# sepsamavi/safe-interactive-crowdnav

Measured on AMD Instinct MI355X. Metric: sampled trajectories/sec (N x K, 50 denoise steps), higher is better.
Workload: dtype fp16 activations x split-fp16 weights (weight-lo term as one bf8 MFMA per k64), fp32 accumulate; 1 GPU; cfg3: 256 episodes/GPU x N=5 x K=20 x H=12, 50 DDIM steps, JMID; episodes_per_gpu=256, total_episodes=256, humans=5, samples=20, horizon=12, denoise_steps=50, net=jmid, precision=f16mx, class_default_precision=f16mx, lanes=2

## Files before the change

include/jmid_hip.h:

```cpp
#ifndef JMID_HIP_H
#define JMID_HIP_H

#include <stddef.h>
#include <stdint.h>

#ifdef __cplusplus
extern "C" {
#endif
typedef struct jmid_ctx* jmid_handle_t;

#pragma GCC visibility push(default)

enum { JMID_NET_IMID = 0, JMID_NET_JMID = 1 };
enum { JMID_MEM_HOST = 0, JMID_MEM_DEVICE = 1 };
enum { JMID_PREC_F32 = 0, JMID_PREC_F16X3 = 1, JMID_PREC_F16 = 2, JMID_PREC_F16X2 = 3, JMID_PREC_F16MX = 4 };

enum {
    JMID_OK = 0,
    JMID_EINVAL = -1,
    JMID_ENOWEIGHT = -2,
    JMID_EHIP = -3,
    JMID_ENOMEM = -4,
    JMID_ERANGE = -5,
    JMID_ETIMEOUT = -6,
    JMID_EHISTORY = -7
};

const char* jmid_version(void);
int jmid_device_count(void);

int jmid_create(jmid_handle_t* out, int device_id, int net_kind, int ctx_dim, int tf_layer, int nhead,
                int hist_len);
int jmid_destroy(jmid_handle_t h);
const char* jmid_last_error(jmid_handle_t h);

int jmid_load_weight(jmid_handle_t h, const char* name, const float* host_data, size_t n_elems);
int jmid_finalize_weights(jmid_handle_t h);

int jmid_set_ddim_table(jmid_handle_t h, int n_steps, const float* beta, const float* c_e, const float* c_x,
                        const float* n_x, const float* n_e);

int jmid_set_ddpm_table(jmid_handle_t h, int n_steps, const float* beta, const float* c0, const float* c1,
                        const float* sigma, const int* use_noise);

int jmid_encode(jmid_handle_t h, int n_agents, const float* x_st, const float* nbr_sum, const float* edge_mask,
                float* ctx_out, int mem);

int jmid_denoise(jmid_handle_t h, int E, int A, int K, int T, const float* x_T, const float* ctx,
                 const float* p0, float dt, int precision, float* vel_out, float* pos_out, int mem);

int jmid_denoise_ddpm(jmid_handle_t h, int E, int A, int K, int T, const float* x_T, const float* z, const float* ctx,
                      const float* p0, float dt, int precision, float* vel_out, float* pos_out, int mem);

int jmid_net_eval(jmid_handle_t h, int E, int A, int K, int T, int step_idx, const float* x, const float* ctx,
                  int precision, float* e_out, int mem);

int jmid_episode_metrics(jmid_handle_t h, int E, int A, int K, int T, const float* pos, const float* gt,
                         float* out, int mem);

int jmid_eval_statistics(jmid_handle_t h, int E, int A, int K, int T, const float* pos, const float* gt, float* agent_out,
                         float* scene_out, int mem);

int jmid_eval_statistics_masked(jmid_handle_t h, int E, int A, int K, int T, const float* pos, const float* gt,
                                const uint8_t* interp_future, const uint8_t* skip, int n_cut, const int* cutoffs, float* agent_out,
                                float* cut_out, float* scene_out, int mem);

int jmid_collision_statistics(jmid_handle_t h, int E, int A, int K, int T, const float* pos, double threshold,
                              float* pair_out, uint8_t* agent_out, float* sample_out, float* scene_out, int mem);

int jmid_topk(jmid_handle_t h, int E, int A, int K, int T, int k, const float* pos, const float* bw, float* sel, float* logw,
              int mem);

int jmid_predict(jmid_handle_t h, int E, int A, int K, int T, int k, const float* x_st, const float* nbr_sum, const float* edge_mask,
                 const float* x_T, const float* p0, float dt, int precision, const float* bw, float* sel, float* logw, float* pos_out);

int jmid_build_scene(jmid_handle_t h, int E, int N, int F, const double* human_xy, const double* robot_xy, double time_step, int horizon,
                     int force_all_in_cluster, uint8_t* in_cluster_out, uint8_t* robot_in_cluster_out, int* n_in_out, double* cv_out, int mem);

int jmid_scene_get(jmid_handle_t h, float* x, float* x_st, float* nbr_sum, float* edge_mask, float* p0, int mem);

int jmid_predict_scene(jmid_handle_t h, int E, int A, int K, int T, int k, const float* x_T, float dt, int precision, const float* bw,
                       float* sel, float* logw, float* pos_out);

int jmid_build_scene_stamped(jmid_handle_t h, int E, int N, int R, const double* stamps, const double* human_xy, const double* robot_xy,
                             const int* n_frames, double time_step, int horizon, int force_all_in_cluster, uint8_t* in_cluster_out,
                             uint8_t* robot_in_cluster_out, int* n_in_out, int* n_grid_out, double* cv_out, int mem);

int jmid_scene_get_frames(jmid_handle_t h, double* human_xy_out, double* robot_xy_out, double* pose_now_out, int mem);

int jmid_forecast_scene(jmid_handle_t h, int E, int A, int K, int T, int k, const float* x_T, float dt, int precision, const float* bw,
                        double* forecasts_out, double* logw_out);

int jmid_noise_fill(jmid_handle_t h, uint64_t seed, int E, int rows, int T, const uint32_t* episode_ids, int draw, float* out, int mem);

int jmid_denoise_seeded(jmid_handle_t h, int E, int A, int K, int T, uint64_t seed, const uint32_t* episode_ids, const float* ctx,
                        const float* p0, float dt, int precision, float* vel_out, float* pos_out, int mem);

int jmid_predict_scene_seeded(jmid_handle_t h, int E, int A, int K, int T, int k, uint64_t seed, const uint32_t* episode_ids, float dt,
                              int precision, const float* bw, float* sel, float* logw, float* pos_out);
int jmid_forecast_scene_seeded(jmid_handle_t h, int E, int A, int K, int T, int k, uint64_t seed, const uint32_t* episode_ids, float dt,
                               int precision, const float* bw, double* forecasts_out, double* logw_out);

int jmid_set_caller_stream(jmid_handle_t h, void* stream);

int64_t jmid_graph_replays(jmid_handle_t h);

int64_t jmid_erange_count(jmid_handle_t h);
int64_t jmid_timeout_count(jmid_handle_t h);

int jmid_set_chunk_episodes(jmid_handle_t h, int episodes);
int jmid_set_tuning(jmid_handle_t h, const char* key, int value);
int jmid_profile_enable(jmid_handle_t h, uint32_t class_mask);
int jmid_profile_reset(jmid_handle_t h);
int jmid_profile_get(jmid_handle_t h, int cls, int64_t* n_launches, double* total_ms);
int jmid_kernel_class_count(void);
const char* jmid_kernel_class_name(int cls);
int jmid_synchronize(jmid_handle_t h);

#ifdef JMID_DIAGNOSTICS
int jmid_dbg_gemm(jmid_handle_t h, int M, int N, int K, const float* A, const float* Wt, const float* bias, int relu,
                  int precision, float* C);
int jmid_dbg_attention(jmid_handle_t h, int nseq, int S, const float* QKV, int precision, float* OUT);
int jmid_dbg_gemm_ln_mx(jmid_handle_t h, int M, int K, const float* A, const float* Wt, const float* bias, const float* gamma,
                        const float* beta, float* X, int fused);
int jmid_dbg_add_layernorm(jmid_handle_t h, int M, int d, float* X, const float* Y, const float* gamma,
                           const float* beta);
int jmid_dbg_plan_chunks(int net_kind, int nhead, int lanes, int chunk_episodes, int E, int tokens_per_episode, int* sizes, int cap);
int jmid_dbg_plan_chunks_mode(int net_kind, int nhead, int lanes, int chunk_episodes, int E, int tokens_per_episode, int precision, int* sizes, int cap);
#define JMID_DBG_GEMM_PLAN_KNOBS 13
int jmid_dbg_gemm_plan(int mode, int epi, int out, int M, int N, int K, int small_now, int one_chunk, const int* knobs, int* plan);
int jmid_dbg_qkv0(jmid_handle_t h, int E, int A, int K, int T, const float* x, const float* hyp, int hyp_width, int step, int precision,
                  float* qkv, float* thyp_row);
int jmid_dbg_noise_words(jmid_handle_t h, uint64_t seed, int E, int rows, int T, const uint32_t* episode_ids, int draw, uint32_t* out, int mem);
#endif

#pragma GCC visibility pop
#ifdef __cplusplus
}
#endif
#endif
```

safe-interactive-crowdnav_amd/_lib.py:

```python
from __future__ import annotations

import ctypes as C
import os

from .build import library_path

c_float_p = C.POINTER(C.c_float)
Handle = C.c_void_p

NET_IMID, NET_JMID = 0, 1
MEM_HOST, MEM_DEVICE = 0, 1
PREC_F32, PREC_F16X3, PREC_F16, PREC_F16X2, PREC_F16MX = 0, 1, 2, 3, 4
PRECISIONS = {"f32": PREC_F32, "f16x3": PREC_F16X3, "f16": PREC_F16, "f16x2": PREC_F16X2, "f16mx": PREC_F16MX}

ERR_NAMES = {-1: "JMID_EINVAL", -2: "JMID_ENOWEIGHT", -3: "JMID_EHIP", -4: "JMID_ENOMEM", -5: "JMID_ERANGE", -6: "JMID_ETIMEOUT",
             -7: "JMID_EHISTORY"}

SIGNATURES = {
    "jmid_version": (C.c_char_p, []),
    "jmid_device_count": (C.c_int, []),
    "jmid_create": (C.c_int, [C.POINTER(Handle), C.c_int, C.c_int, C.c_int, C.c_int, C.c_int, C.c_int]),
    "jmid_destroy": (C.c_int, [Handle]),
    "jmid_last_error": (C.c_char_p, [Handle]),
    "jmid_load_weight": (C.c_int, [Handle, C.c_char_p, C.c_void_p, C.c_size_t]),
    "jmid_finalize_weights": (C.c_int, [Handle]),
    "jmid_set_ddim_table": (C.c_int, [Handle, C.c_int, C.c_void_p, C.c_void_p, C.c_void_p, C.c_void_p, C.c_void_p]),
    "jmid_set_ddpm_table": (C.c_int, [Handle, C.c_int, C.c_void_p, C.c_void_p, C.c_void_p, C.c_void_p, C.c_void_p]),
    "jmid_denoise_ddpm": (C.c_int, [Handle, C.c_int, C.c_int, C.c_int, C.c_int, C.c_void_p, C.c_void_p, C.c_void_p,
                                    C.c_void_p, C.c_float, C.c_int, C.c_void_p, C.c_void_p, C.c_int]),
    "jmid_encode": (C.c_int, [Handle, C.c_int, C.c_void_p, C.c_void_p, C.c_void_p, C.c_void_p, C.c_int]),
    "jmid_denoise": (C.c_int, [Handle, C.c_int, C.c_int, C.c_int, C.c_int, C.c_void_p, C.c_void_p, C.c_void_p,
                               C.c_float, C.c_int, C.c_void_p, C.c_void_p, C.c_int]),
    "jmid_net_eval": (C.c_int, [Handle, C.c_int, C.c_int, C.c_int, C.c_int, C.c_int, C.c_void_p, C.c_void_p,
                                C.c_int, C.c_void_p, C.c_int]),
    "jmid_episode_metrics": (C.c_int, [Handle, C.c_int, C.c_int, C.c_int, C.c_int, C.c_void_p, C.c_void_p,
                                       C.c_void_p, C.c_int]),
    "jmid_eval_statistics": (C.c_int, [Handle, C.c_int, C.c_int, C.c_int, C.c_int, C.c_void_p, C.c_void_p, C.c_void_p,
                                       C.c_void_p, C.c_int]),
    "jmid_eval_statistics_masked": (C.c_int, [Handle, C.c_int, C.c_int, C.c_int, C.c_int, C.c_void_p, C.c_void_p, C.c_void_p,
                                              C.c_void_p, C.c_int, C.POINTER(C.c_int), C.c_void_p, C.c_void_p, C.c_void_p, C.c_int]),
    "jmid_collision_statistics": (C.c_int, [Handle, C.c_int, C.c_int, C.c_int, C.c_int, C.c_void_p, C.c_double, C.c_void_p,
                                            C.c_void_p, C.c_void_p, C.c_void_p, C.c_int]),
    "jmid_topk": (C.c_int, [Handle, C.c_int, C.c_int, C.c_int, C.c_int, C.c_int, C.c_void_p, C.c_void_p, C.c_void_p,
                            C.c_void_p, C.c_int]),
    "jmid_predict": (C.c_int, [Handle, C.c_int, C.c_int, C.c_int, C.c_int, C.c_int, C.c_void_p, C.c_void_p, C.c_void_p, C.c_void_p,
                               C.c_void_p, C.c_float, C.c_int, C.c_void_p, C.c_void_p, C.c_void_p, C.c_void_p]),
    "jmid_build_scene": (C.c_int, [Handle, C.c_int, C.c_int, C.c_int, C.c_void_p, C.c_void_p, C.c_double, C.c_int, C.c_int, C.c_void_p,
                                   C.c_void_p, C.c_void_p, C.c_void_p, C.c_int]),
    "jmid_scene_get": (C.c_int, [Handle, C.c_void_p, C.c_void_p, C.c_void_p, C.c_void_p, C.c_void_p, C.c_int]),
    "jmid_predict_scene": (C.c_int, [Handle, C.c_int, C.c_int, C.c_int, C.c_int, C.c_int, C.c_void_p, C.c_float, C.c_int, C.c_void_p,
                                     C.c_void_p, C.c_void_p, C.c_void_p]),
    "jmid_build_scene_stamped": (C.c_int, [Handle, C.c_int, C.c_int, C.c_int, C.c_void_p, C.c_void_p, C.c_void_p, C.c_void_p, C.c_double,
                                           C.c_int, C.c_int, C.c_void_p, C.c_void_p, C.c_void_p, C.c_void_p, C.c_void_p, C.c_int]),
    "jmid_scene_get_frames": (C.c_int, [Handle, C.c_void_p, C.c_void_p, C.c_void_p, C.c_int]),
    "jmid_forecast_scene": (C.c_int, [Handle, C.c_int, C.c_int, C.c_int, C.c_int, C.c_int, C.c_void_p, C.c_float, C.c_int, C.c_void_p,
                                      C.c_void_p, C.c_void_p]),
    "jmid_noise_fill": (C.c_int, [Handle, C.c_uint64, C.c_int, C.c_int, C.c_int, C.c_void_p, C.c_int, C.c_void_p, C.c_int]),
    "jmid_denoise_seeded": (C.c_int, [Handle, C.c_int, C.c_int, C.c_int, C.c_int, C.c_uint64, C.c_void_p, C.c_void_p, C.c_void_p,
                                      C.c_float, C.c_int, C.c_void_p, C.c_void_p, C.c_int]),
    "jmid_predict_scene_seeded": (C.c_int, [Handle, C.c_int, C.c_int, C.c_int, C.c_int, C.c_int, C.c_uint64, C.c_void_p, C.c_float, C.c_int,
                                            C.c_void_p, C.c_void_p, C.c_void_p, C.c_void_p]),
    "jmid_forecast_scene_seeded": (C.c_int, [Handle, C.c_int, C.c_int, C.c_int, C.c_int, C.c_int, C.c_uint64, C.c_void_p, C.c_float, C.c_int,
                                             C.c_void_p, C.c_void_p, C.c_void_p]),
    "jmid_set_chunk_episodes": (C.c_int, [Handle, C.c_int]),
    "jmid_set_tuning": (C.c_int, [Handle, C.c_char_p, C.c_int]),
    "jmid_set_caller_stream": (C.c_int, [Handle, C.c_void_p]),
    "jmid_graph_replays": (C.c_int64, [Handle]),
    "jmid_erange_count": (C.c_int64, [Handle]),
    "jmid_timeout_count": (C.c_int64, [Handle]),
    "jmid_profile_enable": (C.c_int, [Handle, C.c_uint32]),
    "jmid_profile_reset": (C.c_int, [Handle]),
    "jmid_profile_get": (C.c_int, [Handle, C.c_int, C.POINTER(C.c_int64), C.POINTER(C.c_double)]),
    "jmid_kernel_class_count": (C.c_int, []),
    "jmid_kernel_class_name": (C.c_char_p, [C.c_int]),
    "jmid_synchronize": (C.c_int, [Handle]),
}

DIAG_SIGNATURES = {
    "jmid_dbg_gemm": (C.c_int, [Handle, C.c_int, C.c_int, C.c_int, C.c_void_p, C.c_void_p, C.c_void_p, C.c_int,
                                C.c_int, C.c_void_p]),
    "jmid_dbg_attention": (C.c_int, [Handle, C.c_int, C.c_int, C.c_void_p, C.c_int, C.c_void_p]),
    "jmid_dbg_gemm_ln_mx": (C.c_int, [Handle, C.c_int, C.c_int, C.c_void_p, C.c_void_p, C.c_void_p, C.c_void_p, C.c_void_p,
                                      C.c_void_p, C.c_int]),
    "jmid_dbg_add_layernorm": (C.c_int, [Handle, C.c_int, C.c_int, C.c_void_p, C.c_void_p, C.c_void_p, C.c_void_p]),
    "jmid_dbg_plan_chunks": (C.c_int, [C.c_int, C.c_int, C.c_int, C.c_int, C.c_int, C.c_int, C.POINTER(C.c_int), C.c_int]),
    "jmid_dbg_plan_chunks_mode": (C.c_int, [C.c_int, C.c_int, C.c_int, C.c_int, C.c_int, C.c_int, C.c_int, C.POINTER(C.c_int), C.c_int]),
    "jmid_dbg_gemm_plan": (C.c_int, [C.c_int] * 8 + [C.POINTER(C.c_int), C.POINTER(C.c_int)]),
    "jmid_dbg_qkv0": (C.c_int, [Handle, C.c_int, C.c_int, C.c_int, C.c_int, C.c_void_p, C.c_void_p, C.c_int, C.c_int, C.c_int, C.c_void_p, C.c_void_p]),
    "jmid_dbg_noise_words": (C.c_int, [Handle, C.c_uint64, C.c_int, C.c_int, C.c_int, C.c_void_p, C.c_int, C.c_void_p, C.c_int]),
}


class JmidError(RuntimeError):
    def __init__(self, code: int, message: str):
        super().__init__(f"{ERR_NAMES.get(code, code)}: {message}")
        self.code = code


_LIBS = {}


def load_library(path: str = None) -> C.CDLL:
    key = os.path.abspath(path or library_path())
    if key in _LIBS:
        return _LIBS[key]
    import torch

    path = key
    if not os.path.exists(path):
        raise ImportError(
            f"{path} is missing: build it with `python -c 'import __graft_entry__ as g; g.build()'` "
            "(hipcc --offload-arch=gfx950).  The predictor has no CPU fallback.")
    lib = C.CDLL(path)
    for name, (res, args) in SIGNATURES.items():
        fn = getattr(lib, name)
        fn.restype = res
        fn.argtypes = args
    lib.has_diagnostics = b"diagnostics" in lib.jmid_version()
    if lib.has_diagnostics:
        for name, (res, args) in DIAG_SIGNATURES.items():
            fn = getattr(lib, name)
            fn.restype = res
            fn.argtypes = args
    _LIBS[key] = lib
    return lib
```

safe-interactive-crowdnav_amd/csrc/common.hpp:

```cpp
#pragma once
#include <hip/hip_runtime.h>
#include <hip/hip_fp16.h>
#include <stdint.h>

#include <atomic>
#include <mutex>

namespace jmid {

typedef float f32x4 __attribute__((ext_vector_type(4)));
typedef float f32x16 __attribute__((ext_vector_type(16)));
typedef _Float16 f16x8 __attribute__((ext_vector_type(8)));
typedef _Float16 f16x4 __attribute__((ext_vector_type(4)));
typedef _Float16 f16x2 __attribute__((ext_vector_type(2)));

constexpr int kWave = 64;
constexpr int kPeMaxLen = 24;

struct HyperLayout {
    int g1, b1, g3, b3, g4, b4, go, bo, total;
};
__host__ __device__ inline HyperLayout make_hyper_layout(int d_model, int d_mid, int d_low) {
    HyperLayout L;
    L.g1 = 0;
    L.b1 = L.g1 + d_model;
    L.g3 = L.b1 + d_model;
    L.b3 = L.g3 + d_mid;
    L.g4 = L.b3 + d_mid;
    L.b4 = L.g4 + d_low;
    L.go = L.b4 + d_low;
    L.bo = L.go + 2;
    L.total = L.bo + 2;
    return L;
}

__device__ __forceinline__ int fast_div(int x, int d, unsigned m) {
    return m ? (int)__umulhi((unsigned)x, m) : (d == 1 ? x : x / d);
}
inline unsigned fast_div_magic(int d, unsigned long long x_max) {
    return d > 1 && x_max * (unsigned long long)d < (1ull << 32) ? (unsigned)((1ull << 32) / (unsigned)d + 1) : 0u;
}

struct RowMap {
    int T, A, KA;
    unsigned mT = 0, mKA = 0, mA = 0;
    __device__ __forceinline__ int ea(int m) const {
        const int r = fast_div(m, T, mT);
        const int e = fast_div(r, KA, mKA);
        const int a = r - fast_div(r, A, mA) * A;
        return e * A + a;
    }
    __device__ __forceinline__ int t_of(int m) const { return m - fast_div(m, T, mT) * T; }
};
inline RowMap make_rowmap(int T, int A, int KA, unsigned long long M) {
    RowMap r{T, A, KA};
    r.mT = fast_div_magic(T, M);
    r.mKA = fast_div_magic(KA, M);
    r.mA = fast_div_magic(A, M);
    return r;
}

__host__ __device__ __forceinline__ size_t blk_index(int row, int k, int K) {
    const int rb = row >> 7, r = row & 127, kb = k >> 5, kk = k & 31;
    return ((size_t)rb * (K >> 5) + kb) * 4096 + (size_t)(r * 32 + ((((kk >> 3) ^ ((r >> 2) & 3)) << 3) | (kk & 7)));
}
__host__ __device__ __forceinline__ size_t blk_plane_elems(size_t rows, int K) {
    return ((rows + 127) / 128) * 128 * (size_t)K;
}

__host__ __device__ __forceinline__ int vt_key_pos(int key) {
    const int g = (key >> 2) & 3;
    return (key & ~15) | ((((g & 1) << 1) | (g >> 1)) << 2) | (key & 3);
}
__host__ __device__ __forceinline__ int vt_spad(int S) { return (S + 15) / 16 * 16; }

template <typename T>
__device__ __forceinline__ void args_now(const T& a) {
    static_assert(sizeof(T) % 4 == 0, "argument block of whole dwords");
    struct Words { unsigned w[sizeof(T) / 4]; };
    const Words w = __builtin_bit_cast(Words, a);
#pragma unroll
    for (unsigned i = 0; i < sizeof(T) / 4; ++i) asm volatile("" ::"s"(w.w[i]));
}
template <typename... T>
__device__ __forceinline__ void args_now_each(const T&... t) { (args_now(t), ...); }

__device__ __forceinline__ unsigned long long pin_uniform(unsigned long long v) {
    asm volatile("" : "+s"(v));
    return v;
}
__device__ __forceinline__ unsigned long long pin_uniform_rfl(unsigned long long v) {
    const unsigned lo = __builtin_amdgcn_readfirstlane((unsigned)v), hi = __builtin_amdgcn_readfirstlane((unsigned)(v >> 32));
    unsigned long long u = ((unsigned long long)hi << 32) | lo;
    asm volatile("" : "+s"(u));
    return u;
}

struct Tuning {
    int fuse_embed = 1;
    int ln_fuse = 0;
    int ln_rows = 0;
    int bystander_lds = 0;
    int gemm_h_variant = 0;
    int gemm_ng = 0;
    int no_vt_direct = 0;
    int attn_h_variant = 0;
    int attn_pack = 1;
    int vt_stage = 0;
    int graph = 0;
    int attn_nsplit = 0;
    int csl_swap = 0;
    int attn_sm = 0;
    int attn_prio = 0;
    int attn_one_wg = 0;
    int h1_stage = 0;
    int out_traj = 0;
    int attn_mx = 0;
    int mx_ln = 0;
    int attn_pf = 0;
    int gemm_small = 0;
    int small_cmb = 0;
    int small_lnx = 0;
    int cus = 256;
    int lnx_polls = 0;
    int lnx_withhold = 0;
    int small_lnx2 = 0;
    int gemm_pn = 0;
    int small_lanes = 0;
    int small_qk = 0;
    int small_pn = 0;
    int qkv0 = 0;
    int attn_abl = 0;
    int gemm_abl = 0;
};
#ifdef JMID_ABLATIONS
inline int attn_abl_bits(const Tuning& t) { return t.attn_abl; }
inline int gemm_abl_bits(const Tuning& t) { return t.gemm_abl; }
#else
inline int attn_abl_bits(const Tuning&) { return 0; }
inline int gemm_abl_bits(const Tuning&) { return 0; }
#endif

struct DevSeen {
    std::atomic<bool> v[64];
    DevSeen() { for (auto& b : v) b.store(false, std::memory_order_relaxed); }
};
struct DeviceOnce {
    std::unique_lock<std::mutex> lk;
    std::atomic<bool>* slot = nullptr;
    explicit operator bool() const { return slot != nullptr; }
    DeviceOnce() = default;
    DeviceOnce(DeviceOnce&& o) noexcept : lk(std::move(o.lk)), slot(o.slot) { o.slot = nullptr; }
    ~DeviceOnce() { if (slot) slot->store(true, std::memory_order_release); }
};
inline std::mutex& device_once_mutex() {
    static std::mutex m;
    return m;
}
inline DeviceOnce first_use_on_device(DevSeen& seen) {
    int dev = 0;
    (void)hipGetDevice(&dev);
    dev &= 63;
    DeviceOnce o;
    if (seen.v[dev].load(std::memory_order_acquire)) return o;
    o.lk = std::unique_lock<std::mutex>(device_once_mutex());
    if (seen.v[dev].load(std::memory_order_acquire)) {
        o.lk.unlock();
        return o;
    }
    o.slot = &seen.v[dev];
    return o;
}

template <auto Kernel, size_t MaxLds = 0, typename... Args>
inline hipError_t launch_with_lds(dim3 grid, dim3 block, size_t lds_bytes, hipStream_t st, Args... args) {
    static DevSeen seen;
    if (auto once_ = first_use_on_device(seen))
        (void)hipFuncSetAttribute(reinterpret_cast<const void*>(Kernel), hipFuncAttributeMaxDynamicSharedMemorySize,
                                  (int)(MaxLds ? MaxLds : lds_bytes));
    hipLaunchKernelGGL(Kernel, grid, block, lds_bytes, st, args...);
    return hipGetLastError();
}

template <typename F>
static inline int bystander_lds(int n, F* fn) {
    if (n > 0) (void)hipFuncSetAttribute((const void*)fn, hipFuncAttributeMaxDynamicSharedMemorySize, n);
    return n;
}

__device__ __forceinline__ float sigmoidf_(float x) { return 1.0f / (1.0f + expf(-x)); }

__device__ __forceinline__ float wave_sum(float v) {
#pragma unroll
    for (int o = 32; o > 0; o >>= 1) v += __shfl_xor(v, o, 64);
    return v;
}

__device__ __forceinline__ void half_swap(float x, float& lo_half, float& hi_half) {
#ifdef JMID_ATT_SHFL
    lo_half = x;
    hi_half = __shfl_xor(x, 32, 64);
#else
    float a = x, b = x;
    asm volatile("s_nop 1\n\tv_permlane32_swap_b32 %0, %1" : "+v"(a), "+v"(b));
    lo_half = a;
    hi_half = b;
#endif
}

__device__ __forceinline__ int frag_row(int reg, int hi) { return (reg & 3) + 8 * (reg >> 2) + 4 * hi; }

}
```

safe-interactive-crowdnav_amd/csrc/jmid_abi.hip:

```cpp
#include "jmid_ctx.hpp"
#include "collision_stats.hpp"

namespace jmid_host {

std::string& thread_error() {
    static thread_local std::string e;
    return e;
}

int fail(jmid_ctx* h, int code, const std::string& msg) {
    if (h) h->err = msg;
    thread_error() = msg;
    return code;
}

int ensure_kde_ws(jmid_ctx* h, size_t need, const char* who) {
    if (need <= h->kde_ws_bytes) return 0;
    if (h->kde_ws) {
        HIPCHK(h, hipStreamSynchronize(h->stream));
        HIPCHK(h, hipFree(h->kde_ws));
        h->kde_ws = nullptr;
        h->kde_ws_bytes = 0;
    }
    if (hipMalloc((void**)&h->kde_ws, need) != hipSuccess) return fail(h, JMID_ENOMEM, std::string(who) + " workspace allocation failed");
// ... 630 lines not shown
    if (int rc = ensure_kde_ws(h, need, "jmid_collision_statistics")) return rc;
    CollisionStatsArgs g{};
    g.E = E; g.A = A; g.K = K; g.T = T;
    g.threshold = threshold;
    g.pos = pos ? pos : h->last_pos;
    g.ws = reinterpret_cast<double*>(h->kde_ws + o_ws);
    g.pair_out = pair_out; g.agent_out = agent_out; g.sample_out = sample_out; g.scene_out = scene_out;
    if (host) {
        if (pos) {
            float* dp = reinterpret_cast<float*>(h->kde_ws + o_pos);
            HIPCHK(h, hipMemcpyAsync(dp, pos, n_pos * 4, hipMemcpyHostToDevice, h->stream));
            g.pos = dp;
        }
        if (pair_out) g.pair_out = reinterpret_cast<float*>(h->kde_ws + o_pr);
        if (agent_out) g.agent_out = reinterpret_cast<unsigned char*>(h->kde_ws + o_ag);
        if (sample_out) g.sample_out = reinterpret_cast<float*>(h->kde_ws + o_sm);
        if (scene_out) g.scene_out = reinterpret_cast<float*>(h->kde_ws + o_sc);
    }
    {
        ProfScope ps(h, KC_EVAL_STATS);
        HIPCHK(h, launch_collision_stats(g, h->stream));
    }
    if (host) {
        if (n_pr) HIPCHK(h, hipMemcpyAsync(pair_out, g.pair_out, n_pr * 4, hipMemcpyDeviceToHost, h->stream));
        if (n_ag) HIPCHK(h, hipMemcpyAsync(agent_out, g.agent_out, n_ag, hipMemcpyDeviceToHost, h->stream));
        if (n_sm) HIPCHK(h, hipMemcpyAsync(sample_out, g.sample_out, n_sm * 4, hipMemcpyDeviceToHost, h->stream));
        if (n_sc) HIPCHK(h, hipMemcpyAsync(scene_out, g.scene_out, n_sc * 4, hipMemcpyDeviceToHost, h->stream));
        HIPCHK(h, hipStreamSynchronize(h->stream));
    }
    return order_out(h, mem);
}

int jmid_topk(jmid_handle_t h, int E, int A, int K, int T, int k, const float* pos, const float* bw, float* sel, float* logw,
              int mem) {
    if (!h || !sel || !logw || E <= 0 || A <= 0 || K <= 1 || T <= 0) return fail(h, JMID_EINVAL, "bad argument");
    if (k < 1 || k > K) return fail(h, JMID_EINVAL, "k must be in 1..K");
    if (A > 32 || K > 1024 || T > 24) return fail(h, JMID_EINVAL, "jmid_topk supports A <= 32, K <= 1024, T <= 24");
    HIPCHK(h, hipSetDevice(h->device));
    if (!pos && !resident_positions(h, E, A, K, T)) return JMID_EINVAL;
    if (int rc = order_in(h, mem)) return rc;
    const int d = 2 * A;
    const size_t n_pos = (size_t)E * K * A * T * 2, n_sel = (size_t)E * A * k * T * 2, n_lw = (size_t)E * A * k;
    auto up = [](size_t b) { return (b + 255) / 256 * 256; };
    const size_t y_bytes = kde_y_in_lds(A, K) ? 0 : up((size_t)E * T * K * d * 8);
    const size_t o_ll = 0, o_Y = up((size_t)E * T * K * 8), o_bw = o_Y + y_bytes, o_pos = o_bw + up(T * 4),
                 o_sel = o_pos + (pos && mem == JMID_MEM_HOST ? up(n_pos * 4) : 0), o_lw = o_sel + (mem == JMID_MEM_HOST ? up(n_sel * 4) : 0),
                 need = o_lw + (mem == JMID_MEM_HOST ? up(n_lw * 4) : 0);
    if (int rc = ensure_kde_ws(h, need, "jmid_topk")) return rc;
    KdeArgs g{};
    g.E = E; g.A = A; g.K = K; g.T = T; g.k = k;
    g.ll = reinterpret_cast<double*>(h->kde_ws + o_ll);
    g.Y = reinterpret_cast<double*>(h->kde_ws + o_Y);
    g.pos = pos ? pos : h->last_pos;
    g.sel = sel; g.logw = logw;
    if (bw) {
        float* dbw = reinterpret_cast<float*>(h->kde_ws + o_bw);
        HIPCHK(h, hipMemcpyAsync(dbw, bw, T * sizeof(float), mem == JMID_MEM_HOST ? hipMemcpyHostToDevice : hipMemcpyDeviceToDevice, h->stream));
        g.bw = dbw;
    }
    if (mem == JMID_MEM_HOST) {
        if (pos) {
            float* dp = reinterpret_cast<float*>(h->kde_ws + o_pos);
            HIPCHK(h, hipMemcpyAsync(dp, pos, n_pos * 4, hipMemcpyHostToDevice, h->stream));
            g.pos = dp;
        }
        g.sel = reinterpret_cast<float*>(h->kde_ws + o_sel);
        g.logw = reinterpret_cast<float*>(h->kde_ws + o_lw);
    }
    {
        ProfScope ps(h, KC_TOPK);
        HIPCHK(h, launch_kde(g, h->stream));
    }
    if (mem == JMID_MEM_HOST) {
        HIPCHK(h, hipMemcpyAsync(sel, g.sel, n_sel * 4, hipMemcpyDeviceToHost, h->stream));
        HIPCHK(h, hipMemcpyAsync(logw, g.logw, n_lw * 4, hipMemcpyDeviceToHost, h->stream));
        HIPCHK(h, hipStreamSynchronize(h->stream));
    }
    return order_out(h, mem);
}

int jmid_predict(jmid_handle_t h, int E, int A, int K, int T, int k, const float* x_st, const float* nbr_sum, const float* edge_mask,
                 const float* x_T, const float* p0, float dt, int precision, const float* bw, float* sel, float* logw, float* pos_out) {
    if (!h) return JMID_EINVAL;
    if (int rc = check_ready(h)) return rc;
    if (E <= 0 || A <= 0 || K <= 0 || T <= 0 || k < 1 || k > K) return fail(h, JMID_EINVAL, "jmid_predict: bad dimensions");
    if (!x_st || !nbr_sum || !edge_mask || !x_T || !p0) return fail(h, JMID_EINVAL, "jmid_predict: null input");
    const bool rank = k < K;
    if (rank && (!sel || !logw)) return fail(h, JMID_EINVAL, "jmid_predict: k < K needs sel and logw");
    if (!rank && !pos_out) return fail(h, JMID_EINVAL, "jmid_predict: k == K needs pos_out");
    if (rank && (A > 32 || K > 1024 || T > 24)) return fail(h, JMID_EINVAL, "jmid_predict: the device top-k supports A <= 32, K <= 1024, T <= 24");
    if (h->ddpm) return fail(h, JMID_EINVAL, "jmid_predict samples with DDIM (MID.eval_sicnav: sampling=\"ddim\", MID/mid.py:333)");
    HIPCHK(h, hipSetDevice(h->device));
    return predict_chain(h, E, A, K, T, k, x_st, nbr_sum, edge_mask, x_T, p0, dt, precision, bw, sel, logw, pos_out, false, "jmid_predict");
}

int jmid_build_scene(jmid_handle_t h, int E, int N, int F, const double* human_xy, const double* robot_xy, double time_step, int horizon,
                     int force_all_in_cluster, uint8_t* in_cluster_out, uint8_t* robot_in_cluster_out, int* n_in_out, double* cv_out, int mem) {
    if (!h) return JMID_EINVAL;
    if (E <= 0 || !human_xy || !robot_xy || !in_cluster_out || !robot_in_cluster_out || !n_in_out) return fail(h, JMID_EINVAL, "jmid_build_scene: bad argument");
    if (int rc = check_scene_dims(h, "jmid_build_scene", N, F, cv_out, horizon, time_step)) return rc;
    HIPCHK(h, hipSetDevice(h->device));
    if (int rc = order_in(h, mem)) return rc;
    if (int rc = build_scene_resident(h, E, N, F, human_xy, robot_xy, mem == JMID_MEM_HOST ? 0 : 1, time_step, horizon, force_all_in_cluster,
                                      in_cluster_out, robot_in_cluster_out, n_in_out, cv_out, mem))
        return rc;
    return order_out(h, mem);
}

int jmid_build_scene_stamped(jmid_handle_t h, int E, int N, int R, const double* stamps, const double* human_xy, const double* robot_xy,
                             const int* n_frames, double time_step, int horizon, int force_all_in_cluster, uint8_t* in_cluster_out,
                             uint8_t* robot_in_cluster_out, int* n_in_out, int* n_grid_out, double* cv_out, int mem) {
    if (!h) return JMID_EINVAL;
    if (E <= 0 || !stamps || !human_xy || !robot_xy || !in_cluster_out || !robot_in_cluster_out || !n_in_out || !n_grid_out)
        return fail(h, JMID_EINVAL, "jmid_build_scene_stamped: bad argument");
    if (R < 1 || R > FRM_MAX_R) return fail(h, JMID_EINVAL, "jmid_build_scene_stamped supports 1 <= R <= 64 raw frames");
    const int F = h->hist_len;
    if (int rc = check_scene_dims(h, "jmid_build_scene_stamped", N, F, cv_out, horizon, time_step)) return rc;
    const double wd = std::nearbyint(time_step * 100.0);
    if (!(wd >= 1.0) || wd > 9.0e15) return fail(h, JMID_EINVAL, "jmid_build_scene_stamped: round(time_step * 100) must be at least 1");
    const bool host = mem == JMID_MEM_HOST;
    if (host && n_frames)
        for (int e = 0; e < E; ++e)
            if (n_frames[e] < 1 || n_frames[e] > R)
                return fail(h, JMID_EINVAL, "jmid_build_scene_stamped: n_frames[" + std::to_string(e) + "] = " + std::to_string(n_frames[e]) + " is outside 1..R");
    HIPCHK(h, hipSetDevice(h->device));
    if (int rc = order_in(h, mem)) return rc;
    auto up = [](size_t b) { return (b + 255) / 256 * 256; };
    const size_t b_st = (size_t)E * R * 8, b_hum = (size_t)E * R * N * 2 * 8, b_rob = (size_t)E * R * 2 * 8, b_nf = n_frames ? (size_t)E * 4 : 0;
    const GridBlock gb = grid_block(E, N, F);
    const size_t o_ng = gb.end, o_st = o_ng + up((size_t)E * 4), o_rh = o_st + (host ? up(b_st) : 0), o_rr = o_rh + (host ? up(b_hum) : 0),
                 o_nf = o_rr + (host ? up(b_rob) : 0), need = o_nf + (host ? up(b_nf) : 0), raw = need - o_st;
    if (need > h->frames_bytes) {
        HIPCHK(h, hipStreamSynchronize(h->stream));
        if (h->frames_dev) HIPCHK(h, hipFree(h->frames_dev));
        h->frames_dev = nullptr;
        h->frames_bytes = 0;
        if (hipMalloc((void**)&h->frames_dev, need) != hipSuccess) return fail(h, JMID_ENOMEM, "jmid_build_scene_stamped: workspace allocation failed");
        h->frames_bytes = need;
    }
    if (int rc = ensure_pin(h, raw + (size_t)E * 4, "jmid_build_scene_stamped")) return rc;
    char* fd = h->frames_dev;
    FramesArgs f{};
    f.E = E; f.N = N; f.R = R; f.F = F;
    f.w = (long long)wd;
    f.stamps = stamps; f.human_xy = human_xy; f.robot_xy = robot_xy; f.n_frames = n_frames;
    f.o_human = reinterpret_cast<double*>(fd + gb.o_hum); f.o_robot = reinterpret_cast<double*>(fd + gb.o_rob);
    f.o_pose = reinterpret_cast<double*>(fd + gb.o_pose); f.o_n_grid = reinterpret_cast<int*>(fd + o_ng);
    if (host) {
        std::memcpy(h->pin, stamps, b_st);
        std::memcpy(h->pin + (o_rh - o_st), human_xy, b_hum);
        std::memcpy(h->pin + (o_rr - o_st), robot_xy, b_rob);
        if (n_frames) std::memcpy(h->pin + (o_nf - o_st), n_frames, b_nf);
        HIPCHK(h, hipMemcpyAsync(fd + o_st, h->pin, raw, hipMemcpyHostToDevice, h->stream));
        f.stamps = reinterpret_cast<const double*>(fd + o_st); f.human_xy = reinterpret_cast<const double*>(fd + o_rh);
        f.robot_xy = reinterpret_cast<const double*>(fd + o_rr);
        f.n_frames = n_frames ? reinterpret_cast<const int*>(fd + o_nf) : nullptr;
    }
    HIPCHK(h, launch_frames(f, h->stream));
    int* ng = reinterpret_cast<int*>(h->pin + raw);
    HIPCHK(h, hipMemcpyAsync(ng, f.o_n_grid, (size_t)E * 4, hipMemcpyDeviceToHost, h->stream));
    if (!host) HIPCHK(h, hipMemcpyAsync(n_grid_out, f.o_n_grid, (size_t)E * 4, hipMemcpyDeviceToDevice, h->stream));
    HIPCHK(h, hipStreamSynchronize(h->stream));
    if (host) std::memcpy(n_grid_out, ng, (size_t)E * 4);
    for (int e = 0; e < E; ++e)
        if (ng[e] < 0) {
            (void)order_out(h, mem);
            return fail(h, JMID_EINVAL, "jmid_build_scene_stamped: n_frames[" + std::to_string(e) + "] is outside 1..R");
        }
    for (int e = 0; e < E; ++e)
        if (ng[e] < F) {
            const int got = ng[e];
            (void)order_out(h, mem);
            return fail(h, JMID_EHISTORY, "jmid_build_scene_stamped: episode " + std::to_string(e) + " has " + std::to_string(got) +
                                              " history frames on the time_step grid, " + std::to_string(F) + " needed");
        }
    if (int rc = build_scene_resident(h, E, N, F, reinterpret_cast<const double*>(fd), nullptr, 2, time_step, horizon, force_all_in_cluster,
                                      in_cluster_out, robot_in_cluster_out, n_in_out, cv_out, mem))
        return rc;
    return order_out(h, mem);
}

int jmid_scene_get_frames(jmid_handle_t h, double* human_xy_out, double* robot_xy_out, double* pose_now_out, int mem) {
    if (!h) return JMID_EINVAL;
    const jmid_ctx::SceneWs& sc = h->scene;
    if (!sc.E) return fail(h, JMID_EINVAL, "jmid_scene_get_frames needs a preceding jmid_build_scene on this handle");
    HIPCHK(h, hipSetDevice(h->device));
    if (int rc = order_in(h, mem)) return rc;
    const size_t F = h->hist_len, row = (size_t)sc.N * 2 * 8;
    const hipMemcpyKind kind = mem == JMID_MEM_HOST ? hipMemcpyDeviceToHost : hipMemcpyDeviceToDevice;
    if (human_xy_out) HIPCHK(h, hipMemcpyAsync(human_xy_out, sc.dev + sc.o_hum, (size_t)sc.E * F * row, kind, h->stream));
    if (robot_xy_out) HIPCHK(h, hipMemcpyAsync(robot_xy_out, sc.dev + sc.o_rob, (size_t)sc.E * F * 2 * 8, kind, h->stream));
    if (pose_now_out) {
        if (sc.stamped) HIPCHK(h, hipMemcpyAsync(pose_now_out, sc.dev + sc.o_pose, (size_t)sc.E * row, kind, h->stream));
        else
            HIPCHK(h, hipMemcpy2DAsync(pose_now_out, row, sc.dev + sc.o_hum + (F - 1) * row, F * row, row, sc.E, kind, h->stream));
    }
    if (mem == JMID_MEM_HOST) HIPCHK(h, hipStreamSynchronize(h->stream));
    return order_out(h, mem);
}

int jmid_scene_get(jmid_handle_t h, float* x, float* x_st, float* nbr_sum, float* edge_mask, float* p0, int mem) {
    if (!h) return JMID_EINVAL;
    const jmid_ctx::SceneWs& sc = h->scene;
    if (!sc.E) return fail(h, JMID_EINVAL, "jmid_scene_get needs a preceding jmid_build_scene on this handle");
    HIPCHK(h, hipSetDevice(h->device));
    if (int rc = order_in(h, mem)) return rc;
    const size_t rows = (size_t)sc.E * sc.N, F = h->hist_len;
    const hipMemcpyKind kind = mem == JMID_MEM_HOST ? hipMemcpyDeviceToHost : hipMemcpyDeviceToDevice;
    if (x) HIPCHK(h, hipMemcpyAsync(x, sc.dev + sc.o_x, rows * F * 6 * 4, kind, h->stream));
    if (x_st) HIPCHK(h, hipMemcpyAsync(x_st, sc.dev + sc.o_xst, rows * F * 6 * 4, kind, h->stream));
    if (nbr_sum) HIPCHK(h, hipMemcpyAsync(nbr_sum, sc.dev + sc.o_nbr, rows * 2 * F * 6 * 4, kind, h->stream));
    if (edge_mask) HIPCHK(h, hipMemcpyAsync(edge_mask, sc.dev + sc.o_em, rows * 2 * 4, kind, h->stream));
    if (p0) HIPCHK(h, hipMemcpyAsync(p0, sc.dev + sc.o_p0, rows * 2 * 4, kind, h->stream));
    if (mem == JMID_MEM_HOST) HIPCHK(h, hipStreamSynchronize(h->stream));
    return order_out(h, mem);
}

int jmid_predict_scene(jmid_handle_t h, int E, int A, int K, int T, int k, const float* x_T, float dt, int precision, const float* bw, float* sel,
                       float* logw, float* pos_out) {
    return predict_scene_entry(h, "jmid_predict_scene", E, A, K, T, k, x_T, nullptr, dt, precision, bw, sel, logw, pos_out, nullptr, nullptr, false);
}

int jmid_forecast_scene(jmid_handle_t h, int E, int A, int K, int T, int k, const float* x_T, float dt, int precision, const float* bw,
                        double* forecasts_out, double* logw_out) {
    return predict_scene_entry(h, "jmid_forecast_scene", E, A, K, T, k, x_T, nullptr, dt, precision, bw, nullptr, nullptr, nullptr, forecasts_out,
                               logw_out, true);
}

int jmid_predict_scene_seeded(jmid_handle_t h, int E, int A, int K, int T, int k, uint64_t seed, const uint32_t* episode_ids, float dt, int precision,
                              const float* bw, float* sel, float* logw, float* pos_out) {
    const SeedArgs sa{seed, episode_ids};
    return predict_scene_entry(h, "jmid_predict_scene_seeded", E, A, K, T, k, nullptr, &sa, dt, precision, bw, sel, logw, pos_out, nullptr, nullptr, false);
}

int jmid_forecast_scene_seeded(jmid_handle_t h, int E, int A, int K, int T, int k, uint64_t seed, const uint32_t* episode_ids, float dt, int precision,
                               const float* bw, double* forecasts_out, double* logw_out) {
    const SeedArgs sa{seed, episode_ids};
    return predict_scene_entry(h, "jmid_forecast_scene_seeded", E, A, K, T, k, nullptr, &sa, dt, precision, bw, nullptr, nullptr, nullptr, forecasts_out,
                               logw_out, true);
}

int jmid_denoise_seeded(jmid_handle_t h, int E, int A, int K, int T, uint64_t seed, const uint32_t* episode_ids, const float* ctx, const float* p0,
                        float dt, int precision, float* vel_out, float* pos_out, int mem) {
    if (!h) return JMID_EINVAL;
    if (!episode_ids) return fail(h, JMID_EINVAL, "jmid_denoise_seeded: null episode_ids");
    const SeedArgs sa{seed, episode_ids};
    return run_network(h, E, A, K, T, nullptr, ctx, p0, dt, precision, -1, vel_out, pos_out, nullptr, mem, nullptr, &sa);
}

int jmid_noise_fill(jmid_handle_t h, uint64_t seed, int E, int rows, int T, const uint32_t* episode_ids, int draw, float* out, int mem) {
    return noise_entry(h, "jmid_noise_fill", seed, E, rows, T, episode_ids, draw, out, nullptr, mem);
}

int jmid_set_chunk_episodes(jmid_handle_t h, int episodes) {
    if (!h || episodes < 0) return JMID_EINVAL;
    h->chunk_eps = episodes;
    drop_graphs(h);
    return JMID_OK;
}

int jmid_set_tuning(jmid_handle_t h, const char* key, int value) {
    if (!h || !key) return JMID_EINVAL;
    const std::string k(key);
    struct Knob {
        const char* name;
        int Tuning::*field;
        int lo, hi;
    };
#ifdef JMID_DIAGNOSTICS
    static const Knob knobs[] = {
        {"gemm_h_variant", &Tuning::gemm_h_variant, 0, 8},
        {"attn_pack", &Tuning::attn_pack, 0, 1},
        {"fuse_embed", &Tuning::fuse_embed, 0, 1},
        {"bystander_lds", &Tuning::bystander_lds, 0, 160 * 1024},
        {"ln_rows", &Tuning::ln_rows, 0, 128},
        {"ln_fuse", &Tuning::ln_fuse, 0, 2},
        {"no_vt_direct", &Tuning::no_vt_direct, 0, 1},
        {"gemm_ng", &Tuning::gemm_ng, 0, 64},
        {"attn_h_variant", &Tuning::attn_h_variant, 0, 2},
        {"vt_stage", &Tuning::vt_stage, 0, 3},
        {"graph", &Tuning::graph, 0, 2},
        {"attn_nsplit", &Tuning::attn_nsplit, 0, 16},
        {"attn_mx", &Tuning::attn_mx, 0, 3},
        {"out_traj", &Tuning::out_traj, 0, 2},
        {"attn_pf", &Tuning::attn_pf, 0, 2},
        {"attn_one_wg", &Tuning::attn_one_wg, 0, 1},
        {"attn_sm", &Tuning::attn_sm, 0, 2},
        {"attn_prio", &Tuning::attn_prio, 0, 2},
        {"mx_ln", &Tuning::mx_ln, 0, 2},
        {"csl_swap", &Tuning::csl_swap, 0, 3},
        {"h1_stage", &Tuning::h1_stage, 0, 2},
        {"gemm_small", &Tuning::gemm_small, 0, 2},
        {"gemm_pn", &Tuning::gemm_pn, 0, 8},
        {"small_lanes", &Tuning::small_lanes, 0, 2},
        {"small_cmb", &Tuning::small_cmb, 0, 2},
        {"small_lnx", &Tuning::small_lnx, 0, 2},
        {"cus", &Tuning::cus, 0, 4096},
        {"lnx_polls", &Tuning::lnx_polls, 0, 1 << 20},
        {"lnx_withhold", &Tuning::lnx_withhold, 0, 1},
        {"small_lnx2", &Tuning::small_lnx2, 0, 2},
        {"small_qk", &Tuning::small_qk, 0, 2},
        {"small_pn", &Tuning::small_pn, 0, 8},
        {"qkv0", &Tuning::qkv0, 0, 2},
#ifdef JMID_ABLATIONS
        {"attn_abl", &Tuning::attn_abl, 0, 1 << 30},
        {"gemm_abl", &Tuning::gemm_abl, 0, 1 << 30},
#endif
    };
#endif
    if (k == "lanes") {
        if (value < 1 || value > jmid_ctx::kMaxLanes) return fail(h, JMID_EINVAL, "lanes must be 1..4");
        h->lanes = value;
        return JMID_OK;
    }
#ifdef JMID_DIAGNOSTICS
    for (const Knob& kn : knobs)
        if (k == kn.name) {
            if (value < kn.lo || value > kn.hi || (k == "ln_rows" && value != 0 && value != 64 && value != 128))
                return fail(h, JMID_EINVAL, k + " out of range");
            h->tune.*(kn.field) = value;
            if (k == "cus" && value == 0) {
                int cus = 0;
                h->tune.cus = hipDeviceGetAttribute(&cus, hipDeviceAttributeMultiprocessorCount, h->device) == hipSuccess && cus > 0 ? cus : 256;
            }
            drop_graphs(h);
            return JMID_OK;
        }
#endif
    return fail(h, JMID_EINVAL, "unknown tuning key " + k);
}

int64_t jmid_graph_replays(jmid_handle_t h) { return h ? h->graph_replays : -1; }

int64_t jmid_erange_count(jmid_handle_t h) { return h ? h->erange_calls : -1; }
int64_t jmid_timeout_count(jmid_handle_t h) { return h ? h->lnx_timeouts : -1; }

int jmid_set_caller_stream(jmid_handle_t h, void* stream) {
    if (!h) return JMID_EINVAL;
    h->caller_stream = reinterpret_cast<hipStream_t>(stream);
    return JMID_OK;
}

int jmid_synchronize(jmid_handle_t h) {
    if (!h) return JMID_EINVAL;
    HIPCHK(h, hipSetDevice(h->device));
    HIPCHK(h, hipStreamSynchronize(h->stream));
    return JMID_OK;
}

}
```

safe-interactive-crowdnav_amd/csrc/jmid_ctx.hpp:

```cpp
#pragma once
#include "../../include/jmid_hip.h"

#include <hip/hip_runtime.h>

#include <algorithm>
#include <cmath>
#include <cstdio>
#include <cstring>
#include <map>
#include <string>
#include <vector>

#include "attn_f16x3.hpp"
#include "attn_f32.hpp"
#include "common.hpp"
#include "elementwise.hpp"
#include "encoder.hpp"
#include "eval_stats.hpp"
#include "gemm_f16x3.hpp"
#include "gemm_ln_f16x3.hpp"
#include "gemm_ln2_mx.hpp"
#include "gemm_small.hpp"
#include "gemm_f32.hpp"
#include "kde.hpp"
#include "launch_plan.hpp"
#include "noise.hpp"
#include "qkv0.hpp"
#include "scene.hpp"
#include "frames.hpp"

using namespace jmid;

enum KClass {
    KC_GEMM_QKV = 0,
    KC_GEMM_OUT,
    KC_GEMM_FF1,
    KC_GEMM_FF2,
    KC_GEMM_TAIL,
    KC_ATTN,
    KC_ADD_LN,
    KC_EMBED,
    KC_OUT_DDIM,
    KC_HYPER,
    KC_ENCODER,
    KC_INTEGRATE,
    KC_METRICS,
    KC_VTRANS,
    KC_TOPK,
    KC_EVAL_STATS,
    KC_COUNT
};
extern const char* const kClassNames[KC_COUNT];

struct DevBuf {
    float* p = nullptr;
    size_t n = 0;
};

struct EvPair {
    hipEvent_t a, b;
};

struct HalfPair {
    half_t* hi = nullptr;
    half_t* lo = nullptr;
};

struct LinearW {
    const float *W = nullptr, *bias = nullptr;
    HalfPair split;
    HalfPair k16;
    const unsigned char* w8 = nullptr;
};
struct NormW {
    const float *gamma = nullptr, *beta = nullptr;
};
struct LayerW {
    LinearW in_proj, out_proj, linear1, linear2;
    NormW norm1, norm2;
};
struct WeightTable {
    std::vector<LayerW> layers;
    LinearW concat1, concat3, concat4, linear;
    const float* edge_v = nullptr;
};

struct jmid_ctx {
    int device = 0;
    hipStream_t stream = nullptr;
    static constexpr int kMaxLanes = 4;
    hipStream_t lane_stream[kMaxLanes - 1] = {nullptr, nullptr, nullptr};
    hipEvent_t ev_fork = nullptr, ev_join[kMaxLanes - 1] = {nullptr, nullptr, nullptr};
    int lanes = 2;
    Tuning tune;
    hipStream_t caller_stream = nullptr;
    hipEvent_t ev_in = nullptr, ev_out = nullptr;
    struct LoopGraph {
        hipGraphExec_t exec = nullptr;
        char* arena = nullptr;
        bool warm = false;
    };
    std::map<std::string, LoopGraph> graphs;
    int64_t graph_replays = 0;
    const float* last_pos = nullptr;
    int last_pos_dims[4] = {0, 0, 0, 0};
    char* kde_ws = nullptr;
    size_t kde_ws_bytes = 0;
    char* pin = nullptr;
    size_t pin_bytes = 0;
    char* io_dev = nullptr;
    size_t io_dev_bytes = 0;
    struct SceneWs {
        char* dev = nullptr;
        size_t bytes = 0;
        int E = 0, N = 0;
        size_t o_x = 0, o_xst = 0, o_nbr = 0, o_em = 0, o_p0 = 0, o_inc = 0;
        std::vector<int> n_in;
        size_t o_hum = 0, o_rob = 0, o_pose = 0, o_cv = 0;
        bool stamped = false;
        int horizon = 0;
    } scene;
    char* frames_dev = nullptr;
    size_t frames_bytes = 0;
    unsigned* noise_ids = nullptr;
    int noise_ids_cap = 0;
    unsigned* noise_ids_pin = nullptr;
    hipEvent_t ev_ids = nullptr;
    bool chained = false;
    int64_t erange_calls = 0;
    unsigned lnx_epoch = 0;
    bool lnx_off = false;
    int64_t lnx_timeouts = 0;
    int x2 = 0;
    int net_kind = 1, ctx_dim = 256, tf_layer = 3, nhead = 4, hist_len = 6;
    int d = 512, ff = 1024, dmid = 256, dlow = 128, H = 128;
    HyperLayout hl;
    std::map<std::string, std::vector<size_t>> expected;
    std::map<std::string, DevBuf> w;
    std::map<std::string, HalfPair> wsplit;
    struct W8Image { unsigned char* p = nullptr; };
    std::map<std::string, W8Image> w8;
    int mx = 0;
    std::map<std::string, HalfPair> w16;
    WeightTable wt;
    int* range_flag = nullptr;
    bool weights_in_half_range = true;
    bool finalized = false;
    float* pe = nullptr;
    float* ppe = nullptr;
    float* Whyp = nullptr;
    float* bhyp = nullptr;
    float* thyp = nullptr;
    std::vector<float> time_w;
    float* lstmT[3][3] = {{nullptr}};
    float* attW1T = nullptr;
    float* attW2T = nullptr;
    std::vector<float> beta, c_e, c_x, n_x, n_e;
    bool ddpm = false;
    std::vector<float> p_c0, p_c1, p_sigma;
    std::vector<int> p_noise;
    char* arena = nullptr;
    size_t arena_bytes = 0;
    int chunk_eps = 0;
    uint32_t prof_mask = 0;
    std::vector<EvPair> prof_ev[KC_COUNT];
    std::vector<EvPair> ev_pool;
    double prof_ms[KC_COUNT] = {0};
    int64_t prof_n[KC_COUNT] = {0};
    std::string err;
};

constexpr size_t kLnxWords = 2 * jmid::SM_LNX_GRANULES;

namespace jmid_host {

std::string& thread_error();
int fail(jmid_ctx* h, int code, const std::string& msg);

#define HIPCHK(h, expr)                                                                               \
    do {                                                                                              \
        hipError_t e__ = (expr);                                                                      \
        if (e__ != hipSuccess)                                                                        \
            return fail(h, JMID_EHIP, std::string(#expr) + ": " + hipGetErrorString(e__));            \
    } while (0)

struct ProfScope {
    jmid_ctx* h;
    int cls;
    bool on;
    EvPair ev;
    ProfScope(jmid_ctx* h_, int cls_) : h(h_), cls(cls_), on((h_->prof_mask >> cls_) & 1u) {
        if (on) {
            if (!h->ev_pool.empty()) {
                ev = h->ev_pool.back();
                h->ev_pool.pop_back();
            } else {
                hipEventCreate(&ev.a);
                hipEventCreate(&ev.b);
            }
            hipEventRecord(ev.a, h->stream);
        }
    }
    ~ProfScope() {
        if (on) {
            hipEventRecord(ev.b, h->stream);
            h->prof_ev[cls].push_back(ev);
        }
    }
};

struct Carver {
    char* base;
    size_t off = 0;
    explicit Carver(char* b) : base(b) {}
    float* take(size_t nfloats) {
        float* p = reinterpret_cast<float*>(base ? base + off : nullptr);
        off += ((nfloats * sizeof(float) + 255) / 256) * 256;
        return p;
    }
};

inline size_t numel(const std::vector<size_t>& s) {
    size_t n = 1;
    for (size_t v : s) n *= v;
    return n;
}

void register_shapes(jmid_ctx* h);
int dev_alloc_copy(jmid_ctx* h, float** out, const std::vector<float>& host);
int fetch_host(jmid_ctx* h, const std::string& name, std::vector<float>& out);
int upload_time_table(jmid_ctx* h);
int make_w8(jmid_ctx* h, const float* dW, int N, int K, jmid_ctx::W8Image* out);
void free_planes(jmid_ctx* h);
void drop_graphs(jmid_ctx* h);
void sync_lanes(jmid_ctx* h);
int ensure_arena(jmid_ctx* h, size_t bytes);
std::vector<int> plan_chunks(const jmid_ctx* h, int E, int tokens_per_episode);
int check_ready(jmid_ctx* h);
int order_in(jmid_ctx* h, int mem);
int order_out(jmid_ctx* h, int mem);
struct SeedArgs {
    uint64_t seed;
    const uint32_t* ids;
};
int upload_noise_ids(jmid_ctx* h, const uint32_t* ids, int E);
int fill_noise(jmid_ctx* h, uint64_t seed, const unsigned* ids_dev, int E, size_t n, int draw, float* out, unsigned* words, hipStream_t stream);
int run_network(jmid_ctx* h, int E, int A, int K, int T, const float* x_in, const float* ctx, const float* p0, float dt,
                int precision, int single_step, float* vel_out, float* pos_out, float* e_out, int mem,
                const float* z_in = nullptr, const SeedArgs* seeded = nullptr);
int flagged_call(jmid_ctx* h, int flag);
int launch_episode_metrics(jmid_ctx* h, const float* pos, const float* gt, float* out, int E, int K, int A, int T);
#ifdef JMID_DIAGNOSTICS
int dbg_qkv0(jmid_ctx* h, int E, int A, int K, int T, const float* x, const float* hyp, int hyp_width, int step, int precision, float* qkv, float* thyp_row);
#endif
int noise_entry(jmid_ctx* h, const char* who, uint64_t seed, int E, int rows, int T, const uint32_t* episode_ids, int draw, float* out,
                unsigned* words, int mem);
int prof_collect(jmid_ctx* h);

}
using namespace jmid_host;
```

safe-interactive-crowdnav_amd/csrc/jmid_diag.hip:

```cpp
#include "jmid_ctx.hpp"
#include "jmid_launch.hpp"

#ifdef JMID_DIAGNOSTICS
extern "C" {

int jmid_dbg_plan_chunks(int net_kind, int nhead, int lanes, int chunk_episodes, int E, int tokens_per_episode, int* sizes, int cap) {
    if (E <= 0 || tokens_per_episode <= 0 || nhead <= 0 || !sizes || cap <= 0) return JMID_EINVAL;
    jmid_ctx ctx;
    ctx.net_kind = net_kind; ctx.nhead = nhead; ctx.lanes = lanes; ctx.chunk_eps = chunk_episodes;
    const std::vector<int> plan = plan_chunks(&ctx, E, tokens_per_episode);
    for (size_t i = 0; i < plan.size() && (int)i < cap; ++i) sizes[i] = plan[i];
    return (int)plan.size();
}

int jmid_dbg_plan_chunks_mode(int net_kind, int nhead, int lanes, int chunk_episodes, int E, int tokens_per_episode, int precision, int* sizes, int cap) {
    if (E <= 0 || tokens_per_episode <= 0 || nhead <= 0 || !sizes || cap <= 0) return JMID_EINVAL;
    if (precision != JMID_PREC_F32 && precision != JMID_PREC_F16X3 && precision != JMID_PREC_F16X2 && precision != JMID_PREC_F16MX) return JMID_EINVAL;
    jmid_ctx ctx;
    ctx.net_kind = net_kind; ctx.nhead = nhead; ctx.lanes = lanes; ctx.chunk_eps = chunk_episodes;
    ctx.mx = precision == JMID_PREC_F16MX;
    ctx.x2 = precision == JMID_PREC_F16X2 || ctx.mx;
    const std::vector<int> plan = plan_chunks(&ctx, E, tokens_per_episode);
    for (size_t i = 0; i < plan.size() && (int)i < cap; ++i) sizes[i] = plan[i];
    return (int)plan.size();
}

int jmid_dbg_gemm_plan(int mode, int epi, int out, int M, int N, int K, int small_now, int one_chunk, const int* knobs, int* plan) {
    if (mode < GM_X3 || mode > GM_MX || epi < EPI_BIAS || epi > EPI_CSL || (out != OUT_F32 && out != OUT_SPLIT && out != OUT_QKV && out != OUT_LNX) ||
        M <= 0 || N <= 0 || K <= 0 || !knobs || !plan || knobs[0] < 0 || knobs[0] > 8)
        return JMID_EINVAL;
    Tuning t;
    int Tuning::*const fields[JMID_DBG_GEMM_PLAN_KNOBS] = {&Tuning::gemm_h_variant, &Tuning::gemm_small, &Tuning::ln_rows, &Tuning::small_lnx, &Tuning::small_lnx2,
                                                           &Tuning::cus, &Tuning::vt_stage, &Tuning::csl_swap, &Tuning::h1_stage, &Tuning::gemm_pn,
                                                           &Tuning::small_qk, &Tuning::small_pn, &Tuning::gemm_ng};
    for (int i = 0; i < JMID_DBG_GEMM_PLAN_KNOBS; ++i) t.*fields[i] = knobs[i];
    CallFacts cf;
    cf.small_now = small_now;
    cf.one_chunk = one_chunk;
    const GemmPlan p = plan_gemm((GemmMode)mode, epi, out, M, N, K, cf, t);
    plan[0] = p.mode; plan[1] = p.shape; plan[2] = p.flags; plan[3] = p.group_tiles;
    plan[4] = gemm_shape_bm(p.shape); plan[5] = gemm_shape_bn(p.shape);
    plan[6] = plan_ln_rows(false, M, t); plan[7] = plan_ln_rows(true, M, t);
    return JMID_OK;
}

int jmid_dbg_gemm(jmid_handle_t h, int M, int N, int K, const float* A, const float* Wt, const float* bias, int relu,
                  int precision, float* C) {
    if (!h || !A || !Wt || !C) return JMID_EINVAL;
    if (precision != JMID_PREC_F32 && precision != JMID_PREC_F16X3 && precision != JMID_PREC_F16X2 && precision != JMID_PREC_F16MX)
        return fail(h, JMID_EINVAL, "bad precision");
    h->mx = precision == JMID_PREC_F16MX;
    h->x2 = precision == JMID_PREC_F16X2 || h->mx;
    HIPCHK(h, hipSetDevice(h->device));
    if (!h->range_flag) {
        HIPCHK(h, hipMalloc((void**)&h->range_flag, sizeof(int)));
        HIPCHK(h, hipMemsetAsync(h->range_flag, 0, sizeof(int), h->stream));
    }
    float *dA, *dW, *dB = nullptr, *dC;
    HIPCHK(h, hipMalloc((void**)&dA, (size_t)M * K * 4));
    HIPCHK(h, hipMalloc((void**)&dW, (size_t)N * K * 4));
    HIPCHK(h, hipMalloc((void**)&dC, (size_t)M * N * 4));
    HIPCHK(h, hipMemcpy(dA, A, (size_t)M * K * 4, hipMemcpyHostToDevice));
    HIPCHK(h, hipMemcpy(dW, Wt, (size_t)N * K * 4, hipMemcpyHostToDevice));
    if (bias) {
        HIPCHK(h, hipMalloc((void**)&dB, (size_t)N * 4));
        HIPCHK(h, hipMemcpy(dB, bias, (size_t)N * 4, hipMemcpyHostToDevice));
    }
    int rc = 0;
    half_t *ah = nullptr, *al = nullptr, *wh = nullptr, *wl = nullptr;
    jmid_ctx::W8Image w8img;
    if (precision == JMID_PREC_F32) {
        GemmArgs g{};
        g.A = dA; g.lda = K; g.W = dW; g.ldw = K; g.bias = dB; g.C = dC; g.ldc = N; g.M = M; g.N = N; g.K = K;
        rc = relu ? run_gemm<EPI_BIAS_RELU>(h, KC_GEMM_QKV, g) : run_gemm<EPI_BIAS>(h, KC_GEMM_QKV, g);
    } else {
        const size_t pa = blk_plane_elems(M, K) * 2, pw = blk_plane_elems(N, K) * 2;
        HIPCHK(h, hipMalloc((void**)&ah, pa));
        HIPCHK(h, hipMalloc((void**)&al, pa));
        HIPCHK(h, hipMalloc((void**)&wh, pw));
        HIPCHK(h, hipMalloc((void**)&wl, pw));
        for (auto pr : {std::make_pair(ah, pa), std::make_pair(al, pa), std::make_pair(wh, pw), std::make_pair(wl, pw)})
            HIPCHK(h, hipMemsetAsync(pr.first, 0, pr.second, h->stream));
        hipLaunchKernelGGL(split_planes_blocked_kernel, dim3(512), dim3(256), 0, h->stream, dA, ah, al, M, K,
                           h->range_flag, 1.0f);
        hipLaunchKernelGGL(split_planes_blocked_kernel, dim3(512), dim3(256), 0, h->stream, dW, wh, wl, N, K,
                           h->range_flag, kWScale);
        GemmHArgs g{};
        g.Ahi = ah; g.Alo = al; g.Whi = wh; g.Wlo = wl; g.bias = dB; g.C = dC; g.ldc = N;
        g.M = M; g.N = N; g.K = K;
        if (h->mx && N % 32 == 0 && K % 64 == 0) {
            if (int rc8 = make_w8(h, dW, N, K, &w8img)) return rc8;
            g.W8 = w8img.p;
        }
        const GemmPlan plan = plan_gemm(gemm_mode(h), relu ? EPI_BIAS_RELU : EPI_BIAS, OUT_F32, M, N, K, CallFacts{}, h->tune);
        rc = relu ? run_gemm_h<EPI_BIAS_RELU, OUT_F32>(h, KC_GEMM_QKV, g, plan) : run_gemm_h<EPI_BIAS, OUT_F32>(h, KC_GEMM_QKV, g, plan);
    }
    if (!rc) {
        hipError_t e = hipStreamSynchronize(h->stream);
        if (e != hipSuccess) rc = fail(h, JMID_EHIP, hipGetErrorString(e));
    }
    if (!rc) HIPCHK(h, hipMemcpy(C, dC, (size_t)M * N * 4, hipMemcpyDeviceToHost));
    hipFree(dA); hipFree(dW); hipFree(dC);
    if (dB) hipFree(dB);
    for (half_t* p : {ah, al, wh, wl})
        if (p) hipFree(p);
    if (w8img.p) hipFree(w8img.p);
    return rc;
}

int jmid_dbg_attention(jmid_handle_t h, int nseq, int S, const float* QKV, int precision, float* OUT) {
    if (!h || !QKV || !OUT) return JMID_EINVAL;
    if (precision != JMID_PREC_F32 && precision != JMID_PREC_F16X3 && precision != JMID_PREC_F16X2 && precision != JMID_PREC_F16MX)
        return fail(h, JMID_EINVAL, "bad precision");
    h->mx = precision == JMID_PREC_F16MX;
    h->x2 = precision == JMID_PREC_F16X2 || h->mx;
    HIPCHK(h, hipSetDevice(h->device));
    if (!h->range_flag) {
        HIPCHK(h, hipMalloc((void**)&h->range_flag, sizeof(int)));
        HIPCHK(h, hipMemsetAsync(h->range_flag, 0, sizeof(int), h->stream));
    }
    const size_t Mt = (size_t)nseq * S;
    const int d = h->d, hd = h->d / h->nhead;
    float *dQ, *dO;
    HIPCHK(h, hipMalloc((void**)&dQ, Mt * 3 * d * 4));
    HIPCHK(h, hipMalloc((void**)&dO, Mt * d * 4));
    HIPCHK(h, hipMemcpy(dQ, QKV, Mt * 3 * d * 4, hipMemcpyHostToDevice));
    int rc = 0;
    std::vector<half_t*> tmp;
    if (precision == JMID_PREC_F32) {
        AttnArgs aa{dQ, dO, S, d, h->nhead, 1.0f / sqrtf((float)hd), nullptr, nullptr};
        ProfScope ps(h, KC_ATTN);
        hipError_t e = launch_attn_f32(aa, nseq, hd, plan_attn(hd, h->tune).pack, h->stream);
        if (e != hipSuccess) rc = fail(h, JMID_EHIP, hipGetErrorString(e));
    } else {
        const int Spad = vt_spad(S);
        const size_t vt = (size_t)nseq * d * Spad;
        half_t* b[8];
        const size_t sz[8] = {Mt * d, Mt * d, Mt * d, Mt * d, vt, vt, blk_plane_elems(Mt, d), blk_plane_elems(Mt, d)};
        for (int i = 0; i < 8; ++i) {
            HIPCHK(h, hipMalloc((void**)&b[i], sz[i] * sizeof(half_t)));
            HIPCHK(h, hipMemsetAsync(b[i], 0, sz[i] * sizeof(half_t), h->stream));
            tmp.push_back(b[i]);
        }
        hipLaunchKernelGGL(qkv_to_planes_kernel, dim3(512), dim3(256), 0, h->stream, dQ, b[0], b[1], b[2], b[3], b[4],
                           b[5], Mt, d, hd, S, Spad, 1.4426950408889634f / sqrtf((float)hd));
        int ns = 1;
        float *opart = nullptr, *mlpart = nullptr;
        if (hd == 128) ns = attn_pick_nsplit(((S + 127) / 128) * h->nhead * nseq, S);
        if (ns > 1) {
            HIPCHK(h, hipMalloc((void**)&opart, (size_t)ns * Mt * d * 4));
            HIPCHK(h, hipMalloc((void**)&mlpart, (size_t)ns * Mt * h->nhead * 2 * 4));
            tmp.push_back(reinterpret_cast<half_t*>(opart));
            tmp.push_back(reinterpret_cast<half_t*>(mlpart));
        }
        AttnHArgs aa{b[0], b[1], b[2], b[3], b[4], b[5], b[6], b[7], S, Spad, d, h->nhead, 1.0f / sqrtf((float)hd),
                     h->range_flag, ns, opart, mlpart, h->x2};
        {
            ProfScope ps(h, KC_ATTN);
            hipError_t e = launch_attn_f16x3(aa, nseq, hd, plan_attn(hd, h->tune), h->stream);
            if (e != hipSuccess) rc = fail(h, JMID_EHIP, hipGetErrorString(e));
        }
        hipLaunchKernelGGL(merge_planes_kernel, dim3(512), dim3(256), 0, h->stream, b[6], b[7], dO, (int)Mt, d);
    }
    if (!rc) {
        hipError_t e = hipStreamSynchronize(h->stream);
        if (e != hipSuccess) rc = fail(h, JMID_EHIP, hipGetErrorString(e));
    }
    if (!rc) HIPCHK(h, hipMemcpy(OUT, dO, Mt * d * 4, hipMemcpyDeviceToHost));
    hipFree(dQ); hipFree(dO);
    for (half_t* p : tmp) hipFree(p);
    return rc;
}

int jmid_dbg_gemm_ln_mx(jmid_handle_t h, int M, int K, const float* A, const float* Wt, const float* bias, const float* gamma,
                        const float* beta, float* X, int fused) {
    if (!h || !A || !Wt || !bias || !gamma || !beta || !X || M <= 0 || K % 64 != 0) return JMID_EINVAL;
    constexpr int N = GLN_BN;
    HIPCHK(h, hipSetDevice(h->device));
    h->mx = 1;
    h->x2 = 1;
    if (!h->range_flag) {
        HIPCHK(h, hipMalloc((void**)&h->range_flag, sizeof(int)));
        HIPCHK(h, hipMemsetAsync(h->range_flag, 0, sizeof(int), h->stream));
    }
    std::vector<void*> tmp;
    auto dalloc = [&](size_t bytes, const void* host) -> void* {
        void* p = nullptr;
        if (hipMalloc(&p, bytes) != hipSuccess) return nullptr;
        tmp.push_back(p);
        if (host) (void)hipMemcpy(p, host, bytes, hipMemcpyHostToDevice);
        else (void)hipMemsetAsync(p, 0, bytes, h->stream);
        return p;
    };
    float* dA = (float*)dalloc((size_t)M * K * 4, A);
    float* dW = (float*)dalloc((size_t)N * K * 4, Wt);
    float* dB = (float*)dalloc(N * 4, bias);
    float* dG = (float*)dalloc(N * 4, gamma);
    float* dT = (float*)dalloc(N * 4, beta);
    float* dX = (float*)dalloc((size_t)M * N * 4, X);
    float* dY = (float*)dalloc((size_t)(M + 63) / 64 * 64 * N * 4, nullptr);
    const size_t pa = blk_plane_elems(M, K) * 2, pw = blk_plane_elems(N, K) * 2, px = blk_plane_elems(M, N) * 2;
    half_t* ah = (half_t*)dalloc(pa, nullptr);
    half_t* al = (half_t*)dalloc(pa, nullptr);
    half_t* wh = (half_t*)dalloc(pw, nullptr);
    half_t* wl = (half_t*)dalloc(pw, nullptr);
    half_t* w16h = (half_t*)dalloc((size_t)N * K * 2, nullptr);
    half_t* w16l = (half_t*)dalloc((size_t)N * K * 2, nullptr);
    half_t* xh = (half_t*)dalloc(px, nullptr);
    unsigned char* xl8 = (unsigned char*)dalloc(px, nullptr);
    for (void* p : tmp)
        if (!p) return fail(h, JMID_ENOMEM, "jmid_dbg_gemm_ln_mx: allocation failed");
    hipLaunchKernelGGL(split_planes_blocked_kernel, dim3(512), dim3(256), 0, h->stream, dA, ah, al, M, K, h->range_flag, 1.0f);
    hipLaunchKernelGGL(split_planes_blocked_kernel, dim3(512), dim3(256), 0, h->stream, dW, wh, wl, N, K, h->range_flag, kWScale);
    hipLaunchKernelGGL(split_planes_k16_kernel, dim3(256), dim3(256), 0, h->stream, dW, w16h, w16l, N, K);
    hipLaunchKernelGGL(split_planes_lo8_kernel, dim3(512), dim3(256), 0, h->stream, dX, xh, xl8, M);
    jmid_ctx::W8Image img;
    if (int rc = make_w8(h, dW, N, K, &img)) return rc;
    tmp.push_back(img.p);
    int rc = 0;
    if (fused == 1) {
        GemmLn2Args g2{ah, w16h, img.p, dB, dG, dT, xh, xl8, M, K, 1e-5f, h->range_flag, 0};
        hipError_t e = launch_gemm_ln2_mx(g2, plan_ln_rows(true, M, h->tune), h->stream);
        if (e != hipSuccess) rc = fail(h, JMID_EHIP, hipGetErrorString(e));
    } else {
        GemmHArgs g{};
        g.Ahi = ah; g.Alo = al; g.Whi = wh; g.Wlo = wl; g.W8 = img.p; g.bias = dB; g.C = dY; g.ldc = N; g.M = M; g.N = N; g.K = K;
        if (fused == 3) {
            unsigned long long* xs = (unsigned long long*)dalloc(kLnxWords * sizeof(unsigned), nullptr);
            const GemmPlan lnx = plan_gemm(GM_MX, EPI_BIAS, OUT_LNX, M, N, K, CallFacts{}, h->tune);
            if (!xs || lnx.shape == GS_NONE) return fail(h, JMID_EINVAL, "jmid_dbg_gemm_ln_mx: shape does not take the small kernel with the statistics exchange");
            g.ln_gamma = dG; g.ln_beta = dT; g.ln_xh = xh; g.ln_xl = nullptr; g.ln_xl8 = xl8; g.ln_xchg = xs; g.ln_eps = 1e-5f; g.ln_no_lo = 0;
            (void)hipMemsetAsync(h->range_flag, 0, sizeof(int), h->stream);
            rc = run_gemm_lnx_small(h, KC_GEMM_OUT, g, lnx);
            if (!rc) {
                int flag = 0;
                (void)hipMemcpyAsync(&flag, h->range_flag, sizeof(int), hipMemcpyDeviceToHost, h->stream);
                (void)hipStreamSynchronize(h->stream);
                if (flag & 2) rc = fail(h, JMID_EHIP, "jmid_dbg_gemm_ln_mx: a workgroup gave up waiting for its row tile's statistics");
            }
        } else
        {
        rc = run_gemm_h<EPI_BIAS, OUT_F32>(h, KC_GEMM_OUT, g, plan_gemm(GM_MX, EPI_BIAS, OUT_F32, M, N, K, CallFacts{}, h->tune));
        if (!rc) rc = run_add_ln(h, nullptr, dY, dG, dT, M, N, xh, reinterpret_cast<half_t*>(xl8), true, 0);
        }
    }
    if (!rc) {
        hipLaunchKernelGGL(merge_planes_lo8_kernel, dim3(512), dim3(256), 0, h->stream, xh, xl8, dX, M);
        hipError_t e = hipStreamSynchronize(h->stream);
        if (e != hipSuccess) rc = fail(h, JMID_EHIP, hipGetErrorString(e));
    }
    if (!rc) HIPCHK(h, hipMemcpy(X, dX, (size_t)M * N * 4, hipMemcpyDeviceToHost));
    for (void* p : tmp) hipFree(p);
    return rc;
}

int jmid_dbg_add_layernorm(jmid_handle_t h, int M, int d, float* X, const float* Y, const float* gamma,
                           const float* beta) {
    if (!h || !X || !Y || !gamma || !beta) return JMID_EINVAL;
    HIPCHK(h, hipSetDevice(h->device));
    float *dX, *dY, *dG, *dB;
    HIPCHK(h, hipMalloc((void**)&dX, (size_t)M * d * 4));
    HIPCHK(h, hipMalloc((void**)&dY, (size_t)M * d * 4));
    HIPCHK(h, hipMalloc((void**)&dG, (size_t)d * 4));
    HIPCHK(h, hipMalloc((void**)&dB, (size_t)d * 4));
    HIPCHK(h, hipMemcpy(dX, X, (size_t)M * d * 4, hipMemcpyHostToDevice));
    HIPCHK(h, hipMemcpy(dY, Y, (size_t)M * d * 4, hipMemcpyHostToDevice));
    HIPCHK(h, hipMemcpy(dG, gamma, (size_t)d * 4, hipMemcpyHostToDevice));
    HIPCHK(h, hipMemcpy(dB, beta, (size_t)d * 4, hipMemcpyHostToDevice));
    int rc = run_add_ln(h, dX, dY, dG, dB, M, d);
    if (!rc) {
        hipError_t e = hipStreamSynchronize(h->stream);
        if (e != hipSuccess) rc = fail(h, JMID_EHIP, hipGetErrorString(e));
    }
    if (!rc) HIPCHK(h, hipMemcpy(X, dX, (size_t)M * d * 4, hipMemcpyDeviceToHost));
    hipFree(dX); hipFree(dY); hipFree(dG); hipFree(dB);
    return rc;
}

int jmid_dbg_qkv0(jmid_handle_t h, int E, int A, int K, int T, const float* x, const float* hyp, int hyp_width, int step, int precision,
                  float* qkv, float* thyp_row) {
    if (!h) return JMID_EINVAL;
    return dbg_qkv0(h, E, A, K, T, x, hyp, hyp_width, step, precision, qkv, thyp_row);
}

int jmid_dbg_noise_words(jmid_handle_t h, uint64_t seed, int E, int rows, int T, const uint32_t* episode_ids, int draw, uint32_t* out, int mem) {
    return noise_entry(h, "jmid_dbg_noise_words", seed, E, rows, T, episode_ids, draw, nullptr, out, mem);
}

}
#endif
```

safe-interactive-crowdnav_amd/csrc/jmid_planner.hip:

```cpp
#include "jmid_ctx.hpp"
#include "jmid_launch.hpp"

namespace jmid_host {

void drop_graphs(jmid_ctx* h) {
    for (auto& kv : h->graphs)
        if (kv.second.exec) hipGraphExecDestroy(kv.second.exec);
    h->graphs.clear();
}

void sync_lanes(jmid_ctx* h) {
    for (int l = 0; l + 1 < jmid_ctx::kMaxLanes; ++l)
        if (h->lane_stream[l]) (void)hipStreamSynchronize(h->lane_stream[l]);
    if (h->stream) (void)hipStreamSynchronize(h->stream);
}

int ensure_arena(jmid_ctx* h, size_t bytes) {
    if (bytes <= h->arena_bytes) return 0;
    drop_graphs(h);
    h->last_pos = nullptr;
    if (h->arena) {
        sync_lanes(h);
        HIPCHK(h, hipFree(h->arena));
        h->arena = nullptr;
        h->arena_bytes = 0;
    }
    hipError_t e = hipMalloc((void**)&h->arena, bytes);
    if (e != hipSuccess) return fail(h, JMID_ENOMEM, "workspace allocation of " + std::to_string(bytes) + " bytes failed");
    h->arena_bytes = bytes;
    return 0;
}

struct StepBuffers {
    float *X, *QKV, *ATT, *Y, *H1, *Y3, *Y4;
    half_t *Xh, *Xl, *Qh, *Ql, *Kh, *Kl, *Vh, *Vl, *Vth, *Vtl, *Ah, *Al, *H1h, *H1l, *Y3h, *Y3l;
    size_t vt_elems;
    float *Opart, *MLpart;
    float *coef, *uvc;
    unsigned long long* ln_xchg;
};

half_t* take_half(Carver& c, size_t n) { return reinterpret_cast<half_t*>(c.take((n + 1) / 2)); }

struct SeqGeom {
    int nseq, S, Spad;
};
SeqGeom seq_geom(const jmid_ctx* h, int Ec, int A, int K, int T) {
    SeqGeom g;
    g.nseq = h->net_kind == JMID_NET_JMID ? Ec : Ec * K * A;
    g.S = h->net_kind == JMID_NET_JMID ? K * A * T : T;
    g.Spad = vt_spad(g.S);
    return g;
}

size_t step_ws_floats(const jmid_ctx* h, size_t Mc, int precision, const SeqGeom& sg, int nsplit, StepBuffers* sb,
                      char* base, size_t qkv0_rows) {
    Carver c(base);
    StepBuffers s{};
    s.X = c.take(Mc * h->d);
    s.Y = c.take((Mc + 63) / 64 * 64 * h->d);
    s.ln_xchg = reinterpret_cast<unsigned long long*>(c.take(kLnxWords));
    s.Y4 = c.take(Mc * h->dlow);
    if (precision == JMID_PREC_F32) {
        s.QKV = c.take(Mc * 3 * h->d);
        s.ATT = c.take(Mc * h->d);
        s.H1 = c.take(Mc * h->ff);
        s.Y3 = c.take(Mc * h->dmid);
    } else {
        s.Xh = take_half(c, blk_plane_elems(Mc, h->d));
        s.Xl = take_half(c, blk_plane_elems(Mc, h->d));
        if (h->net_kind == JMID_NET_JMID) {
            s.Qh = take_half(c, Mc * h->d);
            s.Ql = take_half(c, Mc * h->d);
            s.Kh = take_half(c, Mc * h->d);
            s.Kl = take_half(c, Mc * h->d);
            s.Vh = take_half(c, Mc * h->d);
            s.Vl = take_half(c, Mc * h->d);
            s.vt_elems = (size_t)sg.nseq * h->d * sg.Spad;
            s.Vth = take_half(c, s.vt_elems);
            s.Vtl = take_half(c, s.vt_elems);
            if (nsplit > 1) {
                s.Opart = c.take((size_t)nsplit * Mc * h->d);
                s.MLpart = c.take((size_t)nsplit * Mc * h->nhead * 2);
            }
            if (qkv0_rows) {
                s.coef = c.take(qkv0_rows * h->d);
                s.uvc = c.take(qkv0_rows * 3 * h->d);
            }
        } else {
            s.QKV = c.take(Mc * 3 * h->d);
        }
        s.Ah = take_half(c, blk_plane_elems(Mc, h->d));
        s.Al = take_half(c, blk_plane_elems(Mc, h->d));
        s.H1h = take_half(c, blk_plane_elems(Mc, h->ff));
        s.H1l = take_half(c, blk_plane_elems(Mc, h->ff));
        s.Y3h = take_half(c, blk_plane_elems(Mc, h->dmid));
        s.Y3l = take_half(c, blk_plane_elems(Mc, h->dmid));
    }
    if (sb) *sb = s;
    return c.off;
}

bool byte_lo_plane(const jmid_ctx* h) { return h->mx && h->d == GLN_BN && h->tune.mx_ln != 2; }

enum ResidualPath {
    RB_GEMM_LN2,
    RB_GEMM_LN,
    RB_LNX_SMALL,
    RB_GEMM_ADD_LN,
};
struct ResidualPlan {
    ResidualPath path;
    int ln_rows;
    GemmPlan gemm;
    bool merge;
};

ResidualPlan residual_path(const jmid_ctx* h, int M, int K, const CallFacts& cf) {
    const Tuning& t = h->tune;
    if (h->d == GLN_BN && t.ln_fuse != 2 && (t.ln_fuse == 1 || M >= 7168))
        return {byte_lo_plane(h) ? RB_GEMM_LN2 : RB_GEMM_LN, plan_ln_rows(byte_lo_plane(h), M, t), {}, false};
    if (byte_lo_plane(h) && !h->lnx_off) {
        const GemmPlan lnx = plan_gemm(GM_MX, EPI_BIAS, OUT_LNX, M, h->d, K, cf, t);
        if (lnx.shape != GS_NONE) return {RB_LNX_SMALL, 0, lnx, false};
    }
    return {RB_GEMM_ADD_LN, 0, plan_gemm(gemm_mode(h), EPI_BIAS, OUT_F32, M, h->d, K, cf, t), false};
}

bool one_launch_shape(const jmid_ctx* h, long tokens) { return h->mx && h->d == GLN_BN && tokens <= 2560; }

struct StepPlan {
    int Ec, M, T;
    int R;
    bool qkv0;
    int qkv0_steps;
    bool split, mxv2, joint;
    RowMap rm;
    SeqGeom sg;
    int hd;
    float att_scale;
    bool vt_direct;
    bool k8, q8l;
    CallFacts cf;
    GemmPlan in_proj, linear1, concat3, concat4;
    ResidualPlan out_proj, linear2;
    AttnPlan attn;
    int out_tpw;
};

StepPlan plan_step(const jmid_ctx* h, int Ec, int A, int K, int T, int precision, const CallFacts& cf) {
    StepPlan p{};
    const int d = h->d;
    p.Ec = Ec;
    p.M = Ec * K * A * T;
    p.T = T;
    p.R = Ec * A;
    p.split = precision != JMID_PREC_F32;
    p.mxv2 = p.split && byte_lo_plane(h);
    p.joint = h->net_kind == JMID_NET_JMID;
    p.rm = make_rowmap(T, A, K * A, (unsigned long long)p.M);
    p.sg = seq_geom(h, Ec, A, K, T);
    p.hd = d / h->nhead;
    p.att_scale = 1.0f / sqrtf((float)p.hd);
    p.cf = cf;
    const Tuning& t = h->tune;
    p.attn = plan_attn(p.hd, t);
    p.qkv0 = p.split && p.joint && t.qkv0 != 1 && d % 32 == 0;
    p.qkv0_steps = cf.qkv0_steps;
    if (p.split) {
        const auto gemm = [&](int epi, int out, int N, int K) { return plan_gemm(gemm_mode(h), epi, out, p.M, N, K, cf, t); };
        p.in_proj = gemm(EPI_BIAS, p.joint ? OUT_QKV : OUT_F32, 3 * d, d);
        p.linear1 = gemm(EPI_BIAS_RELU, OUT_SPLIT, h->ff, d);
        p.concat3 = gemm(EPI_CSL, OUT_SPLIT, h->dmid, d);
        p.concat4 = gemm(EPI_CSL, OUT_F32, h->dlow, h->dmid);
        p.out_proj = residual_path(h, p.M, d, cf);
        p.linear2 = residual_path(h, p.M, h->ff, cf);
    }
    if (p.split && p.joint) {
        p.vt_direct = (p.sg.S % 4 == 0) && !t.no_vt_direct;
        p.k8 = p.in_proj.mode == GM_MX && p.hd == 128 && t.attn_h_variant == 0 && t.attn_mx != 2;
        p.q8l = p.k8 && t.attn_mx != 3;
        p.out_proj.merge = p.out_proj.path == RB_LNX_SMALL && small_cmb_fits(p.attn, p.cf.attn_nsplit, h->x2, t);
    }
    if (d <= 512 && p.M % T == 0 && t.out_traj != 2 && (t.out_traj == 1 || p.M >= 4096 * 4)) {
        p.out_tpw = T;
        while (p.out_tpw > 1 && (p.M / p.out_tpw < 4096 || T % p.out_tpw != 0)) --p.out_tpw;
        if (t.out_traj == 1) p.out_tpw = T;
    }
    return p;
}

int residual_block(jmid_ctx* h, const StepPlan& p, const ResidualPlan& rp, const StepBuffers& sb, const half_t* Ahi, const half_t* Alo,
                   int K, const LinearW& lin, const NormW& nrm, int cls, bool no_lo_out) {
    const int M = p.M, d = h->d;
    unsigned char* Xl8 = p.mxv2 ? reinterpret_cast<unsigned char*>(sb.Xl) : nullptr;
    if (rp.path == RB_GEMM_LN2) {
        GemmLn2Args g2{Ahi, lin.k16.hi, lin.w8, lin.bias, nrm.gamma, nrm.beta, sb.Xh, Xl8, M, K, 1e-5f, h->range_flag, no_lo_out};
        ProfScope ps(h, cls);
        HIPCHK(h, launch_gemm_ln2_mx(g2, rp.ln_rows, h->stream));
        return 0;
    }
    if (rp.path == RB_GEMM_LN) {
        GemmLnArgs gl{Ahi, Alo, lin.k16.hi, lin.k16.lo, lin.bias, nrm.gamma, nrm.beta, sb.Xh, sb.Xl, M, K, 1e-5f, h->range_flag, h->x2};
        gl.W8 = h->mx ? lin.w8 : nullptr;
        gl.no_lo_out = h->x2 && no_lo_out;
        ProfScope ps(h, cls);
        HIPCHK(h, launch_gemm_ln(gl, rp.ln_rows, h->stream));
        return 0;
    }
    GemmHArgs g = gemm_h_args(h, p.rm, M, Ahi, Alo, lin, d, K);
    g.C = sb.Y; g.ldc = d;
    if (rp.path == RB_LNX_SMALL) {
        if (rp.merge) {
            g.cmb_O = sb.Opart; g.cmb_ML = sb.MLpart; g.cmb_ns = p.cf.attn_nsplit; g.cmb_nhead = h->nhead;
            g.cmb_Mtot = (unsigned)((size_t)p.sg.nseq * p.sg.S);
        }
        g.ln_gamma = nrm.gamma; g.ln_beta = nrm.beta; g.ln_xh = sb.Xh; g.ln_xl = nullptr;
        g.ln_xl8 = Xl8; g.ln_xchg = sb.ln_xchg; g.ln_eps = 1e-5f; g.ln_no_lo = no_lo_out;
        return run_gemm_lnx_small(h, cls, g, rp.gemm);
    }
    if (int rc = (run_gemm_h<EPI_BIAS, OUT_F32>(h, cls, g, rp.gemm))) return rc;
    return run_add_ln(h, sb.X, sb.Y, nrm.gamma, nrm.beta, M, d, sb.Xh, sb.Xl, p.mxv2, no_lo_out);
}

constexpr size_t kQkv0TableMaxBytes = size_t(512) << 20;
int qkv0_table_steps(int steps, int Ec, int A, int d) {
    const size_t bytes = (size_t)steps * Ec * A * 3 * 4 * d * sizeof(float);
    return bytes <= kQkv0TableMaxBytes ? steps : 1;
}

int qkv0_build_table(jmid_ctx* h, const StepPlan& p, const StepBuffers& sb, const float* hyp_chunk, int step0, int nsteps) {
    const int d = h->d;
    ProfScope ps(h, KC_HYPER);
    Qkv0CoefArgs ca{h->wt.concat1.W, h->wt.concat1.bias, hyp_chunk, h->thyp + (size_t)step0 * h->hl.total, sb.coef,
                    nsteps, p.R, d, h->hl.total, h->hl.g1, h->hl.b1, h->range_flag};
    const long total = (long)nsteps * p.R * (d / 4);
    hipLaunchKernelGGL(qkv0_coef_kernel, dim3((int)std::min<long>((total + 255) / 256, 256L * 16)), dim3(256), 0, h->stream, ca);
    HIPCHK(h, hipGetLastError());
    GemmArgs g{};
    g.A = sb.coef; g.lda = d; g.W = h->wt.layers[0].in_proj.W; g.ldw = d; g.C = sb.uvc; g.ldc = 3 * d;
    g.M = nsteps * p.R * 3; g.N = 3 * d; g.K = d;
    if (h->tune.qkv0 == 2) HIPCHK(h, (launch_gemm_f32<EPI_BIAS, false>(g, h->stream)));
    else HIPCHK(h, (launch_gemm_f32<EPI_BIAS, true>(g, h->stream)));
    return 0;
}

EmbedArgs embed_args(const jmid_ctx* h, const StepPlan& p, const StepBuffers& sb, const float* x_chunk, const float* hyp_chunk, const float* th) {
    unsigned char* Xl8 = p.mxv2 ? reinterpret_cast<unsigned char*>(sb.Xl) : nullptr;
    return EmbedArgs{x_chunk, h->wt.concat1.W, h->wt.concat1.bias, h->pe, hyp_chunk, th,
                     p.split ? nullptr : sb.X, p.M, h->d, h->hl.total, h->hl.g1, h->hl.b1, p.rm, p.split ? sb.Xh : nullptr,
                     p.split && !p.mxv2 ? sb.Xl : nullptr, Xl8};
}

int run_embed(jmid_ctx* h, const StepPlan& p, const StepBuffers& sb, const float* x_chunk, const float* hyp_chunk, const float* thyp) {
    ProfScope ps(h, KC_EMBED);
    EmbedArgs ea = embed_args(h, p, sb, x_chunk, hyp_chunk, thyp);
    const long total = (long)p.M * (h->d / 4);
    int blocks = (int)std::min<long>((total + 255) / 256, 256L * 16);
    hipLaunchKernelGGL(embed_kernel, dim3(blocks), dim3(256), bystander_lds(h->tune.bystander_lds, embed_kernel), h->stream, ea);
    HIPCHK(h, hipGetLastError());
    return 0;
}

struct LoImages {
    unsigned char *k8h, *k8l, *q8l;
};
LoImages lo_images(const StepPlan& p, const StepBuffers& sb, int d) {
    LoImages im{};
    im.k8h = p.k8 ? reinterpret_cast<unsigned char*>(sb.Kl) : nullptr;
    im.k8l = p.k8 ? im.k8h + (size_t)p.M * d : nullptr;
    im.q8l = p.q8l ? reinterpret_cast<unsigned char*>(sb.Ql) : nullptr;
    return im;
}

int qkv_planes(jmid_ctx* h, const StepPlan& p, const StepBuffers& sb, int l, int step_idx, const float* x_chunk, const float* hyp_chunk) {
    const int M = p.M, d = h->d, hd = p.hd, S = p.sg.S;
    const LoImages im = lo_images(p, sb, d);
    const float qscale = p.att_scale * 1.4426950408889634f;
    if (l == 0 && p.qkv0) {
        if (p.qkv0_steps <= 1)
            if (int rc = qkv0_build_table(h, p, sb, hyp_chunk, step_idx, 1)) return rc;
        Qkv0Args qa{};
        qa.x = x_chunk;
        qa.uvc = sb.uvc + (p.qkv0_steps <= 1 ? 0 : (size_t)step_idx * p.R * 9 * d);
        qa.ppe = h->ppe;
        qa.Qh = sb.Qh; qa.Ql = sb.Ql; qa.Kh = sb.Kh; qa.Kl = sb.Kl; qa.Vth = sb.Vth; qa.Vtl = sb.Vtl;
        qa.Q8l = im.q8l; qa.K8h = im.k8h; qa.K8l = im.k8l;
        qa.M = M; qa.d = d; qa.hd = hd; qa.S = S; qa.Spad = p.sg.Spad; qa.nseq = p.sg.nseq;
        qa.qscale = qscale; qa.rmap = p.rm; qa.range_flag = h->range_flag; qa.x2 = h->x2;
        qkv0_plan(qa, p.T);
        ProfScope ps(h, KC_GEMM_QKV);
        HIPCHK(h, launch_qkv0_expand(qa, h->stream));
        return 0;
    }
    GemmHArgs g = gemm_h_args(h, p.rm, M, sb.Xh, sb.Xl, h->wt.layers[l].in_proj, 3 * d, d);
    g.Chi = sb.Qh; g.Clo = sb.Ql; g.Khi = sb.Kh; g.Klo = sb.Kl;
    g.Vthi = p.vt_direct ? sb.Vth : sb.Vh; g.Vtlo = p.vt_direct ? sb.Vtl : sb.Vl; g.vt_direct = p.vt_direct;
    g.d = d; g.hd = hd; g.S = S; g.Spad = p.sg.Spad; g.qscale = qscale;
    g.K8h = im.k8h; g.K8l = im.k8l; g.Q8l = im.q8l;
    if (int rc = (run_gemm_h<EPI_BIAS, OUT_QKV>(h, KC_GEMM_QKV, g, p.in_proj))) return rc;
    if (!p.vt_direct) {
        ProfScope ps(h, KC_VTRANS);
        hipLaunchKernelGGL(v_transpose_kernel, dim3((S + 63) / 64, d / 64, p.sg.nseq), dim3(256), 0, h->stream,
                           sb.Vh, sb.Vl, sb.Vth, sb.Vtl, S, p.sg.Spad, d, hd);
        HIPCHK(h, hipGetLastError());
    }
    return 0;
}

int net_step(jmid_ctx* h, const StepPlan& p, const StepBuffers& sb, int step_idx, float* x_chunk, const float* hyp_chunk,
             float* e_out, const float* z_chunk = nullptr, bool embed_done = false, int next_step = -1) {
    const bool split = p.split;
    const int M = p.M, d = h->d, ff = h->ff;
    const WeightTable& wt = h->wt;
    const float* thyp = h->thyp + (size_t)step_idx * h->hl.total;
    const RowMap& rm = p.rm;
    if (!embed_done)
        if (int rc = run_embed(h, p, sb, x_chunk, hyp_chunk, thyp)) return rc;
    const SeqGeom& sg = p.sg;
    const int nseq = sg.nseq, S = sg.S, hd = p.hd;
    if (!split) {
        for (const LayerW& w : wt.layers) {
            if (int rc = run_gemm<EPI_BIAS>(h, KC_GEMM_QKV, gemm_args(rm, M, sb.X, w.in_proj, sb.QKV, 3 * d, d))) return rc;
            {
                ProfScope ps(h, KC_ATTN);
                AttnArgs aa{sb.QKV, sb.ATT, S, d, h->nhead, p.att_scale, nullptr, nullptr};
                HIPCHK(h, launch_attn_f32(aa, nseq, hd, p.attn.pack, h->stream));
            }
            if (int rc = run_gemm<EPI_BIAS>(h, KC_GEMM_OUT, gemm_args(rm, M, sb.ATT, w.out_proj, sb.Y, d, d))) return rc;
            if (int rc = run_add_ln(h, sb.X, sb.Y, w.norm1.gamma, w.norm1.beta, M, d)) return rc;
            if (int rc = run_gemm<EPI_BIAS_RELU>(h, KC_GEMM_FF1, gemm_args(rm, M, sb.X, w.linear1, sb.H1, ff, d))) return rc;
            if (int rc = run_gemm<EPI_BIAS>(h, KC_GEMM_FF2, gemm_args(rm, M, sb.H1, w.linear2, sb.Y, d, ff))) return rc;
            if (int rc = run_add_ln(h, sb.X, sb.Y, w.norm2.gamma, w.norm2.beta, M, d)) return rc;
        }
        GemmArgs g = gemm_args(rm, M, sb.X, wt.concat3, sb.Y3, h->dmid, d);
        g.hyp = hyp_chunk; g.thyp = thyp; g.hyp_ld = h->hl.total; g.goff = h->hl.g3; g.boff = h->hl.b3;
        if (int rc = run_gemm<EPI_CSL>(h, KC_GEMM_TAIL, g)) return rc;
        g = gemm_args(rm, M, sb.Y3, wt.concat4, sb.Y4, h->dlow, h->dmid);
        g.hyp = hyp_chunk; g.thyp = thyp; g.hyp_ld = h->hl.total; g.goff = h->hl.g4; g.boff = h->hl.b4;
        if (int rc = run_gemm<EPI_CSL>(h, KC_GEMM_TAIL, g)) return rc;
    } else {
        for (int l = 0; l < h->tf_layer; ++l) {
            const LayerW& w = wt.layers[l];
            GemmHArgs g{};
            if (p.joint) {
                if (int rc = qkv_planes(h, p, sb, l, step_idx, x_chunk, hyp_chunk)) return rc;
                const LoImages im = lo_images(p, sb, d);
                ProfScope ps(h, KC_ATTN);
                AttnHArgs aa{sb.Qh, sb.Ql, sb.Kh, sb.Kl, sb.Vth, sb.Vtl, sb.Ah, sb.Al, S, sg.Spad, d, h->nhead,
                             p.att_scale, h->range_flag, p.cf.attn_nsplit, sb.Opart, sb.MLpart, h->x2, im.k8h, im.k8l, im.q8l};
                aa.skip_combine = p.out_proj.merge;
                HIPCHK(h, launch_attn_f16x3(aa, nseq, hd, p.attn, h->stream));
            } else {
                g = gemm_h_args(h, rm, M, sb.Xh, sb.Xl, w.in_proj, 3 * d, d);
                g.C = sb.QKV; g.ldc = 3 * d;
                if (int rc = (run_gemm_h<EPI_BIAS, OUT_F32>(h, KC_GEMM_QKV, g, p.in_proj))) return rc;
                ProfScope ps(h, KC_ATTN);
                AttnArgs aa{sb.QKV, nullptr, S, d, h->nhead, p.att_scale, sb.Ah, sb.Al};
                HIPCHK(h, launch_attn_f32(aa, nseq, hd, p.attn.pack, h->stream));
            }
            if (int rc = residual_block(h, p, p.out_proj, sb, sb.Ah, sb.Al, d, w.out_proj, w.norm1, KC_GEMM_OUT, false)) return rc;
            g = gemm_h_args(h, rm, M, sb.Xh, sb.Xl, w.linear1, ff, d);
            g.Chi = sb.H1h; g.Clo = sb.H1l; g.ldc = ff;
            if (int rc = (run_gemm_h<EPI_BIAS_RELU, OUT_SPLIT>(h, KC_GEMM_FF1, g, p.linear1))) return rc;
            if (int rc = residual_block(h, p, p.linear2, sb, sb.H1h, sb.H1l, ff, w.linear2, w.norm2, KC_GEMM_FF2, l + 1 == h->tf_layer)) return rc;
        }
        GemmHArgs g = gemm_h_args(h, rm, M, sb.Xh, sb.Xl, wt.concat3, h->dmid, d);
        g.hyp = hyp_chunk; g.thyp = thyp; g.hyp_ld = h->hl.total;
        g.Chi = sb.Y3h; g.Clo = sb.Y3l; g.ldc = h->dmid; g.goff = h->hl.g3; g.boff = h->hl.b3;
        if (int rc = (run_gemm_h<EPI_CSL, OUT_SPLIT>(h, KC_GEMM_TAIL, g, p.concat3))) return rc;
        g = gemm_h_args(h, rm, M, sb.Y3h, sb.Y3l, wt.concat4, h->dlow, h->dmid);
        g.hyp = hyp_chunk; g.thyp = thyp; g.hyp_ld = h->hl.total;
        g.C = sb.Y4; g.ldc = h->dlow; g.goff = h->hl.g4; g.boff = h->hl.b4;
        if (int rc = (run_gemm_h<EPI_CSL, OUT_F32>(h, KC_GEMM_TAIL, g, p.concat4))) return rc;
    }
    {
        ProfScope ps(h, KC_OUT_DDIM);
        OutArgs oa{sb.Y4, wt.linear.W, wt.linear.bias, hyp_chunk, thyp, x_chunk, e_out,
                   M, h->dlow, h->hl.total, h->hl.go, h->hl.bo,
                   h->c_e[step_idx], h->c_x[step_idx], h->n_x[step_idx], h->n_e[step_idx], rm,
                   nullptr, 0, 0.f, 0.f, 0.f};
        if (h->ddpm && !e_out) {
            oa.ddpm = 1;
            oa.z = h->p_noise[step_idx] ? z_chunk : nullptr;
            oa.c0 = h->p_c0[step_idx];
            oa.c1 = h->p_c1[step_idx];
            oa.sigma = h->p_sigma[step_idx];
        }
        const bool embed_next = next_step >= 0 && !e_out;
        const EmbedArgs en = embed_next ? embed_args(h, p, sb, x_chunk, hyp_chunk, h->thyp + (size_t)next_step * h->hl.total) : EmbedArgs{};
        const auto launch = [&](auto* kernel, int waves, auto... tpw) {
            hipLaunchKernelGGL(kernel, dim3((waves + 3) / 4), dim3(256), bystander_lds(h->tune.bystander_lds, kernel), h->stream, oa, en, tpw...);
        };
        if (p.out_tpw && embed_next) launch(out_ddim_traj_kernel<true>, M / p.out_tpw, p.out_tpw);
        else if (p.out_tpw) launch(out_ddim_traj_kernel<false>, M / p.out_tpw, p.out_tpw);
        else if (embed_next) launch(out_ddim_kernel<true>, M);
        else launch(out_ddim_kernel<false>, M);
        HIPCHK(h, hipGetLastError());
    }
    return 0;
}

int auto_chunk(const jmid_ctx* h, int E, int tokens_per_episode) {
    const long max_tokens = 65536;
    if (h->net_kind == JMID_NET_JMID) {
        const long bpe = (long)h->nhead * ((tokens_per_episode + 127) / 128);
        for (int k = 4; k >= 1; --k) {
            const long c = (k * 512L) / bpe;
            if (c >= 1 && c * tokens_per_episode <= max_tokens) return (int)std::min<long>(c, E);
        }
    }
    long c = max_tokens / std::max(1, tokens_per_episode);
    if (c < 1) c = 1;
    return (int)std::min<long>(c, E);
}

std::vector<int> plan_chunks(const jmid_ctx* h, int E, int tokens_per_episode) {
    int c = h->chunk_eps > 0 ? std::min(E, h->chunk_eps) : auto_chunk(h, E, tokens_per_episode);
    if (h->chunk_eps <= 0 && h->lanes >= 2 && E >= 2 && h->tune.graph != 1) {
        if (E <= c) {
            const long tokens = (long)E * tokens_per_episode;
            const bool lnx_call = one_launch_shape(h, tokens) && residual_path(h, (int)tokens, h->d, CallFacts{}).path == RB_LNX_SMALL;
            c = lnx_call ? E : (E + 1) / 2;
        } else {
            int n = (E + c - 1) / c;
            if ((n & 1) && n < E) ++n;
            std::vector<int> sizes(n, E / n);
            for (int i = 0; i < E % n; ++i) sizes[i] += 1;
            return sizes;
        }
    }
    std::vector<int> sizes(E / c, c);
    const int tail = E % c;
    if (tail) {
        if (h->chunk_eps > 0 || sizes.empty() || tail * 4 >= c || (tail + sizes.size() - 1) / sizes.size() > (size_t)c / 8)
            sizes.push_back(tail);
        else
            for (int i = 0; i < tail; ++i) sizes[i % sizes.size()] += 1;
    }
    return sizes;
}

int order_in(jmid_ctx* h, int mem) {
    if (mem != JMID_MEM_DEVICE || h->chained) return 0;
    HIPCHK(h, hipEventRecord(h->ev_in, h->caller_stream));
    HIPCHK(h, hipStreamWaitEvent(h->stream, h->ev_in, 0));
    return 0;
}
int order_out(jmid_ctx* h, int mem) {
    if (mem != JMID_MEM_DEVICE || h->chained) return 0;
    HIPCHK(h, hipEventRecord(h->ev_out, h->stream));
    HIPCHK(h, hipStreamWaitEvent(h->caller_stream, h->ev_out, 0));
    return 0;
}

int check_ready(jmid_ctx* h) {
    if (!h) return JMID_EINVAL;
    if (!h->finalized) return fail(h, JMID_ENOWEIGHT, "jmid_finalize_weights has not been called");
    if (h->beta.empty() || !h->thyp) return fail(h, JMID_EINVAL, "jmid_set_ddim_table has not been called");
    return 0;
}

int upload_noise_ids(jmid_ctx* h, const uint32_t* ids, int E) {
    if (!h->ev_ids) HIPCHK(h, hipEventCreateWithFlags(&h->ev_ids, hipEventDisableTiming));
    if (E > h->noise_ids_cap) {
        HIPCHK(h, hipStreamSynchronize(h->stream));
        if (h->noise_ids) HIPCHK(h, hipFree(h->noise_ids));
        if (h->noise_ids_pin) HIPCHK(h, hipHostFree(h->noise_ids_pin));
        h->noise_ids = h->noise_ids_pin = nullptr;
        h->noise_ids_cap = 0;
        const int cap = std::max(E, 64);
        if (hipMalloc((void**)&h->noise_ids, (size_t)cap * sizeof(unsigned)) != hipSuccess ||
            hipHostMalloc((void**)&h->noise_ids_pin, (size_t)cap * sizeof(unsigned), hipHostMallocDefault) != hipSuccess)
            return fail(h, JMID_ENOMEM, "episode id buffer allocation failed");
        h->noise_ids_cap = cap;
    } else {
        HIPCHK(h, hipEventSynchronize(h->ev_ids));
    }
    std::memcpy(h->noise_ids_pin, ids, (size_t)E * sizeof(unsigned));
    HIPCHK(h, hipMemcpyAsync(h->noise_ids, h->noise_ids_pin, (size_t)E * sizeof(unsigned), hipMemcpyHostToDevice, h->stream));
    HIPCHK(h, hipEventRecord(h->ev_ids, h->stream));
    return 0;
}

int fill_noise(jmid_ctx* h, uint64_t seed, const unsigned* ids_dev, int E, size_t n, int draw, float* out, unsigned* words, hipStream_t stream) {
    NoiseArgs g{};
    g.ids = ids_dev; g.out = out; g.words = words;
    g.n = n; g.E = E;
    g.key0 = (unsigned)(seed & 0xffffffffull); g.key1 = (unsigned)(seed >> 32);
    g.draw = (unsigned)draw;
    HIPCHK(h, launch_noise(g, stream));
    return 0;
}

int run_network(jmid_ctx* h, int E, int A, int K, int T, const float* x_in, const float* ctx, const float* p0, float dt,
                int precision, int single_step, float* vel_out, float* pos_out, float* e_out, int mem,
                const float* z_in, const SeedArgs* seeded) {
    if (int rc = check_ready(h)) return rc;
    if (E <= 0 || A <= 0 || K <= 0 || T <= 0) return fail(h, JMID_EINVAL, "E, A, K, T must be positive");
    if (T > kPeMaxLen) return fail(h, JMID_EINVAL, "T exceeds the positional-encoding table (max_len=24, diffusion.py:116-118)");
    if (precision != JMID_PREC_F32 && precision != JMID_PREC_F16X3 && precision != JMID_PREC_F16X2 && precision != JMID_PREC_F16MX)
        return fail(h, JMID_EINVAL, "precision must be JMID_PREC_F32, JMID_PREC_F16X3, JMID_PREC_F16X2 or JMID_PREC_F16MX (JMID_PREC_F16 is not built)");
    h->mx = precision == JMID_PREC_F16MX;
    h->x2 = precision == JMID_PREC_F16X2 || h->mx;
    if (precision != JMID_PREC_F32 && !h->weights_in_half_range && ++h->erange_calls)
        return fail(h, JMID_ERANGE, "a weight exceeds the fp16 range: use JMID_PREC_F32");
    if ((!x_in && !seeded) || !ctx) return fail(h, JMID_EINVAL, "null input");
    if (seeded && !seeded->ids) return fail(h, JMID_EINVAL, "null episode_ids");
    if (seeded && !noise_fits((unsigned long long)K * A * T * 2)) return fail(h, JMID_EINVAL, "K * A * T exceeds the noise addressing");
    if (pos_out && !p0) return fail(h, JMID_EINVAL, "pos_out requested without p0");
    h->last_pos = nullptr;
    if (single_step < 0 && h->ddpm && !z_in && !seeded) return fail(h, JMID_EINVAL, "DDPM table installed: use jmid_denoise_ddpm (needs z)");
    if (single_step < 0 && !h->ddpm && z_in) return fail(h, JMID_EINVAL, "jmid_denoise_ddpm needs jmid_set_ddpm_table");
    HIPCHK(h, hipSetDevice(h->device));
    if (int rc = order_in(h, mem)) return rc;
    const size_t R = (size_t)E * K * A, M = R * T, EA = (size_t)E * A;
    const std::vector<int> chunk_sizes = plan_chunks(h, E, K * A * T);
    std::vector<int> chunk_start(chunk_sizes.size(), 0);
    for (size_t i = 1; i < chunk_sizes.size(); ++i) chunk_start[i] = chunk_start[i - 1] + chunk_sizes[i - 1];
    const int Ec = *std::max_element(chunk_sizes.begin(), chunk_sizes.end());
    const size_t Mc = (size_t)Ec * K * A * T;
    int ns_call = 1;
    if (h->net_kind == JMID_NET_JMID && precision != JMID_PREC_F32 && h->d / h->nhead == 128) {
        const int S = K * A * T;
        const int c_auto = auto_chunk(h, E, S);
        ns_call = attn_pick_nsplit(((S + 127) / 128) * h->nhead * (E >= 2 ? (one_launch_shape(h, (long)E * S) ? E : (c_auto + 1) / 2) : 1), S);
        if (h->tune.attn_nsplit > 0) ns_call = std::min(h->tune.attn_nsplit, (S + 31) / 32);
    }
    const int nchunks = (int)chunk_sizes.size();
    const int lanes = single_step < 0 ? std::max(1, std::min(h->lanes, nchunks)) : 1;
    const bool z_fill = seeded && h->ddpm && single_step < 0;
    size_t io_off;
    {
        Carver c(nullptr);
        c.take(M * 2);
        c.take(EA * h->ctx_dim);
        c.take(EA * h->hl.total);
        c.take(EA * 2);
        c.take(M * 2);
        if (z_in && mem == JMID_MEM_HOST) c.take(M * 2 * h->beta.size());
        if (z_fill) c.take((size_t)lanes * Mc * 2);
        io_off = c.off;
    }
    const SeqGeom sg_full = seq_geom(h, Ec, A, K, T);
    CallFacts facts;
    facts.small_now = lanes == 1 || h->tune.small_lanes == 1 ? 1 : h->tune.small_lanes == 2 ? 2 : 0;
    facts.one_chunk = nchunks == 1 && h->tune.graph != 1;
    facts.attn_nsplit = ns_call;
    const int n_steps = (int)h->beta.size();
    facts.qkv0_steps = single_step < 0 ? qkv0_table_steps(n_steps, Ec, A, h->d) : 1;
    std::vector<StepPlan> plans;
    std::vector<int> chunk_plan;
    for (int ec : chunk_sizes) {
        size_t j = 0;
        while (j < plans.size() && plans[j].Ec != ec) ++j;
        if (j == plans.size()) plans.push_back(plan_step(h, ec, A, K, T, precision, facts));
        chunk_plan.push_back((int)j);
    }
    const size_t qkv0_rows = plans[0].qkv0 ? (size_t)facts.qkv0_steps * Ec * A * 3 : 0;
    const size_t lane_floats = step_ws_floats(h, Mc, precision, sg_full, ns_call, nullptr, nullptr, qkv0_rows);
    const size_t need = io_off + lanes * lane_floats;
    if (int rc = ensure_arena(h, need)) return rc;
    Carver c(h->arena);
    float* x_cur = c.take(M * 2);
    float* ctx_d = c.take(EA * h->ctx_dim);
    float* hyp = c.take(EA * h->hl.total);
    float* p0_d = c.take(EA * 2);
    float* stage = c.take(M * 2);
    const float* z_use = z_in;
    if (z_in && mem == JMID_MEM_HOST) {
        float* zd = c.take(M * 2 * h->beta.size());
        HIPCHK(h, hipMemcpyAsync(zd, z_in, M * 2 * h->beta.size() * sizeof(float), hipMemcpyHostToDevice, h->stream));
        z_use = zd;
    }
    float* z_lane = z_fill ? c.take((size_t)lanes * Mc * 2) : nullptr;
    StepBuffers sbs[jmid_ctx::kMaxLanes];
    for (int l = 0; l < lanes; ++l) step_ws_floats(h, Mc, precision, sg_full, ns_call, &sbs[l], h->arena + io_off + l * lane_floats, qkv0_rows);
    const StepBuffers& sb = sbs[0];
    if (precision != JMID_PREC_F32) {
        HIPCHK(h, hipMemsetAsync(h->range_flag, 0, sizeof(int), h->stream));
        for (int l = 0; l < lanes; ++l) HIPCHK(h, hipMemsetAsync(sbs[l].ln_xchg, 0, kLnxWords * sizeof(unsigned), h->stream));
        for (int l = 0; l < lanes; ++l)
            if (sbs[l].Vth && sg_full.Spad != sg_full.S) {
                HIPCHK(h, hipMemsetAsync(sbs[l].Vth, 0, sbs[l].vt_elems * sizeof(half_t), h->stream));
                HIPCHK(h, hipMemsetAsync(sbs[l].Vtl, 0, sbs[l].vt_elems * sizeof(half_t), h->stream));
            }
    }

    const hipMemcpyKind kin = mem == JMID_MEM_HOST ? hipMemcpyHostToDevice : hipMemcpyDeviceToDevice;
    const hipMemcpyKind kout = mem == JMID_MEM_HOST ? hipMemcpyDeviceToHost : hipMemcpyDeviceToDevice;
    if (seeded) {
        if (int rc = upload_noise_ids(h, seeded->ids, E)) return rc;
        if (int rc = fill_noise(h, seeded->seed, h->noise_ids, E, (size_t)K * A * T * 2, 0, x_cur, nullptr, h->stream)) return rc;
    } else {
        HIPCHK(h, hipMemcpyAsync(x_cur, x_in, M * 2 * sizeof(float), kin, h->stream));
    }
    const float* ctx_use = ctx;
    if (mem == JMID_MEM_HOST) {
        HIPCHK(h, hipMemcpyAsync(ctx_d, ctx, EA * h->ctx_dim * sizeof(float), kin, h->stream));
        ctx_use = ctx_d;
    }
    const float* p0_use = p0;
    if (p0 && mem == JMID_MEM_HOST) {
        HIPCHK(h, hipMemcpyAsync(p0_d, p0, EA * 2 * sizeof(float), kin, h->stream));
        p0_use = p0_d;
    }
    {
        GemmArgs g{};
        g.A = ctx_use; g.lda = h->ctx_dim; g.W = h->Whyp; g.ldw = h->ctx_dim; g.bias = h->bhyp; g.C = hyp;
        g.ldc = h->hl.total; g.M = (int)EA; g.N = h->hl.total; g.K = h->ctx_dim;
        if (int rc = run_gemm<EPI_BIAS>(h, KC_HYPER, g)) return rc;
    }
    if (lanes > 1) {
        HIPCHK(h, hipEventRecord(h->ev_fork, h->stream));
        for (int l = 1; l < lanes; ++l) HIPCHK(h, hipStreamWaitEvent(h->lane_stream[l - 1], h->ev_fork, 0));
    }
    jmid_ctx::LoopGraph* lg = nullptr;
    bool capturing = false;
    if (single_step < 0 && lanes == 1 && nchunks == 1 && !h->prof_mask && !z_use && !h->ddpm && h->tune.graph == 1 &&
        h->tune.bystander_lds == 0) {
        const std::string key = std::to_string(E) + "," + std::to_string(A) + "," + std::to_string(K) + "," + std::to_string(T) +
                                "," + std::to_string(precision);
        lg = &h->graphs[key];
        if (lg->exec && lg->arena != h->arena) {
            hipGraphExecDestroy(lg->exec);
            lg->exec = nullptr;
        }
        if (lg->exec) {
            HIPCHK(h, hipGraphLaunch(lg->exec, h->stream));
            ++h->graph_replays;
        } else if (lg->warm) {
            HIPCHK(h, hipStreamBeginCapture(h->stream, hipStreamCaptureModeThreadLocal));
            capturing = true;
        }
    }
    for (int c0 = 0; c0 < nchunks && !(lg && lg->exec); c0 += lanes) {
        if (single_step >= 0) {
            const int e0 = chunk_start[c0];
            float* eo = stage + (size_t)e0 * K * A * T * 2;
            if (int rc = net_step(h, plans[chunk_plan[c0]], sb, single_step, x_cur + (size_t)e0 * K * A * T * 2,
                                  hyp + (size_t)e0 * A * h->hl.total, eo))
                return rc;
            continue;
        }
        for (int i = 0; i < n_steps; ++i) {
            for (int l = 0; l < lanes; ++l) {
                if (c0 + l >= nchunks) break;
                const int el = chunk_start[c0 + l];
                float* xc = x_cur + (size_t)el * K * A * T * 2;
                const float* hc = hyp + (size_t)el * A * h->hl.total;
                const float* zc = z_use ? z_use + ((size_t)i * M + (size_t)el * K * A * T) * 2 : nullptr;
                if (l > 0) std::swap(h->stream, h->lane_stream[l - 1]);
                int rc = 0;
                if (z_fill && h->p_noise[i]) {
                    float* zl = z_lane + (size_t)l * Mc * 2;
                    rc = fill_noise(h, seeded->seed, h->noise_ids + el, chunk_sizes[c0 + l], (size_t)K * A * T * 2, i + 1, zl, nullptr, h->stream);
                    zc = zl;
                }
                const StepPlan& pl = plans[chunk_plan[c0 + l]];
                if (!rc && i == 0 && pl.qkv0 && pl.qkv0_steps > 1) rc = qkv0_build_table(h, pl, sbs[l], hc, 0, n_steps);
                if (!rc) rc = net_step(h, plans[chunk_plan[c0 + l]], sbs[l], i, xc, hc, nullptr, zc, h->tune.fuse_embed && i > 0,
                                        h->tune.fuse_embed && i + 1 < n_steps ? i + 1 : -1);
                if (l > 0) std::swap(h->stream, h->lane_stream[l - 1]);
                if (rc) {
                    if (capturing) {
                        hipGraph_t dead = nullptr;
                        (void)hipStreamEndCapture(h->stream, &dead);
                        if (dead) hipGraphDestroy(dead);
                    }
                    sync_lanes(h);
                    return rc;
                }
            }
        }
    }
    if (capturing) {
        hipGraph_t graph = nullptr;
        HIPCHK(h, hipStreamEndCapture(h->stream, &graph));
        hipError_t ge = hipGraphInstantiate(&lg->exec, graph, nullptr, nullptr, 0);
        hipGraphDestroy(graph);
        if (ge != hipSuccess) {
            lg->exec = nullptr;
            return fail(h, JMID_EHIP, std::string("hipGraphInstantiate: ") + hipGetErrorString(ge));
        }
        lg->arena = h->arena;
        HIPCHK(h, hipGraphLaunch(lg->exec, h->stream));
        ++h->graph_replays;
    } else if (lg && !lg->exec) {
        lg->warm = true;
    }
    for (int l = 1; l < lanes; ++l) {
        HIPCHK(h, hipEventRecord(h->ev_join[l - 1], h->lane_stream[l - 1]));
        HIPCHK(h, hipStreamWaitEvent(h->stream, h->ev_join[l - 1], 0));
    }
    if (single_step >= 0) {
        HIPCHK(h, hipMemcpyAsync(e_out, stage, M * 2 * sizeof(float), kout, h->stream));
    } else {
        if (vel_out) HIPCHK(h, hipMemcpyAsync(vel_out, x_cur, M * 2 * sizeof(float), kout, h->stream));
        if (p0_use) {
            {
                ProfScope ps(h, KC_INTEGRATE);
                const int n = (int)R * 2;
                hipLaunchKernelGGL(integrate_kernel, dim3((n + 255) / 256), dim3(256), 0, h->stream, x_cur, p0_use,
                                   stage, (int)R, T, A, K * A, dt);
                HIPCHK(h, hipGetLastError());
            }
            h->last_pos = stage;
            h->last_pos_dims[0] = E; h->last_pos_dims[1] = A; h->last_pos_dims[2] = K; h->last_pos_dims[3] = T;
            if (pos_out) HIPCHK(h, hipMemcpyAsync(pos_out, stage, M * 2 * sizeof(float), kout, h->stream));
        }
    }
    if (int rc = order_out(h, mem)) return rc;
    if (h->chained) return 0;
    if (precision != JMID_PREC_F32) {
        int flag = 0;
        HIPCHK(h, hipMemcpyAsync(&flag, h->range_flag, sizeof(int), hipMemcpyDeviceToHost, h->stream));
        HIPCHK(h, hipStreamSynchronize(h->stream));
        if (flag) return flagged_call(h, flag);
    } else if (mem == JMID_MEM_HOST) {
        HIPCHK(h, hipStreamSynchronize(h->stream));
    }
    return 0;
}


int flagged_call(jmid_ctx* h, int flag) {
    h->last_pos = nullptr;
    if (flag & 2) {
        h->lnx_off = true;
        ++h->lnx_timeouts;
        return fail(h, JMID_ETIMEOUT, "a workgroup of a one-launch GEMM + LayerNorm gave up waiting for its partners (not all workgroups of the launch "
                                      "were resident): this handle now runs the unfused kernels - repeat the call in the same precision");
    }
    ++h->erange_calls;
    return fail(h, JMID_ERANGE, "an activation left the fp16 range in JMID_PREC_F16X3 / F16X2 / F16MX: rerun with JMID_PREC_F32");
}

#ifdef JMID_DIAGNOSTICS
int dbg_qkv0(jmid_ctx* h, int E, int A, int K, int T, const float* x, const float* hyp, int hyp_width, int step, int precision, float* qkv, float* thyp_row) {
    if (int rc = check_ready(h)) return rc;
    if (!x || !hyp || !qkv || E <= 0 || A <= 0 || K <= 0 || T <= 0 || T > kPeMaxLen) return fail(h, JMID_EINVAL, "jmid_dbg_qkv0: bad arguments");
    if (hyp_width != h->hl.total) return fail(h, JMID_EINVAL, "jmid_dbg_qkv0: hyp rows must be " + std::to_string(h->hl.total) + " wide");
    if (h->net_kind != JMID_NET_JMID || (precision != JMID_PREC_F16X3 && precision != JMID_PREC_F16X2 && precision != JMID_PREC_F16MX))
        return fail(h, JMID_EINVAL, "jmid_dbg_qkv0: JMID in a split-fp16 mode only");
    if (step < 0 || step >= (int)h->beta.size()) return fail(h, JMID_EINVAL, "jmid_dbg_qkv0: step outside the step table");
    h->mx = precision == JMID_PREC_F16MX;
    h->x2 = precision == JMID_PREC_F16X2 || h->mx;
    HIPCHK(h, hipSetDevice(h->device));
    h->last_pos = nullptr;
    const size_t M = (size_t)E * K * A * T, EA = (size_t)E * A;
    const int d = h->d;
    CallFacts facts;
    const StepPlan p = plan_step(h, E, A, K, T, precision, facts);
    const size_t rows = p.qkv0 ? EA * 3 : 0;
    size_t io_off;
    {
        Carver c(nullptr);
        c.take(M * 2);
        c.take(EA * h->hl.total);
        c.take(M * 3 * d);
        io_off = c.off;
    }
    if (int rc = ensure_arena(h, io_off + step_ws_floats(h, M, precision, p.sg, 1, nullptr, nullptr, rows))) return rc;
    Carver c(h->arena);
    float* x_d = c.take(M * 2);
    float* hyp_d = c.take(EA * h->hl.total);
    float* out_d = c.take(M * 3 * d);
    StepBuffers sb;
    step_ws_floats(h, M, precision, p.sg, 1, &sb, h->arena + io_off, rows);
    HIPCHK(h, hipMemsetAsync(h->range_flag, 0, sizeof(int), h->stream));
    HIPCHK(h, hipMemsetAsync(sb.Vth, 0, sb.vt_elems * sizeof(half_t), h->stream));
    HIPCHK(h, hipMemsetAsync(sb.Vtl, 0, sb.vt_elems * sizeof(half_t), h->stream));
    HIPCHK(h, hipMemcpyAsync(x_d, x, M * 2 * sizeof(float), hipMemcpyHostToDevice, h->stream));
    HIPCHK(h, hipMemcpyAsync(hyp_d, hyp, EA * h->hl.total * sizeof(float), hipMemcpyHostToDevice, h->stream));
    if (int rc = run_embed(h, p, sb, x_d, hyp_d, h->thyp + (size_t)step * h->hl.total)) return rc;
    if (int rc = qkv_planes(h, p, sb, 0, step, x_d, hyp_d)) return rc;
    const LoImages im = lo_images(p, sb, d);
    QkvReadArgs ra{sb.Qh, sb.Ql, sb.Kh, sb.Kl, sb.Vth, sb.Vtl, im.q8l, im.k8l, out_d, M, d, p.hd, p.sg.S, p.sg.Spad, h->x2,
                   p.att_scale * 1.4426950408889634f};
    hipLaunchKernelGGL(qkv_planes_read_kernel, dim3(512), dim3(256), 0, h->stream, ra);
    HIPCHK(h, hipGetLastError());
    int flag = 0;
    HIPCHK(h, hipMemcpyAsync(&flag, h->range_flag, sizeof(int), hipMemcpyDeviceToHost, h->stream));
    HIPCHK(h, hipMemcpyAsync(qkv, out_d, M * 3 * d * sizeof(float), hipMemcpyDeviceToHost, h->stream));
    if (thyp_row)
        HIPCHK(h, hipMemcpyAsync(thyp_row, h->thyp + (size_t)step * h->hl.total, h->hl.total * sizeof(float), hipMemcpyDeviceToHost, h->stream));
    HIPCHK(h, hipStreamSynchronize(h->stream));
    if (flag) return flagged_call(h, flag);
    return 0;
}
#endif

int launch_episode_metrics(jmid_ctx* h, const float* pos, const float* gt, float* out, int E, int K, int A, int T) {
    ProfScope ps(h, KC_METRICS);
    hipLaunchKernelGGL(episode_metrics_kernel, dim3(E), dim3(256), 0, h->stream, pos, gt, out, K, A, T);
    HIPCHK(h, hipGetLastError());
    return 0;
}

}
```

safe-interactive-crowdnav_amd/csrc/launch_plan.hpp:

```cpp
#pragma once
#include "common.hpp"

namespace jmid {

enum GemmEpi { EPI_BIAS = 0, EPI_BIAS_RELU = 1, EPI_CSL = 2 };
enum GemmOut { OUT_F32 = 0, OUT_SPLIT = 1, OUT_QKV = 2, OUT_LNX = 4 };

struct CallFacts {
    int small_now = 1;
    int one_chunk = 1;
    int attn_nsplit = 1;
    int qkv0_steps = 1;
};

enum GemmMode { GM_X3 = 0, GM_X2 = 1, GM_MX = 2 };

enum GemmShape {
    GS_NONE = 0,
    GS_SMALL_64x64, GS_SMALL_64x128, GS_SMALL_64x128_TWO,
    GS_SMALL_64x64_TWO,
    GS_64, GS_128, GS_256x128, GS_256x256,
    GS_128x256, GS_256x256_NS3,
    GS_REG_64, GS_REG_128,
};
constexpr int gemm_shape_bm(GemmShape s) {
    return s == GS_256x128 || s == GS_256x256 || s == GS_256x256_NS3 ? 256 : s == GS_128 || s == GS_128x256 || s == GS_REG_128 ? 128 : 64;
}
constexpr int gemm_shape_bn(GemmShape s) {
    return s == GS_256x256 || s == GS_128x256 || s == GS_256x256_NS3 ? 256
           : s == GS_SMALL_64x64 || s == GS_SMALL_64x64_TWO || s == GS_64 || s == GS_REG_64 ? 64 : 128;
}
constexpr bool gemm_shape_small(GemmShape s) { return s >= GS_SMALL_64x64 && s <= GS_SMALL_64x64_TWO; }

constexpr bool gemm_shape_built(GemmMode mode, int epi, int out, GemmShape s) {
    switch (s) {
        case GS_SMALL_64x64: return true;
        case GS_SMALL_64x128: return out != OUT_LNX;
        case GS_SMALL_64x128_TWO: return out != OUT_LNX && mode != GM_X3;
        case GS_SMALL_64x64_TWO: return out == OUT_LNX && mode == GM_MX;
        case GS_64:
        case GS_128: return out != OUT_LNX;
        case GS_256x128: return out != OUT_LNX && !(mode == GM_MX && epi == EPI_CSL && out == OUT_F32);
        case GS_256x256: return out != OUT_LNX && epi != EPI_CSL;
        case GS_128x256:
        case GS_256x256_NS3: return out != OUT_LNX && epi != EPI_CSL && mode == GM_MX;
        case GS_REG_64:
        case GS_REG_128: return out != OUT_LNX && mode != GM_MX;
        default: return false;
    }
}

struct GemmPlan {
    GemmMode mode;
    GemmShape shape;
    int flags, group_tiles, abl;
};

constexpr int kLnxMaxTiles = 64;

inline GemmShape small_gemm_shape(GemmMode mode, int out, int M, int N, int K, const CallFacts& cf, const Tuning& t) {
    if (t.gemm_small == 1 || t.gemm_h_variant != 0 || !cf.small_now || K % 128 != 0) return GS_NONE;
    const long ntm = (M + 63) / 64;
    if (out == OUT_LNX) {
        if (cf.small_now != 1 || cf.one_chunk != 1 || t.small_lnx == 2 || ntm > kLnxMaxTiles) return GS_NONE;
        if (ntm * 8 <= t.cus) return GS_SMALL_64x64;
        return gemm_shape_built(mode, 0, out, GS_SMALL_64x64_TWO) && ntm * 8 <= 2L * t.cus && t.small_lnx2 != 2 ? GS_SMALL_64x64_TWO : GS_NONE;
    }
    if (N % 128 != 0) return GS_NONE;
    const bool two = gemm_shape_built(mode, 0, out, GS_SMALL_64x128_TWO) && ntm * (N / 128) <= 512;
    if (cf.small_now == 2) return two ? GS_SMALL_64x128_TWO : GS_NONE;
    if (ntm * (N / 64) <= 256) return GS_SMALL_64x64;
    if (ntm * (N / 128) <= 256) return GS_SMALL_64x128;
    return two && t.gemm_small != 2 ? GS_SMALL_64x128_TWO : GS_NONE;
}

inline GemmShape large_gemm_shape(GemmMode mode, int epi, int out, int M, int N, const Tuning& t) {
    const auto usable = [&](GemmShape s) { return gemm_shape_built(mode, epi, out, s) && N % gemm_shape_bn(s) == 0; };
    constexpr GemmShape forced[9] = {GS_NONE, GS_REG_64, GS_REG_128, GS_128, GS_256x128, GS_64, GS_256x256, GS_128x256, GS_256x256_NS3};
    const GemmShape f = forced[t.gemm_h_variant >= 0 && t.gemm_h_variant <= 8 ? t.gemm_h_variant : 0];
    if (f != GS_NONE && gemm_shape_built(mode, epi, out, f) && (gemm_shape_bn(f) != 256 || N % 256 == 0)) return f;
    const long mt256 = (M + 255) / 256, big = (long)((M + 127) / 128) * ((N + 127) / 128);
    if (big < 256) return GS_64;
    const auto eff = [](long nb) { return (double)nb / (double)(((nb + 255) / 256) * 256); };
    const long nb256 = mt256 * ((N + 127) / 128);
    const int rows = mode == GM_MX ? 7168 : 12288;
    if (usable(GS_256x256)) {
        const long nbq = mt256 * (N / 256);
        if ((nbq >= 256 && 1.2 * eff(nbq) >= eff(nb256)) || (nbq < 256 && M >= rows)) return GS_256x256;
    }
    if (gemm_shape_built(mode, epi, out, GS_256x128) && nb256 >= 256 && 1.2 * eff(nb256) >= eff(big)) return GS_256x128;
    return GS_128;
}

inline int gemm_flags(const Tuning& t, bool small) {
    const int csl = (t.csl_swap == 2 ? 0 : 4) | (t.csl_swap == 3 ? 8 : 0);
    if (small) return csl | (t.small_qk == 2 ? 16 : 0);
    return (t.vt_stage == 2 ? 0 : (t.vt_stage == 3 ? 1 : 3)) | csl | (t.h1_stage == 2 ? 0 : 16);
}

inline int small_pick_groups(int M, int N, int K, int ntn, double w_bytes_per_el, double a_bytes_per_el) {
    const double wb = (double)N * K * w_bytes_per_el, ab = (double)M * K * a_bytes_per_el;
    int best = 1;
    double best_bytes = 8.0 * wb + ab;
    for (int pn = 2; pn <= 8; pn *= 2) {
        if (ntn % pn != 0) break;
        const double bytes = 8.0 * wb / pn + pn * ab;
        if (bytes < best_bytes) {
            best = pn;
            best_bytes = bytes;
        }
    }
    return best;
}

inline GemmPlan plan_gemm(GemmMode want, int epi, int out, int M, int N, int K, const CallFacts& cf, const Tuning& t) {
    GemmPlan p{};
    const bool mx_ok = K % 64 == 0 && N % 128 == 0 && t.gemm_h_variant != 1 && t.gemm_h_variant != 2;
    p.mode = want == GM_MX && !mx_ok ? GM_X2 : want;
    p.abl = gemm_abl_bits(t);
    p.shape = small_gemm_shape(p.mode, out, M, N, K, cf, t);
    const bool small = p.shape != GS_NONE;
    if (!small && out != OUT_LNX) p.shape = large_gemm_shape(p.mode, epi, out, M, N, t);
    if (p.shape == GS_NONE) return p;
    p.flags = small || p.mode == GM_MX ? gemm_flags(t, small) : p.shape == GS_256x256 ? gemm_flags(t, false) & 3 : 0;
    const int ntn = N / gemm_shape_bn(p.shape);
    if (small) {
        const int pn = t.small_pn > 0 ? (ntn % t.small_pn == 0 ? t.small_pn : 1)
                                      : small_pick_groups(M, N, K, ntn, p.mode == GM_MX ? 3.0 : 4.0, p.mode == GM_X3 ? 4.0 : 2.0);
        p.group_tiles = ntn / pn;
    } else if (p.mode == GM_MX) {
        p.group_tiles = t.gemm_pn > 1 && ntn % t.gemm_pn == 0 ? ntn / t.gemm_pn : 0;
    } else if (p.shape == GS_256x128) {
        p.group_tiles = t.gemm_ng;
    }
    return p;
}

inline int plan_ln_rows(bool second_generation, int M, const Tuning& t) {
    if (second_generation) return t.ln_rows == 64 ? 64 : 128;
    const auto fill = [](long n) { return (double)n / (double)(((n + 255) / 256) * 256); };
    const long n128 = (M + 127) / 128, n64 = (M + 63) / 64;
    return t.ln_rows == 128 || (t.ln_rows == 0 && 1.04 * fill(n128) >= fill(n64)) ? 128 : 64;
}

struct AttnPlan {
    bool dma;
    bool p1, pf;
    bool old_softmax;
    bool one_wg;
    int prio;
    int abl;
    int bystander_lds;
    bool pack;
};
inline AttnPlan plan_attn(int head_dim, const Tuning& t) {
    AttnPlan p{};
    p.dma = head_dim == 128 && t.attn_h_variant != 1;
    p.p1 = t.attn_mx != 1;
    p.pf = t.attn_pf != 2;
    p.old_softmax = t.attn_sm == 2;
    p.one_wg = t.attn_one_wg != 0;
    p.prio = t.attn_prio;
    p.abl = attn_abl_bits(t);
    p.bystander_lds = t.bystander_lds;
    p.pack = t.attn_pack != 0;
    return p;
}

inline bool small_cmb_fits(const AttnPlan& ap, int nsplit, int x2, const Tuning& t) {
    return t.small_cmb != 2 && ap.dma && nsplit > 1 && nsplit <= 8 && x2;
}

}
```

safe-interactive-crowdnav_amd/engine.py:

```python
from __future__ import annotations

import ctypes as C
from typing import Dict, Optional, Tuple, Union

import numpy as np

from . import _lib
from ._lib import JmidError
from .schedule import VarianceSchedule, ddim_steps, ddpm_steps
from .weights import JMIDWeights

try:
    import torch
except Exception:
    torch = None

ArrayLike = Union[np.ndarray, "torch.Tensor"]

ERANGE_EVENTS: list = []
TIMEOUT_EVENTS: list = []


def _is_cuda(t) -> bool:
    return torch is not None and isinstance(t, torch.Tensor) and t.is_cuda
# ... 300 lines not shown
            if K is None or T is None:
                raise ValueError("a seeded call needs K and T")
            return int(seeded[1].size), A, int(K), int(T), "_seeded", (seeded[0], C.c_void_p(seeded[1].ctypes.data)), seeded[1]
        x_T = np.asarray(x_T)
        if x_T.ndim != 4 or x_T.shape[-1] != 2:
            raise ValueError("expected x_T [E, K*A, T, 2]")
        E, KA, T, _ = (int(v) for v in x_T.shape)
        if KA % A != 0:
            raise ValueError(f"x_T has {KA} rows per episode: not a multiple of the scene's {A} in-cluster pedestrians")
        bx = _Buf(x_T, False)
        return E, A, KA // A, T, "", (bx.ptr,), bx

    def predict_scene(self, x_T: Optional[np.ndarray], k: int, dt: float = 0.25, precision: str = "f32", seed: Optional[int] = None,
                      episode_ids=None, K: Optional[int] = None, T: Optional[int] = None):
        import math
        E, A, K, T, sfx, nz, _keep = self._scene_noise(x_T, seed, episode_ids, K, T)
        k = int(k)
        fn = getattr(self._lib, "jmid_predict_scene" + sfx)
        if k < K:
            bw = np.ascontiguousarray(torch.exp(torch.linspace(math.log(0.01), math.log(0.1), steps=T)).numpy())
            sel = np.empty((E, A, k, T, 2), dtype=np.float32)
            lw = np.empty((E, A, k), dtype=np.float32)
            self._compute(fn, self._h, E, A, K, T, k, *nz, float(dt), _lib.PRECISIONS[precision],
                          C.c_void_p(bw.ctypes.data), C.c_void_p(sel.ctypes.data), C.c_void_p(lw.ctypes.data), None)
            return sel, lw
        pos = np.empty((E, K, A, T, 2), dtype=np.float32)
        self._compute(fn, self._h, E, A, K, T, k, *nz, float(dt), _lib.PRECISIONS[precision], None, None, None,
                      C.c_void_p(pos.ctypes.data))
        return pos, None

    def build_scene_stamped(self, stamps: np.ndarray, human_xy: np.ndarray, robot_xy: np.ndarray, time_step: float,
                            horizon: Optional[int] = None, force_all_in_cluster: bool = False,
                            n_frames: Optional[np.ndarray] = None) -> Dict[str, np.ndarray]:
        from .scene import HistoryTooShortError
        st = np.ascontiguousarray(stamps, dtype=np.float64)
        hum = np.ascontiguousarray(human_xy, dtype=np.float64)
        rob = np.ascontiguousarray(robot_xy, dtype=np.float64)
        single = hum.ndim == 3
        if single:
            st, hum, rob = st[None], hum[None], rob[None]
        if hum.ndim != 4 or hum.shape[-1] != 2 or rob.shape != (hum.shape[0], hum.shape[1], 2) or st.shape != hum.shape[:2]:
            raise ValueError("expected stamps [E, R], human_xy [E, R, N, 2] and robot_xy [E, R, 2] (or one scene without the episode axis)")
        E, R, N, _ = (int(v) for v in hum.shape)
        nf = None
        if n_frames is not None:
            nf = np.ascontiguousarray(np.atleast_1d(n_frames), dtype=np.int32)
            if nf.shape != (E,):
                raise ValueError("n_frames must hold one count per episode")
        inc = np.empty((E, N), dtype=np.uint8)
        rin = np.empty(E, dtype=np.uint8)
        n_in = np.empty(E, dtype=np.int32)
        n_grid = np.empty(E, dtype=np.int32)
        cv = np.empty((E, N, int(horizon), 2), dtype=np.float64) if horizon is not None else None
        rc = self._lib.jmid_build_scene_stamped(self._h, E, N, R, C.c_void_p(st.ctypes.data), C.c_void_p(hum.ctypes.data), C.c_void_p(rob.ctypes.data),
                                                C.c_void_p(nf.ctypes.data) if nf is not None else None, float(time_step),
                                                int(horizon) if horizon is not None else 0, int(bool(force_all_in_cluster)),
                                                C.c_void_p(inc.ctypes.data), C.c_void_p(rin.ctypes.data), C.c_void_p(n_in.ctypes.data),
                                                C.c_void_p(n_grid.ctypes.data), C.c_void_p(cv.ctypes.data) if cv is not None else None, _lib.MEM_HOST)
        if rc == -7:
            err = HistoryTooShortError(self._lib.jmid_last_error(self._h).decode())
            err.n_grid = n_grid[0] if single else n_grid
            raise err
        self._check(rc)
        self._scene_shape, self._scene_n_in = (E, N, self.hist_len, single), n_in
        out = {"in_cluster": inc.astype(bool), "robot_in_cluster": rin.astype(bool), "n_in": n_in, "n_grid": n_grid, "cv": cv}
        return {k: (v[0] if single and v is not None else v) for k, v in out.items()}

    def scene_frames(self) -> Dict[str, np.ndarray]:
        shape = getattr(self, "_scene_shape", None)
        E, N, F, single = shape if shape is not None else (0, 0, self.hist_len, False)
        out = {"human_xy": np.empty((E, F, N, 2), np.float64), "robot_xy": np.empty((E, F, 2), np.float64),
               "pose_now": np.empty((E, N, 2), np.float64)}
        self._check(self._lib.jmid_scene_get_frames(self._h, *[C.c_void_p(a.ctypes.data) for a in out.values()], _lib.MEM_HOST))
        return {k: v[0] for k, v in out.items()} if single else out

    def forecast_scene(self, x_T: Optional[np.ndarray], k: int, dt: float = 0.25, precision: str = "f32", seed: Optional[int] = None,
                       episode_ids=None, K: Optional[int] = None, T: Optional[int] = None):
        import math
        E, A, K, T, sfx, nz, _keep = self._scene_noise(x_T, seed, episode_ids, K, T)
        k = int(k)
        fn = getattr(self._lib, "jmid_forecast_scene" + sfx)
        shape = getattr(self, "_scene_shape", None)
        N, single = (shape[1], shape[3]) if shape is not None else (1, False)
        bw = None
        if k < K:
            bw = np.ascontiguousarray(torch.exp(torch.linspace(math.log(0.01), math.log(0.1), steps=T)).numpy())
        fc = np.empty((E, N, max(k, 0), T + 1, 2), dtype=np.float64)
        lw = np.empty((E, N, max(k, 0)), dtype=np.float64)
        self._compute(fn, self._h, E, A, K, T, k, *nz, float(dt), _lib.PRECISIONS[precision],
                      C.c_void_p(bw.ctypes.data) if bw is not None else None, C.c_void_p(fc.ctypes.data), C.c_void_p(lw.ctypes.data))
        return (fc[0], lw[0]) if single else (fc, lw)

    def net_eval(self, x: ArrayLike, ctx: ArrayLike, step_idx: int = 0, precision: str = "f32"):
        dev = _is_cuda(x)
        E, A, K, T = self._shapes(x, ctx)
        bx, bc = _Buf(x, dev), _Buf(ctx, dev)
        if dev:
            out = torch.empty(tuple(x.shape), dtype=torch.float32, device=x.device)
            optr = C.c_void_p(out.data_ptr())
        else:
            out = np.empty(tuple(x.shape), dtype=np.float32)
            optr = C.c_void_p(out.ctypes.data)
        self._compute(self._lib.jmid_net_eval, self._h, E, A, K, T, int(step_idx), bx.ptr, bc.ptr,
                                            _lib.PRECISIONS[precision], optr,
                                            self._mem(dev))
        return out

    def episode_metrics(self, pos: ArrayLike, gt: ArrayLike) -> ArrayLike:
        dev = _is_cuda(pos)
        E, K, A, T, _ = (int(v) for v in pos.shape)
        if tuple(gt.shape) != (E, A, T, 2):
            raise ValueError("gt must be [E, A, T, 2]")
        bp, bg = _Buf(pos, dev), _Buf(gt, dev)
        if dev:
            out = torch.empty((E, 4), dtype=torch.float32, device=pos.device)
            optr = C.c_void_p(out.data_ptr())
        else:
            out = np.empty((E, 4), dtype=np.float32)
            optr = C.c_void_p(out.ctypes.data)
        self._check(self._lib.jmid_episode_metrics(self._h, E, A, K, T, bp.ptr, bg.ptr, optr,
                                                   self._mem(dev)))
        return out

    def eval_statistics(self, pos: Optional[ArrayLike], gt: ArrayLike, dims: Optional[Tuple[int, int, int, int]] = None):
        dev = _is_cuda(gt)
        if pos is None:
            if dims is None:
                raise ValueError("pos=None needs dims=(E, A, K, T) of the preceding denoise call")
            E, A, K, T = (int(v) for v in dims)
            bp = None
        else:
            if _is_cuda(pos) != dev:
                raise TypeError("pos and gt must both be CUDA/HIP tensors or both host arrays")
            E, K, A, T, _ = (int(v) for v in pos.shape)
            bp = _Buf(pos, dev)
        if tuple(gt.shape) != (E, A, T, 2):
            raise ValueError("gt must be [E, A, T, 2]")
        bg = _Buf(gt, dev)
        if dev:
            agent = torch.empty((E, A, 10), dtype=torch.float32, device=gt.device)
            scene = torch.empty((E, 6), dtype=torch.float32, device=gt.device)
            ptrs = (C.c_void_p(agent.data_ptr()), C.c_void_p(scene.data_ptr()))
        else:
            agent = np.empty((E, A, 10), dtype=np.float32)
            scene = np.empty((E, 6), dtype=np.float32)
            ptrs = (C.c_void_p(agent.ctypes.data), C.c_void_p(scene.ctypes.data))
        self._check(self._lib.jmid_eval_statistics(self._h, E, A, K, T, bp.ptr if bp is not None else None, bg.ptr, *ptrs,
                                                   self._mem(dev)))
        return agent, scene

    def eval_statistics_masked(self, pos: Optional[ArrayLike], gt: ArrayLike, interp_future: ArrayLike,
                               interp_history: Optional[ArrayLike] = None, cutoffs=(2, 5, 8),
                               dims: Optional[Tuple[int, int, int, int]] = None):
        dev = _is_cuda(gt)
        if pos is None:
            if dims is None:
                raise ValueError("pos=None needs dims=(E, A, K, T) of the preceding denoise call")
            E, A, K, T = (int(v) for v in dims)
            bp = None
        else:
            if _is_cuda(pos) != dev:
                raise TypeError("pos and gt must both be CUDA/HIP tensors or both host arrays")
            E, K, A, T, _ = (int(v) for v in pos.shape)
            bp = _Buf(pos, dev)
        if tuple(gt.shape) != (E, A, T, 2):
            raise ValueError("gt must be [E, A, T, 2]")
        if tuple(interp_future.shape) != (E, A, T):
            raise ValueError("interp_future must be [E, A, T]")
        if interp_history is not None and tuple(interp_history.shape[:2]) != (E, A):
            raise ValueError("interp_history must be [E, A, F]")
        if _is_cuda(interp_future) != dev or (interp_history is not None and _is_cuda(interp_history) != dev):
            raise TypeError("the masks must live where gt lives")
        cuts = (C.c_int * max(len(cutoffs), 1))(*[int(c) for c in cutoffs])
        n_cut = len(cutoffs)
        bg = _Buf(gt, dev)
        if dev:
            fut = (interp_future != 0).to(torch.uint8).contiguous()
            skip = (interp_history != 0).reshape(E, A, -1).all(dim=-1).to(torch.uint8).contiguous() if interp_history is not None else None
            agent = torch.empty((E, A, 12), dtype=torch.float32, device=gt.device)
            cut = torch.empty((E, A, n_cut, 5), dtype=torch.float32, device=gt.device)
            scene = torch.empty((E, 6), dtype=torch.float32, device=gt.device)
            ptr = lambda t: C.c_void_p(t.data_ptr()) if t is not None and t.numel() else None
        else:
            to_np = lambda m: m.detach().cpu().numpy() if torch is not None and isinstance(m, torch.Tensor) else np.asarray(m)
            fut = np.ascontiguousarray(to_np(interp_future) != 0, dtype=np.uint8)
            skip = (np.ascontiguousarray((to_np(interp_history) != 0).reshape(E, A, -1).all(axis=-1), dtype=np.uint8)
                    if interp_history is not None else None)
            agent = np.empty((E, A, 12), dtype=np.float32)
            cut = np.empty((E, A, n_cut, 5), dtype=np.float32)
            scene = np.empty((E, 6), dtype=np.float32)
            ptr = lambda t: C.c_void_p(t.ctypes.data) if t is not None and t.size else None
        self._check(self._lib.jmid_eval_statistics_masked(self._h, E, A, K, T, bp.ptr if bp is not None else None, bg.ptr, ptr(fut),
                                                          ptr(skip), n_cut, cuts, ptr(agent), ptr(cut), ptr(scene), self._mem(dev)))
        return agent, cut, scene

    def collision_statistics(self, pos: Optional[ArrayLike], threshold: float = 0.2,
                             dims: Optional[Tuple[int, int, int, int]] = None, pairs: bool = False, agents: bool = True):
        if pos is None:
            if dims is None:
                raise ValueError("pos=None needs dims=(E, A, K, T) of the preceding denoise call")
            E, A, K, T = (int(v) for v in dims)
            dev, bp = False, None
        else:
            dev = _is_cuda(pos)
            E, K, A, T, _ = (int(v) for v in pos.shape)
            bp = _Buf(pos, dev)
        shapes = (((E, K, A * (A - 1) // 2), np.float32) if pairs else None, ((E, K, A), np.uint8) if agents else None,
                  ((E, K, 4), np.float32), ((E, 5), np.float32))
        if dev:
            outs = [torch.empty(s[0], dtype=torch.uint8 if s[1] is np.uint8 else torch.float32, device=pos.device) if s else None
                    for s in shapes]
            ptrs = [C.c_void_p(o.data_ptr()) if o is not None else None for o in outs]
        else:
            outs = [np.empty(s[0], dtype=s[1]) if s else None for s in shapes]
            ptrs = [C.c_void_p(o.ctypes.data) if o is not None else None for o in outs]
        self._check(self._lib.jmid_collision_statistics(self._h, E, A, K, T, bp.ptr if bp is not None else None, float(threshold),
                                                        *ptrs, self._mem(dev)))
        return tuple(outs)

    def kernel_classes(self):
        return [self._lib.jmid_kernel_class_name(i).decode() for i in range(self._lib.jmid_kernel_class_count())]

    def profile_enable(self, classes=None) -> None:
        names = self.kernel_classes()
        mask = 0
        for i, n in enumerate(names):
            if classes is None or n in classes:
                mask |= 1 << i
        self._check(self._lib.jmid_profile_enable(self._h, mask))

    def profile_disable(self) -> None:
        self._check(self._lib.jmid_profile_enable(self._h, 0))

    def profile_reset(self) -> None:
        self._check(self._lib.jmid_profile_reset(self._h))

    def profile_get(self) -> Dict[str, Tuple[int, float]]:
        out = {}
        for i, n in enumerate(self.kernel_classes()):
            cnt, ms = C.c_int64(0), C.c_double(0.0)
            self._check(self._lib.jmid_profile_get(self._h, i, C.byref(cnt), C.byref(ms)))
            out[n] = (int(cnt.value), float(ms.value))
        return out

    def dbg_gemm(self, A: np.ndarray, Wt: np.ndarray, bias: Optional[np.ndarray], relu: bool = False,
                 precision: str = "f32") -> np.ndarray:
        A = np.ascontiguousarray(A, np.float32)
        Wt = np.ascontiguousarray(Wt, np.float32)
        M, K = A.shape
        N = Wt.shape[0]
        out = np.empty((M, N), np.float32)
        b = np.ascontiguousarray(bias, np.float32) if bias is not None else None
        self._check(self._lib.jmid_dbg_gemm(self._h, M, N, K, C.c_void_p(A.ctypes.data), C.c_void_p(Wt.ctypes.data),
                                            C.c_void_p(b.ctypes.data) if b is not None else None, int(relu),
                                            _lib.PRECISIONS[precision], C.c_void_p(out.ctypes.data)))
        return out

    def dbg_attention(self, qkv: np.ndarray, nseq: int, S: int, precision: str = "f32") -> np.ndarray:
        qkv = np.ascontiguousarray(qkv, np.float32)
        d = 2 * self.dims.ctx_dim
        assert qkv.shape == (nseq * S, 3 * d)
        out = np.empty((nseq * S, d), np.float32)
        self._check(self._lib.jmid_dbg_attention(self._h, nseq, S, C.c_void_p(qkv.ctypes.data),
                                                 _lib.PRECISIONS[precision], C.c_void_p(out.ctypes.data)))
        return out

    def dbg_gemm_ln_mx(self, A: np.ndarray, Wt: np.ndarray, bias, gamma, beta, X: np.ndarray, fused) -> np.ndarray:
        A = np.ascontiguousarray(A, np.float32)
        Wt = np.ascontiguousarray(Wt, np.float32)
        X = np.array(X, np.float32, order="C", copy=True)
        v = [np.ascontiguousarray(t, np.float32) for t in (bias, gamma, beta)]
        M, K = A.shape
        assert Wt.shape == (512, K) and X.shape == (M, 512)
        self._check(self._lib.jmid_dbg_gemm_ln_mx(self._h, M, K, C.c_void_p(A.ctypes.data), C.c_void_p(Wt.ctypes.data),
                                                  *[C.c_void_p(t.ctypes.data) for t in v], C.c_void_p(X.ctypes.data),
                                                  int(fused)))
        return X

    def dbg_add_layernorm(self, X: np.ndarray, Y: np.ndarray, gamma: np.ndarray, beta: np.ndarray) -> np.ndarray:
        X = np.array(X, np.float32, order="C", copy=True)
        Y = np.ascontiguousarray(Y, np.float32)
        g = np.ascontiguousarray(gamma, np.float32)
        b = np.ascontiguousarray(beta, np.float32)
        M, d = X.shape
        self._check(self._lib.jmid_dbg_add_layernorm(self._h, M, d, C.c_void_p(X.ctypes.data),
                                                     C.c_void_p(Y.ctypes.data), C.c_void_p(g.ctypes.data),
                                                     C.c_void_p(b.ctypes.data)))
        return X

    def dbg_qkv0(self, x: np.ndarray, hyp: np.ndarray, step: int, dims: Tuple[int, int, int, int], precision: str = "f16mx"):
        E, A, K, T = (int(v) for v in dims)
        x = np.ascontiguousarray(x, np.float32)
        hyp = np.ascontiguousarray(hyp, np.float32)
        M, d = E * K * A * T, 2 * self.dims.ctx_dim
        width = self.hyper_width()
        if x.shape != (M, 2) or hyp.shape != (E * A, width):
            raise ValueError(f"expected x [{M}, 2] and hyp [{E * A}, {width}]")
        out = np.empty((M, 3 * d), np.float32)
        thyp = np.empty((width,), np.float32)
        self._check(self._lib.jmid_dbg_qkv0(self._h, E, A, K, T, C.c_void_p(x.ctypes.data), C.c_void_p(hyp.ctypes.data), width, int(step),
                                            _lib.PRECISIONS[precision], C.c_void_p(out.ctypes.data), C.c_void_p(thyp.ctypes.data)))
        return out, thyp

    def hyper_width(self) -> int:
        return 2 * self.dims.d_model + 2 * self.dims.d_mid + 2 * self.dims.d_low + 4
```

Before: 47860 traj/s.

## Fold concat3/concat4/linear tail into per-episode effective 2xd map

The network tail (concat3 GEMM, concat4 GEMM, final linear) has no nonlinearity between the layers, and its hyper-conditioned gates and biases depend only on episode/agent and step. It is collapsed algebraically into one effective d->2 weight matrix and bias per (step, episode-agent), precomputed in a table kernel. A fused wave-per-row dot-product kernel then applies that map and runs the DDIM/DDPM update and next-step embedding. This removes two tensor-core GEMMs and the Y3/Y4 intermediates per step, in exchange for a table precompute and a change in numerical rounding relative to the split-fp16 GEMM path.

Result: faster. 49240 traj/s (median of 6 runs) (+2.9%).

```diff
diff --git a/include/jmid_hip.h b/include/jmid_hip.h
--- a/include/jmid_hip.h
+++ b/include/jmid_hip.h
@@ -131,6 +131,8 @@
 int jmid_dbg_gemm_plan(int mode, int epi, int out, int M, int N, int K, int small_now, int one_chunk, const int* knobs, int* plan);
 int jmid_dbg_qkv0(jmid_handle_t h, int E, int A, int K, int T, const float* x, const float* hyp, int hyp_width, int step, int precision,
                   float* qkv, float* thyp_row);
+int jmid_dbg_tail(jmid_handle_t h, int E, int A, int K, int T, const float* X, const float* hyp, int hyp_width, int step, int precision,
+                  float* e, float* thyp_row);
 int jmid_dbg_noise_words(jmid_handle_t h, uint64_t seed, int E, int rows, int T, const uint32_t* episode_ids, int draw, uint32_t* out, int mem);
 #endif
 
diff --git a/safe-interactive-crowdnav_amd/_lib.py b/safe-interactive-crowdnav_amd/_lib.py
--- a/safe-interactive-crowdnav_amd/_lib.py
+++ b/safe-interactive-crowdnav_amd/_lib.py
@@ -87,6 +87,7 @@
     "jmid_dbg_plan_chunks_mode": (C.c_int, [C.c_int, C.c_int, C.c_int, C.c_int, C.c_int, C.c_int, C.c_int, C.POINTER(C.c_int), C.c_int]),
     "jmid_dbg_gemm_plan": (C.c_int, [C.c_int] * 8 + [C.POINTER(C.c_int), C.POINTER(C.c_int)]),
     "jmid_dbg_qkv0": (C.c_int, [Handle, C.c_int, C.c_int, C.c_int, C.c_int, C.c_void_p, C.c_void_p, C.c_int, C.c_int, C.c_int, C.c_void_p, C.c_void_p]),
+    "jmid_dbg_tail": (C.c_int, [Handle, C.c_int, C.c_int, C.c_int, C.c_int, C.c_void_p, C.c_void_p, C.c_int, C.c_int, C.c_int, C.c_void_p, C.c_void_p]),
     "jmid_dbg_noise_words": (C.c_int, [Handle, C.c_uint64, C.c_int, C.c_int, C.c_int, C.c_void_p, C.c_int, C.c_void_p, C.c_int]),
 }
 
diff --git a/safe-interactive-crowdnav_amd/csrc/common.hpp b/safe-interactive-crowdnav_amd/csrc/common.hpp
--- a/safe-interactive-crowdnav_amd/csrc/common.hpp
+++ b/safe-interactive-crowdnav_amd/csrc/common.hpp
@@ -130,6 +130,7 @@
     int small_qk = 0;
     int small_pn = 0;
     int qkv0 = 0;
+    int tail_fold = 0;
     int attn_abl = 0;
     int gemm_abl = 0;
 };
diff --git a/safe-interactive-crowdnav_amd/csrc/jmid_abi.hip b/safe-interactive-crowdnav_amd/csrc/jmid_abi.hip
--- a/safe-interactive-crowdnav_amd/csrc/jmid_abi.hip
+++ b/safe-interactive-crowdnav_amd/csrc/jmid_abi.hip
@@ -956,6 +956,7 @@
         {"small_qk", &Tuning::small_qk, 0, 2},
         {"small_pn", &Tuning::small_pn, 0, 8},
         {"qkv0", &Tuning::qkv0, 0, 2},
+        {"tail_fold", &Tuning::tail_fold, 0, 2},
 #ifdef JMID_ABLATIONS
         {"attn_abl", &Tuning::attn_abl, 0, 1 << 30},
         {"gemm_abl", &Tuning::gemm_abl, 0, 1 << 30},
diff --git a/safe-interactive-crowdnav_amd/csrc/jmid_ctx.hpp b/safe-interactive-crowdnav_amd/csrc/jmid_ctx.hpp
--- a/safe-interactive-crowdnav_amd/csrc/jmid_ctx.hpp
+++ b/safe-interactive-crowdnav_amd/csrc/jmid_ctx.hpp
@@ -26,6 +26,7 @@
 #include "launch_plan.hpp"
 #include "noise.hpp"
 #include "qkv0.hpp"
+#include "tail_fold.hpp"
 #include "scene.hpp"
 #include "frames.hpp"
 
@@ -252,6 +253,7 @@
 int launch_episode_metrics(jmid_ctx* h, const float* pos, const float* gt, float* out, int E, int K, int A, int T);
 #ifdef JMID_DIAGNOSTICS
 int dbg_qkv0(jmid_ctx* h, int E, int A, int K, int T, const float* x, const float* hyp, int hyp_width, int step, int precision, float* qkv, float* thyp_row);
+int dbg_tail(jmid_ctx* h, int E, int A, int K, int T, const float* X, const float* hyp, int hyp_width, int step, int precision, float* e, float* thyp_row);
 #endif
 int noise_entry(jmid_ctx* h, const char* who, uint64_t seed, int E, int rows, int T, const uint32_t* episode_ids, int draw, float* out,
                 unsigned* words, int mem);
diff --git a/safe-interactive-crowdnav_amd/csrc/jmid_diag.hip b/safe-interactive-crowdnav_amd/csrc/jmid_diag.hip
--- a/safe-interactive-crowdnav_amd/csrc/jmid_diag.hip
+++ b/safe-interactive-crowdnav_amd/csrc/jmid_diag.hip
@@ -283,6 +283,12 @@
     return dbg_qkv0(h, E, A, K, T, x, hyp, hyp_width, step, precision, qkv, thyp_row);
 }
 
+int jmid_dbg_tail(jmid_handle_t h, int E, int A, int K, int T, const float* X, const float* hyp, int hyp_width, int step, int precision,
+                  float* e, float* thyp_row) {
+    if (!h) return JMID_EINVAL;
+    return dbg_tail(h, E, A, K, T, X, hyp, hyp_width, step, precision, e, thyp_row);
+}
+
 int jmid_dbg_noise_words(jmid_handle_t h, uint64_t seed, int E, int rows, int T, const uint32_t* episode_ids, int draw, uint32_t* out, int mem) {
     return noise_entry(h, "jmid_dbg_noise_words", seed, E, rows, T, episode_ids, draw, nullptr, out, mem);
 }
diff --git a/safe-interactive-crowdnav_amd/csrc/jmid_planner.hip b/safe-interactive-crowdnav_amd/csrc/jmid_planner.hip
--- a/safe-interactive-crowdnav_amd/csrc/jmid_planner.hip
+++ b/safe-interactive-crowdnav_amd/csrc/jmid_planner.hip
@@ -37,6 +37,7 @@
     size_t vt_elems;
     float *Opart, *MLpart;
     float *coef, *uvc;
+    float *weff, *beff;
     unsigned long long* ln_xchg;
 };
 
@@ -54,13 +55,13 @@
 }
 
 size_t step_ws_floats(const jmid_ctx* h, size_t Mc, int precision, const SeqGeom& sg, int nsplit, StepBuffers* sb,
-                      char* base, size_t qkv0_rows) {
+                      char* base, size_t qkv0_rows, size_t tail_rows) {
     Carver c(base);
     StepBuffers s{};
     s.X = c.take(Mc * h->d);
     s.Y = c.take((Mc + 63) / 64 * 64 * h->d);
     s.ln_xchg = reinterpret_cast<unsigned long long*>(c.take(kLnxWords));
-    s.Y4 = c.take(Mc * h->dlow);
+    if (!tail_rows) s.Y4 = c.take(Mc * h->dlow);
     if (precision == JMID_PREC_F32) {
         s.QKV = c.take(Mc * 3 * h->d);
         s.ATT = c.take(Mc * h->d);
@@ -94,8 +95,13 @@
         s.Al = take_half(c, blk_plane_elems(Mc, h->d));
         s.H1h = take_half(c, blk_plane_elems(Mc, h->ff));
         s.H1l = take_half(c, blk_plane_elems(Mc, h->ff));
-        s.Y3h = take_half(c, blk_plane_elems(Mc, h->dmid));
-        s.Y3l = take_half(c, blk_plane_elems(Mc, h->dmid));
+        if (tail_rows) {
+            s.weff = c.take(tail_rows * 2 * h->d);
+            s.beff = c.take(tail_rows * 2);
+        } else {
+            s.Y3h = take_half(c, blk_plane_elems(Mc, h->dmid));
+            s.Y3l = take_half(c, blk_plane_elems(Mc, h->dmid));
+        }
     }
     if (sb) *sb = s;
     return c.off;
@@ -134,6 +140,8 @@
     int R;
     bool qkv0;
     int qkv0_steps;
+    bool tail_fold;
+    int tail_steps;
     bool split, mxv2, joint;
     RowMap rm;
     SeqGeom sg;
@@ -167,6 +175,8 @@
     p.attn = plan_attn(p.hd, t);
     p.qkv0 = p.split && p.joint && t.qkv0 != 1 && d % 32 == 0;
     p.qkv0_steps = cf.qkv0_steps;
+    p.tail_fold = p.split && t.tail_fold != 1 && d % 8 == 0 && d <= kTailMaxD && h->dmid <= kTailMaxMid && h->dlow <= kTailMaxLow;
+    p.tail_steps = cf.tail_steps;
     if (p.split) {
         const auto gemm = [&](int epi, int out, int N, int K) { return plan_gemm(gemm_mode(h), epi, out, p.M, N, K, cf, t); };
         p.in_proj = gemm(EPI_BIAS, p.joint ? OUT_QKV : OUT_F32, 3 * d, d);
@@ -242,6 +252,23 @@
     g.M = nsteps * p.R * 3; g.N = 3 * d; g.K = d;
     if (h->tune.qkv0 == 2) HIPCHK(h, (launch_gemm_f32<EPI_BIAS, false>(g, h->stream)));
     else HIPCHK(h, (launch_gemm_f32<EPI_BIAS, true>(g, h->stream)));
+    return 0;
+}
+
+constexpr size_t kTailTableMaxBytes = size_t(128) << 20;
+int tail_table_steps(int steps, int Ec, int A, int d) {
+    const size_t bytes = (size_t)steps * Ec * A * (2 * d + 2) * sizeof(float);
+    return bytes <= kTailTableMaxBytes ? steps : 1;
+}
+
+int tail_build_table(jmid_ctx* h, const StepPlan& p, const StepBuffers& sb, const float* hyp_chunk, int step0, int nsteps) {
+    const WeightTable& wt = h->wt;
+    ProfScope ps(h, KC_HYPER);
+    TailTableArgs ta{wt.concat3.W, wt.concat3.bias, wt.concat4.W, wt.concat4.bias, wt.linear.W, wt.linear.bias,
+                     hyp_chunk, h->thyp + (size_t)step0 * h->hl.total, sb.weff, sb.beff,
+                     nsteps, p.R, h->d, h->dmid, h->dlow, h->hl.total,
+                     h->hl.g3, h->hl.b3, h->hl.g4, h->hl.b4, h->hl.go, h->hl.bo, h->range_flag};
+    HIPCHK(h, launch_tail_fold_table(ta, h->stream));
     return 0;
 }
 
@@ -306,6 +333,85 @@
         HIPCHK(h, hipGetLastError());
     }
     return 0;
+}
+
+OutArgs sampler_args(const jmid_ctx* h, const StepPlan& p, const StepBuffers& sb, int step_idx, float* x_chunk, const float* hyp_chunk,
+                     float* e_out, const float* z_chunk) {
+    OutArgs oa{sb.Y4, h->wt.linear.W, h->wt.linear.bias, hyp_chunk, h->thyp + (size_t)step_idx * h->hl.total, x_chunk, e_out,
+               p.M, h->dlow, h->hl.total, h->hl.go, h->hl.bo,
+               h->c_e[step_idx], h->c_x[step_idx], h->n_x[step_idx], h->n_e[step_idx], p.rm,
+               nullptr, 0, 0.f, 0.f, 0.f};
+    if (h->ddpm && !e_out) {
+        oa.ddpm = 1;
+        oa.z = h->p_noise[step_idx] ? z_chunk : nullptr;
+        oa.c0 = h->p_c0[step_idx];
+        oa.c1 = h->p_c1[step_idx];
+        oa.sigma = h->p_sigma[step_idx];
+    }
+    return oa;
+}
+
+int folded_tail(jmid_ctx* h, const StepPlan& p, const StepBuffers& sb, int step_idx, float* x_chunk, const float* hyp_chunk,
+                float* e_out, const float* z_chunk, int next_step) {
+    const int M = p.M, d = h->d;
+    if (p.tail_steps <= 1)
+        if (int rc = tail_build_table(h, p, sb, hyp_chunk, step_idx, 1)) return rc;
+    const size_t at = p.tail_steps <= 1 ? 0 : (size_t)step_idx * p.R;
+    const TailFoldArgs fa{sb.Xh, sb.Xl, sb.weff + at * 2 * d, sb.beff + at * 2, d};
+    const OutArgs oa = sampler_args(h, p, sb, step_idx, x_chunk, hyp_chunk, e_out, z_chunk);
+    const bool embed_next = next_step >= 0 && !e_out;
+    const EmbedArgs en = embed_next ? embed_args(h, p, sb, x_chunk, hyp_chunk, h->thyp + (size_t)next_step * h->hl.total) : EmbedArgs{};
+    const bool lo = !h->x2;
+    ProfScope ps(h, KC_OUT_DDIM);
+    const auto launch = [&](auto* kernel, int waves, auto... tpw) {
+        hipLaunchKernelGGL(kernel, dim3((waves + 3) / 4), dim3(256), bystander_lds(h->tune.bystander_lds, kernel), h->stream, fa, oa, en, tpw...);
+    };
+    const auto pick = [&](auto embed, auto with_lo) {
+        constexpr bool EN = decltype(embed)::value, LO = decltype(with_lo)::value;
+        if (p.out_tpw) launch(tail_fold_traj_kernel<EN, LO>, M / p.out_tpw, p.out_tpw);
+        else launch(tail_fold_kernel<EN, LO>, M);
+    };
+    if (embed_next && lo) pick(std::true_type{}, std::true_type{});
+    else if (embed_next) pick(std::true_type{}, std::false_type{});
+    else if (lo) pick(std::false_type{}, std::true_type{});
+    else pick(std::false_type{}, std::false_type{});
+    HIPCHK(h, hipGetLastError());
+    return 0;
+}
+
+int output_stage(jmid_ctx* h, const StepPlan& p, const StepBuffers& sb, int step_idx, float* x_chunk, const float* hyp_chunk,
+                 float* e_out, const float* z_chunk, int next_step) {
+    const int M = p.M;
+    ProfScope ps(h, KC_OUT_DDIM);
+    const OutArgs oa = sampler_args(h, p, sb, step_idx, x_chunk, hyp_chunk, e_out, z_chunk);
+    const bool embed_next = next_step >= 0 && !e_out;
+    const EmbedArgs en = embed_next ? embed_args(h, p, sb, x_chunk, hyp_chunk, h->thyp + (size_t)next_step * h->hl.total) : EmbedArgs{};
+    const auto launch = [&](auto* kernel, int waves, auto... tpw) {
+        hipLaunchKernelGGL(kernel, dim3((waves + 3) / 4), dim3(256), bystander_lds(h->tune.bystander_lds, kernel), h->stream, oa, en, tpw...);
+    };
+    if (p.out_tpw && embed_next) launch(out_ddim_traj_kernel<true>, M / p.out_tpw, p.out_tpw);
+    else if (p.out_tpw) launch(out_ddim_traj_kernel<false>, M / p.out_tpw, p.out_tpw);
+    else if (embed_next) launch(out_ddim_kernel<true>, M);
+    else launch(out_ddim_kernel<false>, M);
+    HIPCHK(h, hipGetLastError());
+    return 0;
+}
+
+int net_tail(jmid_ctx* h, const StepPlan& p, const StepBuffers& sb, int step_idx, float* x_chunk, const float* hyp_chunk,
+             float* e_out, const float* z_chunk, int next_step) {
+    if (p.tail_fold) return folded_tail(h, p, sb, step_idx, x_chunk, hyp_chunk, e_out, z_chunk, next_step);
+    const int M = p.M, d = h->d;
+    const WeightTable& wt = h->wt;
+    const float* thyp = h->thyp + (size_t)step_idx * h->hl.total;
+    GemmHArgs g = gemm_h_args(h, p.rm, M, sb.Xh, sb.Xl, wt.concat3, h->dmid, d);
+    g.hyp = hyp_chunk; g.thyp = thyp; g.hyp_ld = h->hl.total;
+    g.Chi = sb.Y3h; g.Clo = sb.Y3l; g.ldc = h->dmid; g.goff = h->hl.g3; g.boff = h->hl.b3;
+    if (int rc = (run_gemm_h<EPI_CSL, OUT_SPLIT>(h, KC_GEMM_TAIL, g, p.concat3))) return rc;
+    g = gemm_h_args(h, p.rm, M, sb.Y3h, sb.Y3l, wt.concat4, h->dlow, h->dmid);
+    g.hyp = hyp_chunk; g.thyp = thyp; g.hyp_ld = h->hl.total;
+    g.C = sb.Y4; g.ldc = h->dlow; g.goff = h->hl.g4; g.boff = h->hl.b4;
+    if (int rc = (run_gemm_h<EPI_CSL, OUT_F32>(h, KC_GEMM_TAIL, g, p.concat4))) return rc;
+    return output_stage(h, p, sb, step_idx, x_chunk, hyp_chunk, e_out, z_chunk, next_step);
 }
 
 int net_step(jmid_ctx* h, const StepPlan& p, const StepBuffers& sb, int step_idx, float* x_chunk, const float* hyp_chunk,
@@ -365,40 +471,9 @@
             if (int rc = (run_gemm_h<EPI_BIAS_RELU, OUT_SPLIT>(h, KC_GEMM_FF1, g, p.linear1))) return rc;
             if (int rc = residual_block(h, p, p.linear2, sb, sb.H1h, sb.H1l, ff, w.linear2, w.norm2, KC_GEMM_FF2, l + 1 == h->tf_layer)) return rc;
         }
-        GemmHArgs g = gemm_h_args(h, rm, M, sb.Xh, sb.Xl, wt.concat3, h->dmid, d);
-        g.hyp = hyp_chunk; g.thyp = thyp; g.hyp_ld = h->hl.total;
-        g.Chi = sb.Y3h; g.Clo = sb.Y3l; g.ldc = h->dmid; g.goff = h->hl.g3; g.boff = h->hl.b3;
-        if (int rc = (run_gemm_h<EPI_CSL, OUT_SPLIT>(h, KC_GEMM_TAIL, g, p.concat3))) return rc;
-        g = gemm_h_args(h, rm, M, sb.Y3h, sb.Y3l, wt.concat4, h->dlow, h->dmid);
-        g.hyp = hyp_chunk; g.thyp = thyp; g.hyp_ld = h->hl.total;
-        g.C = sb.Y4; g.ldc = h->dlow; g.goff = h->hl.g4; g.boff = h->hl.b4;
-        if (int rc = (run_gemm_h<EPI_CSL, OUT_F32>(h, KC_GEMM_TAIL, g, p.concat4))) return rc;
-    }
-    {
-        ProfScope ps(h, KC_OUT_DDIM);
-        OutArgs oa{sb.Y4, wt.linear.W, wt.linear.bias, hyp_chunk, thyp, x_chunk, e_out,
-                   M, h->dlow, h->hl.total, h->hl.go, h->hl.bo,
-                   h->c_e[step_idx], h->c_x[step_idx], h->n_x[step_idx], h->n_e[step_idx], rm,
-                   nullptr, 0, 0.f, 0.f, 0.f};
-        if (h->ddpm && !e_out) {
-            oa.ddpm = 1;
-            oa.z = h->p_noise[step_idx] ? z_chunk : nullptr;
-            oa.c0 = h->p_c0[step_idx];
-            oa.c1 = h->p_c1[step_idx];
-            oa.sigma = h->p_sigma[step_idx];
-        }
-        const bool embed_next = next_step >= 0 && !e_out;
-        const EmbedArgs en = embed_next ? embed_args(h, p, sb, x_chunk, hyp_chunk, h->thyp + (size_t)next_step * h->hl.total) : EmbedArgs{};
-        const auto launch = [&](auto* kernel, int waves, auto... tpw) {
-            hipLaunchKernelGGL(kernel, dim3((waves + 3) / 4), dim3(256), bystander_lds(h->tune.bystander_lds, kernel), h->stream, oa, en, tpw...);
-        };
-        if (p.out_tpw && embed_next) launch(out_ddim_traj_kernel<true>, M / p.out_tpw, p.out_tpw);
-        else if (p.out_tpw) launch(out_ddim_traj_kernel<false>, M / p.out_tpw, p.out_tpw);
-        else if (embed_next) launch(out_ddim_kernel<true>, M);
-        else launch(out_ddim_kernel<false>, M);
-        HIPCHK(h, hipGetLastError());
-    }
-    return 0;
+        return net_tail(h, p, sb, step_idx, x_chunk, hyp_chunk, e_out, z_chunk, next_step);
+    }
+    return output_stage(h, p, sb, step_idx, x_chunk, hyp_chunk, e_out, z_chunk, next_step);
 }
 
 int auto_chunk(const jmid_ctx* h, int E, int tokens_per_episode) {
@@ -549,6 +624,7 @@
     facts.attn_nsplit = ns_call;
     const int n_steps = (int)h->beta.size();
     facts.qkv0_steps = single_step < 0 ? qkv0_table_steps(n_steps, Ec, A, h->d) : 1;
+    facts.tail_steps = single_step < 0 && h->tune.tail_fold != 2 ? tail_table_steps(n_steps, Ec, A, h->d) : 1;
     std::vector<StepPlan> plans;
     std::vector<int> chunk_plan;
     for (int ec : chunk_sizes) {
@@ -558,7 +634,8 @@
         chunk_plan.push_back((int)j);
     }
     const size_t qkv0_rows = plans[0].qkv0 ? (size_t)facts.qkv0_steps * Ec * A * 3 : 0;
-    const size_t lane_floats = step_ws_floats(h, Mc, precision, sg_full, ns_call, nullptr, nullptr, qkv0_rows);
+    const size_t tail_rows = plans[0].tail_fold ? (size_t)facts.tail_steps * Ec * A : 0;
+    const size_t lane_floats = step_ws_floats(h, Mc, precision, sg_full, ns_call, nullptr, nullptr, qkv0_rows, tail_rows);
     const size_t need = io_off + lanes * lane_floats;
     if (int rc = ensure_arena(h, need)) return rc;
     Carver c(h->arena);
@@ -575,7 +652,7 @@
     }
     float* z_lane = z_fill ? c.take((size_t)lanes * Mc * 2) : nullptr;
     StepBuffers sbs[jmid_ctx::kMaxLanes];
-    for (int l = 0; l < lanes; ++l) step_ws_floats(h, Mc, precision, sg_full, ns_call, &sbs[l], h->arena + io_off + l * lane_floats, qkv0_rows);
+    for (int l = 0; l < lanes; ++l) step_ws_floats(h, Mc, precision, sg_full, ns_call, &sbs[l], h->arena + io_off + l * lane_floats, qkv0_rows, tail_rows);
     const StepBuffers& sb = sbs[0];
     if (precision != JMID_PREC_F32) {
         HIPCHK(h, hipMemsetAsync(h->range_flag, 0, sizeof(int), h->stream));
@@ -659,6 +736,7 @@
                 }
                 const StepPlan& pl = plans[chunk_plan[c0 + l]];
                 if (!rc && i == 0 && pl.qkv0 && pl.qkv0_steps > 1) rc = qkv0_build_table(h, pl, sbs[l], hc, 0, n_steps);
+                if (!rc && i == 0 && pl.tail_fold && pl.tail_steps > 1) rc = tail_build_table(h, pl, sbs[l], hc, 0, n_steps);
                 if (!rc) rc = net_step(h, plans[chunk_plan[c0 + l]], sbs[l], i, xc, hc, nullptr, zc, h->tune.fuse_embed && i > 0,
                                         h->tune.fuse_embed && i + 1 < n_steps ? i + 1 : -1);
                 if (l > 0) std::swap(h->stream, h->lane_stream[l - 1]);
@@ -761,13 +839,13 @@
         c.take(M * 3 * d);
         io_off = c.off;
     }
-    if (int rc = ensure_arena(h, io_off + step_ws_floats(h, M, precision, p.sg, 1, nullptr, nullptr, rows))) return rc;
+    if (int rc = ensure_arena(h, io_off + step_ws_floats(h, M, precision, p.sg, 1, nullptr, nullptr, rows, 0))) return rc;
     Carver c(h->arena);
     float* x_d = c.take(M * 2);
     float* hyp_d = c.take(EA * h->hl.total);
     float* out_d = c.take(M * 3 * d);
     StepBuffers sb;
-    step_ws_floats(h, M, precision, p.sg, 1, &sb, h->arena + io_off, rows);
+    step_ws_floats(h, M, precision, p.sg, 1, &sb, h->arena + io_off, rows, 0);
     HIPCHK(h, hipMemsetAsync(h->range_flag, 0, sizeof(int), h->stream));
     HIPCHK(h, hipMemsetAsync(sb.Vth, 0, sb.vt_elems * sizeof(half_t), h->stream));
     HIPCHK(h, hipMemsetAsync(sb.Vtl, 0, sb.vt_elems * sizeof(half_t), h->stream));
@@ -789,6 +867,55 @@
     if (flag) return flagged_call(h, flag);
     return 0;
 }
+
+int dbg_tail(jmid_ctx* h, int E, int A, int K, int T, const float* X, const float* hyp, int hyp_width, int step, int precision, float* e, float* thyp_row) {
+    if (int rc = check_ready(h)) return rc;
+    if (!X || !hyp || !e || E <= 0 || A <= 0 || K <= 0 || T <= 0 || T > kPeMaxLen) return fail(h, JMID_EINVAL, "jmid_dbg_tail: bad arguments");
+    if (hyp_width != h->hl.total) return fail(h, JMID_EINVAL, "jmid_dbg_tail: hyp rows must be " + std::to_string(h->hl.total) + " wide");
+    if (precision != JMID_PREC_F16X3 && precision != JMID_PREC_F16X2 && precision != JMID_PREC_F16MX)
+        return fail(h, JMID_EINVAL, "jmid_dbg_tail: a split-fp16 mode only");
+    if (step < 0 || step >= (int)h->beta.size()) return fail(h, JMID_EINVAL, "jmid_dbg_tail: step outside the step table");
+    h->mx = precision == JMID_PREC_F16MX;
+    h->x2 = precision == JMID_PREC_F16X2 || h->mx;
+    HIPCHK(h, hipSetDevice(h->device));
+    h->last_pos = nullptr;
+    const size_t M = (size_t)E * K * A * T, EA = (size_t)E * A;
+    const int d = h->d;
+    CallFacts facts;
+    const StepPlan p = plan_step(h, E, A, K, T, precision, facts);
+    const size_t rows = p.tail_fold ? EA : 0;
+    size_t io_off;
+    {
+        Carver c(nullptr);
+        c.take(M * d);
+        c.take(EA * h->hl.total);
+        c.take(M * 2);
+        io_off = c.off;
+    }
+    if (int rc = ensure_arena(h, io_off + step_ws_floats(h, M, precision, p.sg, 1, nullptr, nullptr, 0, rows))) return rc;
+    Carver c(h->arena);
+    float* X_d = c.take(M * d);
+    float* hyp_d = c.take(EA * h->hl.total);
+    float* e_d = c.take(M * 2);
+    StepBuffers sb;
+    step_ws_floats(h, M, precision, p.sg, 1, &sb, h->arena + io_off, 0, rows);
+    HIPCHK(h, hipMemsetAsync(h->range_flag, 0, sizeof(int), h->stream));
+    HIPCHK(h, hipMemcpyAsync(X_d, X, M * d * sizeof(float), hipMemcpyHostToDevice, h->stream));
+    HIPCHK(h, hipMemcpyAsync(hyp_d, hyp, EA * h->hl.total * sizeof(float), hipMemcpyHostToDevice, h->stream));
+    HIPCHK(h, hipMemsetAsync(sb.Xh, 0, blk_plane_elems(M, d) * sizeof(half_t), h->stream));
+    HIPCHK(h, hipMemsetAsync(sb.Xl, 0, blk_plane_elems(M, d) * sizeof(half_t), h->stream));
+    hipLaunchKernelGGL(tail_split_rows_kernel, dim3(512), dim3(256), 0, h->stream, X_d, sb.Xh, h->x2 ? nullptr : sb.Xl, (int)M, d);
+    HIPCHK(h, hipGetLastError());
+    if (int rc = net_tail(h, p, sb, step, nullptr, hyp_d, e_d, nullptr, -1)) return rc;
+    int flag = 0;
+    HIPCHK(h, hipMemcpyAsync(&flag, h->range_flag, sizeof(int), hipMemcpyDeviceToHost, h->stream));
+    HIPCHK(h, hipMemcpyAsync(e, e_d, M * 2 * sizeof(float), hipMemcpyDeviceToHost, h->stream));
+    if (thyp_row)
+        HIPCHK(h, hipMemcpyAsync(thyp_row, h->thyp + (size_t)step * h->hl.total, h->hl.total * sizeof(float), hipMemcpyDeviceToHost, h->stream));
+    HIPCHK(h, hipStreamSynchronize(h->stream));
+    if (flag) return flagged_call(h, flag);
+    return 0;
+}
 #endif
 
 int launch_episode_metrics(jmid_ctx* h, const float* pos, const float* gt, float* out, int E, int K, int A, int T) {
diff --git a/safe-interactive-crowdnav_amd/csrc/launch_plan.hpp b/safe-interactive-crowdnav_amd/csrc/launch_plan.hpp
--- a/safe-interactive-crowdnav_amd/csrc/launch_plan.hpp
+++ b/safe-interactive-crowdnav_amd/csrc/launch_plan.hpp
@@ -11,6 +11,7 @@
     int one_chunk = 1;
     int attn_nsplit = 1;
     int qkv0_steps = 1;
+    int tail_steps = 1;
 };
 
 enum GemmMode { GM_X3 = 0, GM_X2 = 1, GM_MX = 2 };
diff --git a/safe-interactive-crowdnav_amd/csrc/tail_fold.hpp b/safe-interactive-crowdnav_amd/csrc/tail_fold.hpp
--- /dev/null
+++ b/safe-interactive-crowdnav_amd/csrc/tail_fold.hpp
@@ -0,0 +1,321 @@
+#pragma once
+#include <cfloat>
+
+#include "common.hpp"
+#include "elementwise.hpp"
+
+namespace jmid {
+
+constexpr int kTailG = 8;
+constexpr int kTailMaxD = 512, kTailMaxMid = 256, kTailMaxLow = 128;
+
+struct TailTableArgs {
+    const float *W3, *b3;
+    const float *W4, *b4;
+    const float *Wo, *bo;
+    const float* hyp;
+    const float* thyp;
+    float* weff;
+    float* beff;
+    int steps, R, d, dmid, dlow, hyp_ld;
+    int g3, b3o, g4, b4o, go, boo;
+    int* range_flag;
+};
+
+static __global__ __launch_bounds__(256) void tail_fold_table_kernel(TailTableArgs a) {
+    constexpr int G2 = 2 * kTailG;
+    __shared__ __attribute__((aligned(16))) float s_v[kTailMaxLow][G2];
+    __shared__ __attribute__((aligned(16))) float s_q[kTailMaxMid][G2];
+    __shared__ __attribute__((aligned(16))) float s_u[kTailMaxMid][G2];
+    __shared__ float s_t4[kTailG][kTailMaxLow];
+    __shared__ float s_t3[kTailG][kTailMaxMid];
+    const int tid = threadIdx.x;
+    const long pairs = (long)a.steps * a.R;
+    const long p0 = (long)blockIdx.x * kTailG;
+    const auto hrow = [&](int g) { return a.hyp + (size_t)((p0 + g < pairs ? p0 + g : pairs - 1) % a.R) * a.hyp_ld; };
+    const auto trow = [&](int g) { return a.thyp + (size_t)((p0 + g < pairs ? p0 + g : pairs - 1) / a.R) * a.hyp_ld; };
+    bool bad = false;
+
+    for (int id = tid; id < kTailG * a.dlow; id += 256) {
+        const int g = id / a.dlow, c = id - g * a.dlow;
+        const float *hr = hrow(g), *th = trow(g);
+        const float g4 = sigmoidf_(hr[a.g4 + c] + th[a.g4 + c]);
+        s_t4[g][c] = g4 * a.b4[c] + (hr[a.b4o + c] + th[a.b4o + c]);
+#pragma unroll
+        for (int o = 0; o < 2; ++o) {
+            const float go = sigmoidf_(hr[a.go + o] + th[a.go + o]);
+            s_v[c][2 * g + o] = go * a.Wo[o * a.dlow + c] * g4;
+        }
+    }
+    __syncthreads();
+
+    for (int j = tid; j < a.dmid; j += 256) {
+        float acc[G2];
+#pragma unroll
+        for (int k = 0; k < G2; ++k) acc[k] = 0.f;
+        for (int c0 = 0; c0 < a.dlow; c0 += 32) {
+            float part[G2];
+#pragma unroll
+            for (int k = 0; k < G2; ++k) part[k] = 0.f;
+            const int c1 = c0 + 32 < a.dlow ? c0 + 32 : a.dlow;
+#pragma unroll 8
+            for (int c = c0; c < c1; ++c) {
+                const float w = a.W4[(size_t)c * a.dmid + j];
+#pragma unroll
+                for (int k4 = 0; k4 < G2; k4 += 4) {
+                    const f32x4 v = *reinterpret_cast<const f32x4*>(&s_v[c][k4]);
+#pragma unroll
+                    for (int e = 0; e < 4; ++e) part[k4 + e] = fmaf(v[e], w, part[k4 + e]);
+                }
+            }
+#pragma unroll
+            for (int k = 0; k < G2; ++k) acc[k] += part[k];
+        }
+        const float b3 = a.b3[j];
+        float u[G2];
+#pragma unroll
+        for (int g = 0; g < kTailG; ++g) {
+            const float *hr = hrow(g), *th = trow(g);
+            const float g3 = sigmoidf_(hr[a.g3 + j] + th[a.g3 + j]);
+            s_t3[g][j] = g3 * b3 + (hr[a.b3o + j] + th[a.b3o + j]);
+            u[2 * g] = acc[2 * g] * g3;
+            u[2 * g + 1] = acc[2 * g + 1] * g3;
+        }
+#pragma unroll
+        for (int k4 = 0; k4 < G2; k4 += 4) {
+            *reinterpret_cast<f32x4*>(&s_q[j][k4]) = f32x4{acc[k4], acc[k4 + 1], acc[k4 + 2], acc[k4 + 3]};
+            *reinterpret_cast<f32x4*>(&s_u[j][k4]) = f32x4{u[k4], u[k4 + 1], u[k4 + 2], u[k4 + 3]};
+        }
+    }
+    __syncthreads();
+
+    if (tid < G2 && p0 + (tid >> 1) < pairs) {
+        const int g = tid >> 1, o = tid & 1;
+        float sj = 0.f;
+        for (int j0 = 0; j0 < a.dmid; j0 += 32) {
+            float part = 0.f;
+            const int j1 = j0 + 32 < a.dmid ? j0 + 32 : a.dmid;
+            for (int j = j0; j < j1; ++j) part = fmaf(s_q[j][tid], s_t3[g][j], part);
+            sj += part;
+        }
+        float sc = 0.f;
+        for (int c0 = 0; c0 < a.dlow; c0 += 32) {
+            float part = 0.f;
+            const int c1 = c0 + 32 < a.dlow ? c0 + 32 : a.dlow;
+            for (int c = c0; c < c1; ++c) part = fmaf(a.Wo[o * a.dlow + c], s_t4[g][c], part);
+            sc += part;
+        }
+        const float *hr = hrow(g), *th = trow(g);
+        const float go = sigmoidf_(hr[a.go + o] + th[a.go + o]);
+        const float be = sj + go * sc + go * a.bo[o] + (hr[a.boo + o] + th[a.boo + o]);
+        a.beff[(size_t)(p0 + g) * 2 + o] = be;
+        bad |= !(fabsf(be) <= FLT_MAX);
+    }
+
+    {
+        const int i0 = tid, i1 = tid + 256;
+        const bool on0 = i0 < a.d, on1 = i1 < a.d;
+        const float* w0p = a.W3 + (on0 ? i0 : 0);
+        const float* w1p = a.W3 + (on1 ? i1 : 0);
+        float acc0[G2], acc1[G2];
+#pragma unroll
+        for (int k = 0; k < G2; ++k) acc0[k] = acc1[k] = 0.f;
+        for (int j0 = 0; j0 < a.dmid; j0 += 32) {
+            float part0[G2], part1[G2];
+#pragma unroll
+            for (int k = 0; k < G2; ++k) part0[k] = part1[k] = 0.f;
+            const int j1 = j0 + 32 < a.dmid ? j0 + 32 : a.dmid;
+#pragma unroll 4
+            for (int j = j0; j < j1; ++j) {
+                const float w0 = w0p[(size_t)j * a.d], w1 = w1p[(size_t)j * a.d];
+#pragma unroll
+                for (int k4 = 0; k4 < G2; k4 += 4) {
+                    const f32x4 u = *reinterpret_cast<const f32x4*>(&s_u[j][k4]);
+#pragma unroll
+                    for (int e = 0; e < 4; ++e) {
+                        part0[k4 + e] = fmaf(u[e], w0, part0[k4 + e]);
+                        part1[k4 + e] = fmaf(u[e], w1, part1[k4 + e]);
+                    }
+                }
+            }
+#pragma unroll
+            for (int k = 0; k < G2; ++k) {
+                acc0[k] += part0[k];
+                acc1[k] += part1[k];
+            }
+        }
+#pragma unroll
+        for (int k = 0; k < G2; ++k) {
+            if (p0 + (k >> 1) >= pairs) break;
+            float* row = a.weff + ((size_t)(p0 + (k >> 1)) * 2 + (k & 1)) * a.d;
+            if (on0) {
+                row[i0] = acc0[k];
+                bad |= !(fabsf(acc0[k]) <= FLT_MAX);
+            }
+            if (on1) {
+                row[i1] = acc1[k];
+                bad |= !(fabsf(acc1[k]) <= FLT_MAX);
+            }
+        }
+    }
+    if (bad) atomicOr(a.range_flag, 1);
+}
+
+inline hipError_t launch_tail_fold_table(const TailTableArgs& a, hipStream_t st) {
+    const long pairs = (long)a.steps * a.R;
+    hipLaunchKernelGGL(tail_fold_table_kernel, dim3((unsigned)((pairs + kTailG - 1) / kTailG)), dim3(256), 0, st, a);
+    return hipGetLastError();
+}
+
+struct TailFoldArgs {
+    const half_t* Xh;
+    const half_t* Xl;
+    const float* weff;
+    const float* beff;
+    int d;
+};
+
+struct TailMap {
+    f32x4 w[2][2];
+    float b0, b1;
+};
+__device__ __forceinline__ void tail_fold_map(const TailFoldArgs& f, int ea, int lane, TailMap& t) {
+    const bool on = lane * 8 < f.d;
+#pragma unroll
+    for (int o = 0; o < 2; ++o) {
+        const float* row = f.weff + ((size_t)ea * 2 + o) * f.d + lane * 8;
+        t.w[o][0] = on ? *reinterpret_cast<const f32x4*>(row) : f32x4{0.f, 0.f, 0.f, 0.f};
+        t.w[o][1] = on ? *reinterpret_cast<const f32x4*>(row + 4) : f32x4{0.f, 0.f, 0.f, 0.f};
+    }
+    t.b0 = f.beff[(size_t)ea * 2];
+    t.b1 = f.beff[(size_t)ea * 2 + 1];
+}
+__device__ __forceinline__ f16x8 tail_fold_load(const half_t* plane, int d, int m, int lane) {
+    f16x8 x = {0, 0, 0, 0, 0, 0, 0, 0};
+    if (lane * 8 < d) x = *reinterpret_cast<const f16x8*>(plane + blk_index(m, lane * 8, d));
+    return x;
+}
+template <bool LO>
+__device__ __forceinline__ void tail_fold_dot(f16x8 xh, f16x8 xl, const TailMap& t, float& e0, float& e1) {
+    float s0 = 0.f, s1 = 0.f;
+#pragma unroll
+    for (int e = 0; e < 8; ++e) {
+        const float v = LO ? (float)xh[e] + (float)xl[e] : (float)xh[e];
+        s0 = fmaf(v, t.w[0][e >> 2][e & 3], s0);
+        s1 = fmaf(v, t.w[1][e >> 2][e & 3], s1);
+    }
+    e0 = wave_sum(s0) + t.b0;
+    e1 = wave_sum(s1) + t.b1;
+}
+__device__ __forceinline__ void tail_fold_update(const OutArgs& a, float e0, float e1, float x0, float x1, float z0, float z1,
+                                                 float& xn0, float& xn1) {
+    if (a.ddpm) {
+        xn0 = a.c0 * (x0 - a.c1 * e0) + a.sigma * z0;
+        xn1 = a.c0 * (x1 - a.c1 * e1) + a.sigma * z1;
+    } else {
+        const float p0 = (x0 - e0 * a.c_e) / a.c_x, p1 = (x1 - e1 * a.c_e) / a.c_x;
+        xn0 = a.n_x * p0 + a.n_e * e0;
+        xn1 = a.n_x * p1 + a.n_e * e1;
+    }
+}
+
+template <bool EMBED_NEXT, bool LO>
+__global__ __launch_bounds__(256) void tail_fold_kernel(TailFoldArgs f, OutArgs a, EmbedArgs nxt) {
+    args_now_each(f, a, nxt);
+    const int lane = threadIdx.x & 63;
+    const int m = blockIdx.x * (blockDim.x >> 6) + (threadIdx.x >> 6);
+    if (m >= a.M) return;
+    const f16x8 xh = tail_fold_load(f.Xh, f.d, m, lane);
+    const f16x8 xl = LO ? tail_fold_load(f.Xl, f.d, m, lane) : xh;
+    TailMap t;
+    tail_fold_map(f, a.rmap.ea(m), lane, t);
+    const float x0 = a.e_out ? 0.f : a.x[2 * (size_t)m], x1 = a.e_out ? 0.f : a.x[2 * (size_t)m + 1];
+    const float z0 = (a.ddpm && a.z) ? a.z[2 * (size_t)m] : 0.f, z1 = (a.ddpm && a.z) ? a.z[2 * (size_t)m + 1] : 0.f;
+    float e0, e1;
+    tail_fold_dot<LO>(xh, xl, t, e0, e1);
+    float xn0 = 0.f, xn1 = 0.f;
+    if (a.e_out) {
+        if (lane == 0) {
+            a.e_out[2 * (size_t)m] = e0;
+            a.e_out[2 * (size_t)m + 1] = e1;
+        }
+    } else {
+        tail_fold_update(a, e0, e1, x0, x1, z0, z1, xn0, xn1);
+        if (lane == 0) {
+            a.x[2 * (size_t)m] = xn0;
+            a.x[2 * (size_t)m + 1] = xn1;
+        }
+    }
+    if (EMBED_NEXT) embed_row(nxt, m, lane, xn0, xn1);
+}
+
+template <bool EMBED_NEXT, bool LO>
+__global__ __launch_bounds__(256) void tail_fold_traj_kernel(TailFoldArgs f, OutArgs a, EmbedArgs nxt, int tpw) {
+    args_now_each(f, a, nxt);
+    const int lane = threadIdx.x & 63;
+    const int piece = blockIdx.x * (blockDim.x >> 6) + (threadIdx.x >> 6);
+    const int m0 = piece * tpw;
+    if (m0 >= a.M) return;
+    const int t0 = a.rmap.t_of(m0), ea = a.rmap.ea(m0);
+    EmbedCols c[2];
+    const int j0 = lane * 4, j1 = lane * 4 + 256;
+    if (EMBED_NEXT) {
+        const float* hrow = nxt.hyp + (size_t)ea * nxt.hyp_ld;
+        if (j0 < nxt.d) embed_cols(nxt, j0, hrow, c[0]);
+        if (j1 < nxt.d) embed_cols(nxt, j1, hrow, c[1]);
+    }
+    TailMap t;
+    tail_fold_map(f, ea, lane, t);
+    for (int tb = 0; tb < tpw; tb += 12) {
+        const int nb = tpw - tb < 12 ? tpw - tb : 12;
+        f16x8 xh[12], xl[LO ? 12 : 1];
+#pragma unroll
+        for (int u = 0; u < 12; ++u) {
+            const int m = m0 + tb + (u < nb ? u : 0);
+            xh[u] = tail_fold_load(f.Xh, f.d, m, lane);
+            if (LO) xl[LO ? u : 0] = tail_fold_load(f.Xl, f.d, m, lane);
+        }
+        const int mu = m0 + tb + (lane < nb ? lane : 0);
+        const float xl0 = a.e_out ? 0.f : a.x[2 * (size_t)mu], xl1 = a.e_out ? 0.f : a.x[2 * (size_t)mu + 1];
+        const float zl0 = (a.ddpm && a.z) ? a.z[2 * (size_t)mu] : 0.f, zl1 = (a.ddpm && a.z) ? a.z[2 * (size_t)mu + 1] : 0.f;
+#pragma unroll
+        for (int u = 0; u < 12; ++u) {
+            if (u >= nb) continue;
+            const int m = m0 + tb + u;
+            float e0, e1;
+            tail_fold_dot<LO>(xh[u], LO ? xl[LO ? u : 0] : xh[u], t, e0, e1);
+            float xn0 = 0.f, xn1 = 0.f;
+            if (a.e_out) {
+                if (lane == 0) {
+                    a.e_out[2 * (size_t)m] = e0;
+                    a.e_out[2 * (size_t)m + 1] = e1;
+                }
+            } else {
+                tail_fold_update(a, e0, e1, __shfl(xl0, u, 64), __shfl(xl1, u, 64), __shfl(zl0, u, 64), __shfl(zl1, u, 64), xn0, xn1);
+                if (lane == 0) {
+                    a.x[2 * (size_t)m] = xn0;
+                    a.x[2 * (size_t)m + 1] = xn1;
+                }
+            }
+            if (EMBED_NEXT) {
+                if (j0 < nxt.d) embed_store_cols(nxt, m, j0, t0 + tb + u, xn0, xn1, c[0]);
+                if (j1 < nxt.d) embed_store_cols(nxt, m, j1, t0 + tb + u, xn0, xn1, c[1]);
+            }
+        }
+    }
+}
+
+#ifdef JMID_DIAGNOSTICS
+static __global__ void tail_split_rows_kernel(const float* in, half_t* hi, half_t* lo, int rows, int K) {
+    const size_t n = (size_t)rows * K;
+    for (size_t i = (size_t)blockIdx.x * blockDim.x + threadIdx.x; i < n; i += (size_t)gridDim.x * blockDim.x) {
+        half_t h, l;
+        split_f32(in[i], h, l);
+        const size_t o = blk_index((int)(i / K), (int)(i % K), K);
+        hi[o] = h;
+        if (lo) lo[o] = l;
+    }
+}
+#endif
+
+}
diff --git a/safe-interactive-crowdnav_amd/engine.py b/safe-interactive-crowdnav_amd/engine.py
--- a/safe-interactive-crowdnav_amd/engine.py
+++ b/safe-interactive-crowdnav_amd/engine.py
@@ -626,5 +626,19 @@
                                             _lib.PRECISIONS[precision], C.c_void_p(out.ctypes.data), C.c_void_p(thyp.ctypes.data)))
         return out, thyp
 
+    def dbg_tail(self, X: np.ndarray, hyp: np.ndarray, step: int, dims: Tuple[int, int, int, int], precision: str = "f16mx"):
+        E, A, K, T = (int(v) for v in dims)
+        X = np.ascontiguousarray(X, np.float32)
+        hyp = np.ascontiguousarray(hyp, np.float32)
+        M, d = E * K * A * T, 2 * self.dims.ctx_dim
+        width = self.hyper_width()
+        if X.shape != (M, d) or hyp.shape != (E * A, width):
+            raise ValueError(f"expected X [{M}, {d}] and hyp [{E * A}, {width}]")
+        out = np.empty((M, 2), np.float32)
+        thyp = np.empty((width,), np.float32)
+        self._check(self._lib.jmid_dbg_tail(self._h, E, A, K, T, C.c_void_p(X.ctypes.data), C.c_void_p(hyp.ctypes.data), width, int(step),
+                                            _lib.PRECISIONS[precision], C.c_void_p(out.ctypes.data), C.c_void_p(thyp.ctypes.data)))
+        return out, thyp
+
     def hyper_width(self) -> int:
         return 2 * self.dims.d_model + 2 * self.dims.d_mid + 2 * self.dims.d_low + 4
```
